# frankyeh/UNet-Studio

Measured on AMD Instinct MI355X. Metric: voxels/sec 3D U-Net train step @128^3 bf16, higher is better.
Workload: dtype bf16

## Files before the change

### include/unet_hip.h

```cpp
#ifndef UNET_HIP_H
#define UNET_HIP_H
#include <stddef.h>
#include <stdint.h>

#ifdef __cplusplus
extern "C" {
#endif

#define UNET_DTYPE_F32 0
#define UNET_DTYPE_BF16 1

#define UNET_IMPL_AUTO 0
#define UNET_IMPL_DIRECT 1

typedef struct unet_plan unet_plan;

const char* unet_last_error(void);
void unet_set_error(const char* msg);

int unet_init(int* n_devices);
int unet_device_info(int device, char* name, size_t name_len, size_t* total_mem, int* compute_units, int* gcn_arch_is_gfx950);

int unet_plan_create(const char* arch_dsl, int in_c, int out_c, int D, int H, int W, int dtype, int device, int impl,
                     unet_plan** out);
void unet_plan_destroy(unet_plan* plan);

int unet_plan_param_count(const unet_plan* plan, int* n);
int unet_plan_param_shape(const unet_plan* plan, int i, int64_t dims[5], int* ndim);
int unet_plan_param_name(const unet_plan* plan, int i, char* name, size_t name_len);
int unet_plan_param_decay(const unet_plan* plan, int i, int* decay);
int unet_plan_param_fan_in(const unet_plan* plan, int i, int64_t* fan_in, int* is_norm_weight);
int unet_plan_buffer_count(const unet_plan* plan, int* n);
int unet_plan_buffer_shape(const unet_plan* plan, int i, int64_t* numel);
int unet_plan_output_count(const unet_plan* plan, int* n);
int unet_plan_output_shape(const unet_plan* plan, int level, int64_t dims[5]);
int unet_plan_workspace_bytes(const unet_plan* plan, size_t* bytes);
int unet_plan_flops(const unet_plan* plan, double* fwd, double* bwd);
size_t unet_plan_describe(const unet_plan* plan, char* buf, size_t len);

int unet_plan_op_count(const unet_plan* plan, int* n);
int unet_plan_op_info(const unet_plan* plan, int i, int* kind, int* cin, int* cout, int* ks, int* stride, int64_t in_dims[3],
                      int64_t out_dims[3], char* name, size_t name_len);

#define UNET_PROF_CONV_FWD 0
#define UNET_PROF_DGRAD 1
#define UNET_PROF_WGRAD 2
#define UNET_PROF_NORM_FWD 3
#define UNET_PROF_NORM_BWD 4
#define UNET_PROF_OTHER 5
int unet_profile_begin(void);
int unet_profile_end(int max_records, int* op_index, int* category, float* ms, int* n_records);

#define UNET_MODE_PACKS_CURRENT 2
int unet_forward(const unet_plan* plan, const float* const* params, float* const* buffers, const float* x,
                 float* const* outs, void* workspace, int mode, void* stream);

int unet_backward(const unet_plan* plan, const float* const* params, const float* const* grad_outs,
                  float* const* grad_params, float* grad_x, void* workspace, void* stream);

int unet_plan_backward_buckets(const unet_plan* plan, int max_buckets, int* n_buckets, int* op_lo, int64_t* elem_lo);
int unet_backward_part(const unet_plan* plan, const float* const* params, const float* const* grad_outs, float* const* grad_params,
                       float* grad_x, void* workspace, int op_hi, int op_lo, void* stream);

int unet_loss_scratch_bytes(const unet_plan* plan, size_t* bytes);
int unet_loss(const unet_plan* plan, const float* const* outs, const int64_t* target, int cost_mask, int collapse_before,
              float* const* grad_outs, float* losses_out, void* scratch, void* stream);

int unet_forward_loss(const unet_plan* plan, const float* const* params, float* const* buffers, const float* x, float* const* outs,
                      const int64_t* target, int cost_mask, int collapse_before, float* const* grad_outs, float* losses_out,
                      void* loss_scratch, void* workspace, void* stream);
int unet_forward_loss_mode(const unet_plan* plan, const float* const* params, float* const* buffers, const float* x, float* const* outs,
                           const int64_t* target, int cost_mask, int collapse_before, float* const* grad_outs, float* losses_out,
                           void* loss_scratch, void* workspace, int mode, void* stream);

int unet_stream_create_cu_range(int device, int cu_first, int cu_count, void** stream);
int unet_stream_destroy(void* stream);
int unet_plan_side_cu_range(unet_plan* plan, int cu_first, int cu_count);

int unet_pack_filters(const unet_plan* plan, const float* const* params, void* workspace, int with_dgrad, int* made, void* stream);

#define UNET_SUM_MAX_BUFFERS 64
int unet_sum_buffers(const float* const* bufs, int n, float* out, int64_t count, int zero_inputs, void* stream);

int unet_sgd_step(const unet_plan* plan, float* params_flat, float* grads_flat, float* momentum_flat, float lr,
                  float momentum, int nesterov, float weight_decay, float clip_norm, float grad_scale, float* norm_out,
                  void* scratch, void* stream);

int unet_op_scratch_bytes(int cin, int cout, int D, int H, int W, size_t* bytes);
int unet_op_conv3d_fwd(int dtype, int impl, const void* x, const float* w, const float* b, void* y, int cin, int cout, int D,
                       int H, int W, int ks, int stride, void* scratch, void* stream);
int unet_op_conv3d_fwd_fused(int dtype, int impl, const void* x, const float* scale, const float* shift, int act, const float* w,
                             const float* b, void* y, float* stats, int cin, int cout, int D, int H, int W, int ks, int stride,
                             void* scratch, void* stream);
int unet_op_conv3d_pack(int dtype, const float* w, void* wpacked, int cin, int cout, int D, int H, int W, int ks, int stride,
                        void* stream);
int unet_op_conv3d_fwd_packed(int dtype, const void* x, const void* wpacked, const float* b, void* y, float* stats_partials,
                              int cin, int cout, int D, int H, int W, int ks, int stride, void* stream);
int unet_op_conv3d_bwd_data(int dtype, int impl, const void* dy, const float* w, void* dx, int cin, int cout, int D, int H,
                            int W, int ks, int stride, void* scratch, void* stream);
int unet_op_conv3d_fwd_norm(const void* x0, const void* x1, int cin0, int cin1, const float* w, const float* b, const float* gamma,
                            const float* beta, double eps, float* rm, float* rv, double momentum, int use_running, int act, void* y,
                            void* y_act, float* stat, int cout, int D, int H, int W, int stride, void* scratch, void* stream);
int unet_op_conv3d_bwd_data_norm(int transposed, const void* dy, const float* w, void* dx, int accumulate, const void* u, const float* stat,
                                 const float* gamma, int act, float* coef, float* dgamma, float* dbeta, int cin, int cout, int D, int H,
                                 int W, void* scratch, void* stream);
int unet_op_conv3d_bwd_weight(int dtype, int impl, const void* x, const void* dy, float* dw, float* db, int cin, int cout,
                              int D, int H, int W, int ks, int stride, void* scratch, void* stream);
int unet_op_convt_fwd(int dtype, int impl, const void* x, const float* w, const float* b, void* y, int cin, int cout, int D,
                      int H, int W, void* scratch, void* stream);
int unet_op_convt_bwd_data(int dtype, int impl, const void* dy, const float* w, void* dx, int cin, int cout, int D, int H,
                           int W, void* scratch, void* stream);
int unet_op_convt_bwd_weight(int dtype, int impl, const void* x, const void* dy, float* dw, float* db, int cin, int cout,
                             int D, int H, int W, void* scratch, void* stream);
int unet_op_pack_ndhwc(int dtype, const float* x_ncdhw, void* y_ndhwc, int C, int64_t S, void* stream);
int unet_op_unpack_ncdhw(int dtype, const void* x_ndhwc, float* y_ncdhw, int C, int64_t S, void* stream);

#define UNET_COMM_ID_BYTES 128
typedef struct unet_comm unet_comm;
int unet_comm_unique_id(void* id_bytes );
int unet_comm_create(int rank, int world, const void* id_bytes, int device, unet_comm** out);
int unet_comm_create_all(int n, const int* devices, unet_comm** out );
int unet_comm_destroy(unet_comm* comm);
int unet_comm_rank(const unet_comm* comm, int* rank, int* world);
int unet_allreduce_grads(unet_comm* comm, float* flat, int64_t elem_lo, int64_t elem_hi, void* stream);
int unet_allreduce_grads_all(unet_comm* const* comms, int n, float* const* flats, int64_t elem_lo, int64_t elem_hi, void* const* streams);
int unet_comm_broadcast(unet_comm* comm, float* buf, int64_t n, int root, void* stream);
int unet_comm_join(unet_comm* comm, void* stream);

#ifdef __cplusplus
}
#endif
#endif
```

### unet-studio_amd/csrc/engine.cpp

```cpp
#include <hip/hip_runtime.h>

#include <algorithm>
#include <atomic>
#include <cmath>
#include <cstdio>
#include <cstring>
#include <functional>
#include <stdexcept>
#include <string>
#include <mutex>
#include <random>
#include <unordered_map>
#include <vector>

#include "../../include/unet_hip.h"
#include "conv_select.h"
#include "graph.hpp"
#include "kernels.h"

using namespace unet;

namespace {

thread_local std::string g_err;
int fail(const std::string& m) { g_err = m; return 1; }

#define HIP_OK(expr)                                                                              \
    do {                                                                                          \
        hipError_t e_ = (expr);                                                                   \
        if (e_ != hipSuccess) throw std::runtime_error(std::string(#expr) + ": " + hipGetErrorString(e_)); \
    } while (0)

struct DeviceGuard {
    int prev = -1;
    explicit DeviceGuard(int dev) {
        HIP_OK(hipGetDevice(&prev));
        if (prev != dev) HIP_OK(hipSetDevice(dev));
        else prev = -1;
    }
    ~DeviceGuard() { if (prev >= 0) (void)hipSetDevice(prev); }
};

size_t align_up(size_t v, size_t a = 256) { return (v + a - 1) / a * a; }

struct EnvSwitches {
    bool no_side_stream = getenv("UNET_NO_SIDE_STREAM"), no_first_wgrad_fuse = getenv("UNET_NO_FIRST_WGRAD_FUSE"), op_polite = getenv("UNET_OP_POLITE");
};
const EnvSwitches& env() { static const EnvSwitches e; return e; }

struct ProfRec { int op, cat; hipEvent_t e0, e1; };
struct ProfSink { std::vector<ProfRec> recs; };
thread_local ProfSink* g_prof = nullptr;
struct ProfScope {
    ProfRec r{};
    hipStream_t s = nullptr;
    bool on = false;
    ProfScope(int op, int cat, hipStream_t st) {
        if (!g_prof) return;
        on = true; s = st; r.op = op; r.cat = cat;
        if (hipEventCreate(&r.e0) != hipSuccess || hipEventCreate(&r.e1) != hipSuccess) { on = false; return; }
        (void)hipEventRecord(r.e0, s);
    }
    ~ProfScope() {
        if (!on) return;
        (void)hipEventRecord(r.e1, s);
        g_prof->recs.push_back(r);
    }
};

}

struct unet_plan {
    Graph g;
    int dtype = 0, device = 0, impl = 0;
    size_t elsize = 4;
    std::vector<size_t> t_off, g_off;
    std::vector<size_t> a_off;
    std::vector<size_t> n_stat, n_coef;
    std::vector<size_t> w_fwd, w_dgrad;
    std::vector<size_t> wm_fwd, wm_dgrad;
    std::vector<int> n_consumers;
    std::vector<int> first_consumer;
    mutable std::mutex bn_mu;
    mutable std::unordered_map<const void*, std::pair<int, int>> bn_pending;
    mutable std::unordered_map<const void*, std::vector<int>> bn_done;
    std::vector<ConvChoice> conv;
    size_t wgrad_off = 0;
    std::vector<size_t> wz_off;
    std::vector<int> wz_job_of_op;
    std::vector<WgradReduceJob> wz_jobs;
    WgradReduceJob* wz_jobs_dev = nullptr;
    size_t partial_off = 0, partial_bytes = 0;
    size_t ws_bytes = 0;
    size_t loss_bytes = 0;
    std::vector<int64_t> p_off;
    std::vector<PackJob> pack_jobs;
    int64_t pack_blocks = 0;
    PackJob* jobs_dev = nullptr;
    SgdSeg* segs_dev = nullptr;
    int nseg = 0;
    int64_t n_param_elems = 0;

    hipStream_t side = nullptr;
    hipEvent_t ev_fork = nullptr, ev_join = nullptr, ev_pack = nullptr, ev_packd = nullptr;
    int pack_split_op = 0;
    int64_t pack_split_blocks = 0, pack_fwd_blocks = 0;
    size_t head_off = 0;
    size_t deep_part_off = 0, deep_part_bytes = 0, deep_cnt_off = 0;
    static constexpr int deep_ncnt = 4096;
    std::vector<size_t> head_op_off;

    ~unet_plan() {
        if (segs_dev) (void)hipFree(segs_dev);
        if (wz_jobs_dev) (void)hipFree(wz_jobs_dev);
        if (jobs_dev) (void)hipFree(jobs_dev);
        if (ev_fork) (void)hipEventDestroy(ev_fork);
        if (ev_join) (void)hipEventDestroy(ev_join);
        if (ev_pack) (void)hipEventDestroy(ev_pack);
        if (ev_packd) (void)hipEventDestroy(ev_packd);
        if (side) (void)hipStreamDestroy(side);
    }

    ConvGeom op_geom_of(const Op& op) const {
        const Tensor& a = g.tensors[op.src[0]];
        const Tensor& o = g.tensors[op.dst];
        ConvGeom cg;
        cg.Cin = op.cin; cg.Cout = op.cout; cg.D = a.D; cg.H = a.H; cg.W = a.W; cg.Do = o.D; cg.Ho = o.H; cg.Wo = o.W;
        cg.ks = op.ks; cg.stride = op.stride;
        return cg;
// ... 19 lines not shown
            const Op& op = g.ops[i];
            if (op.kind == OP_CONV || op.kind == OP_CONVT) side_polite[i] = wgrad_on_main[i] ? 0 : 1;
        }
    }

    bool head_only(size_t t) const {
        if (dtype != UNET_DTYPE_BF16 || g.tensors[t].norm < 0 || g.tensors[t].C % 16) return false;
        int readers = 0;
        for (size_t i = 0; i < g.ops.size(); ++i) {
            const Op& op = g.ops[i];
            if (op.kind == OP_NORM) continue;
            for (int k = 0; k < op.nsrc; ++k) {
                if (op.src[k] != (int)t) continue;
                if (conv[i].fwd != Fwd::head) return false;
                ++readers;
            }
        }
        return readers > 0;
    }
    void layout() {
        choose_polite();
        conv.assign(g.ops.size(), ConvChoice());
        for (size_t i = 0; i < g.ops.size(); ++i) {
            const Op& op = g.ops[i];
            if (op.kind != OP_CONV && op.kind != OP_CONVT) continue;
            SrcDesc sd[2];
            src_chans(op, sd);
            conv[i] = choose_conv(dtype, impl, op_geom_of(op), sd, op.nsrc, op.out_level >= 0, op.kind == OP_CONVT);
        }
        size_t off = 0;
        auto take = [&](size_t bytes) { size_t o = off; off = align_up(off + bytes); return o; };
        t_off.assign(g.tensors.size(), SIZE_MAX);
        g_off.assign(g.tensors.size(), SIZE_MAX);
        n_consumers.assign(g.tensors.size(), 0);
        first_consumer.assign(g.tensors.size(), -1);
        for (size_t oi = 0; oi < g.ops.size(); ++oi) {
            const Op& op = g.ops[oi];
            for (int k = 0; k < op.nsrc && op.kind != OP_NORM; ++k)
                if (op.src[k] >= 0) { ++n_consumers[op.src[k]]; if (first_consumer[op.src[k]] < 0) first_consumer[op.src[k]] = (int)oi; }
        }
        a_off.assign(g.tensors.size(), SIZE_MAX);
        for (size_t i = 0; i < g.tensors.size(); ++i) {
            t_off[i] = take((size_t)g.tensors[i].numel() * elsize);
            if (g.tensors[i].needs_grad) g_off[i] = take((size_t)g.tensors[i].numel() * elsize);
            if (impl == UNET_IMPL_AUTO && (g.tensors[i].norm >= 0 || g.tensors[i].act != ACT_NONE) && !head_only(i))
                a_off[i] = take((size_t)g.tensors[i].numel() * elsize);
        }
        n_stat.resize(g.norms.size()); n_coef.resize(g.norms.size());
        size_t pmax = 0;
        for (size_t i = 0; i < g.norms.size(); ++i) {
            n_stat[i] = take(4 * (size_t)g.norms[i].C * 4);
            n_coef[i] = take(3 * (size_t)g.norms[i].C * 4);
            size_t pb = (size_t)stats_blocks(g.tensors[g.norms[i].tensor].voxels()) * g.norms[i].C * 2 * (dtype == UNET_DTYPE_F32 ? 8 : 4);
            if (pb > pmax) pmax = pb;
        }
        w_fwd.assign(g.ops.size(), SIZE_MAX); w_dgrad.assign(g.ops.size(), SIZE_MAX);
        wm_fwd.assign(g.ops.size(), SIZE_MAX); wm_dgrad.assign(g.ops.size(), SIZE_MAX);
        auto grow = [](size_t& m, size_t b) { if (b > m) m = b; };
        for (size_t i = 0; i < g.ops.size(); ++i) {
            const Op& op = g.ops[i];
            if (op.kind != OP_CONV && op.kind != OP_CONVT) continue;
            const ConvChoice& c = conv[i];
            const ConvGeom cg = op_geom_of(op);
            int k3 = op.kind == OP_CONV ? op.ks * op.ks * op.ks : 8;
            w_fwd[i] = take((size_t)k3 * op.cin * round_up(op.cout, 8) * 4);
            w_dgrad[i] = take((size_t)k3 * op.cout * round_up(op.cin, 8) * 4);
            if (op.kind == OP_CONVT) {
                if (c.mfma_fwd()) { wm_fwd[i] = take(mfma_convt_w_bytes(cg)); wm_dgrad[i] = take(mfma_convt_dgrad_w_bytes(cg)); }
                continue;
            }
            const bool stats = g.tensors[op.dst].norm >= 0;
            SrcDesc sd[2];
            src_chans(op, sd);
            if (c.mfma_fwd()) {
                wm_fwd[i] = take(mfma_conv_w_bytes(cg));
                if (stats) grow(pmax, (size_t)mfma_conv_blocks(cg) * op.cout * 2 * 4);
            }
            if (c.fwd == Fwd::first_f32_mfma && stats) grow(pmax, (size_t)conv_first_f32_mfma_blocks(cg) * op.cout * 2 * 8);
            if (c.fwd == Fwd::f32_mfma && stats) grow(pmax, (size_t)conv_f32_mfma_stat_rows(cg, sd) * op.cout * 2 * 8);
            if (c.dgrad == Dgrad::mfma) {
                wm_dgrad[i] = take(mfma_conv_dgrad_w_bytes(cg));
                if (op.stride == 2) grow(pmax, (size_t)s2_conv_dgrad_rows_max() * op.cin * 2 * 4);
            }
        }
        partial_bytes = pmax ? pmax : 256;
        partial_off = take(partial_bytes);
        size_t wmax = 0, hmax = 0;
        for (size_t i = 0; i < g.ops.size(); ++i) {
            const Op& op = g.ops[i];
            if (op.kind != OP_CONV && op.kind != OP_CONVT) continue;
            const ConvChoice& c = conv[i];
            const ConvGeom cg = op_geom_of(op);
            grow(wmax, wgrad_direct_scratch_bytes(cg, op.kind == OP_CONVT));
            if (op.kind == OP_CONVT) {
                if (c.wgrad == Wgrad::mfma) {
                    grow(wmax, mfma_convt_wgrad_scratch_bytes(cg));
                    grow(wmax, bias_grad_scratch_bytes(cg.Cout, (int64_t)cg.Do * cg.Ho * cg.Wo));
                }
                continue;
            }
            if (c.wgrad == Wgrad::mfma) grow(wmax, mfma_wgrad_scratch_bytes(cg, side_polite[i]));
            if (c.wgrad == Wgrad::f32_mfma) grow(wmax, wgrad_f32_mfma_scratch_bytes(cg));
            if (wgrad_small_supported(cg, op.nsrc)) grow(wmax, wgrad_small_scratch_bytes(cg));
            if (cg.Cin == 1 && (cg.Cout == 16 || cg.Cout == 32)) grow(wmax, conv_first_wgrad_mfma_scratch_bytes(cg));
            if (head_supported(cg, op.nsrc)) grow(hmax, head_bwd_scratch_bytes(cg));
        }
        wgrad_off = take(wmax ? wmax : 256);
        head_off = take(hmax ? hmax : 256);
        if (dtype == UNET_DTYPE_BF16 && impl == UNET_IMPL_AUTO) {
            deep_part_bytes = (size_t)8 << 20;
            deep_part_off = take(deep_part_bytes);
            deep_cnt_off = take((size_t)deep_ncnt * 4);
        }
        head_op_off.assign(g.ops.size(), SIZE_MAX);
        for (size_t i = 0; i < g.ops.size(); ++i)
            if (conv[i].fwd == Fwd::head) head_op_off[i] = take(head_bwd_scratch_bytes(op_geom_of(g.ops[i])));
        wz_off.assign(g.ops.size(), SIZE_MAX);
        for (size_t i = 0; i < g.ops.size(); ++i) {
            const Op& op = g.ops[i];
            const Wgrad w = conv[i].wgrad;
            if (op.out_level >= 0 || (w != Wgrad::first_mfma && w != Wgrad::mfma)) continue;
            const ConvGeom cg = op_geom_of(op);
            if (w == Wgrad::first_mfma) wz_off[i] = take(conv_first_wgrad_mfma_scratch_bytes(cg));
            else if (op.kind == OP_CONV) { if (!mfma_conv_wgrad_direct(cg)) wz_off[i] = take(mfma_wgrad_scratch_bytes(cg, side_polite[i])); }
            else if (!mfma_convt_wgrad_direct(cg)) wz_off[i] = take(mfma_convt_wgrad_scratch_bytes(cg));
        }
        ws_bytes = off;
        p_off.assign(g.params.size() + 1, 0);
        for (size_t i = 0; i < g.params.size(); ++i) {
            int64_t n = 1;
            for (auto d : g.params[i].shape) n *= d;
            p_off[i + 1] = p_off[i] + n;
        }
        wz_jobs.clear();
        wz_job_of_op.assign(g.ops.size(), -1);
        int wz_blk = 0;
        for (size_t i = 0; i < g.ops.size(); ++i) {
            if (wz_off[i] == SIZE_MAX) continue;
            const Op& op = g.ops[i];
            ConvGeom cg = op_geom_of(op);
            WgradReduceJob j;
            j.op = (int)i;
            j.slab_off = (long long)(wz_off[i] / 4);
            j.dw_off = p_off[op.weight];
            j.Cb = op.cout;
            if (op.kind == OP_CONVT) {
                j.nsplit = mfma_convt_wgrad_splits(cg);
                j.n = (long long)8 * op.cin * op.cout;
                j.bias_off = op.bias >= 0 ? j.slab_off + (long long)j.nsplit * j.n : -1;
                j.db_off = op.bias >= 0 ? p_off[op.bias] : -1;
            } else {
                j.nsplit = conv[i].wgrad == Wgrad::first_mfma ? conv_first_wgrad_splits(cg) : mfma_conv_wgrad_splits(cg, side_polite[i]);
                j.n = (long long)27 * op.cin * op.cout;
                j.bias_off = op.bias >= 0 ? j.slab_off + (long long)j.nsplit * j.n : -1;
                j.db_off = op.bias >= 0 ? p_off[op.bias] : -1;
            }
            wz_blk += wgrad_reduce_job_blocks(j, wz_blk);
            wz_job_of_op[i] = (int)wz_jobs.size();
            wz_jobs.push_back(j);
        }
        pack_jobs.clear();
        pack_blocks = 0;
        pack_split_op = -1; pack_split_blocks = 0; pack_fwd_blocks = 0;
        for (int which = 0; which < 2; ++which) {
            for (size_t i = 0; i < g.ops.size(); ++i) {
                const Op& op = g.ops[i];
// ... 193 lines not shown
                        case Fwd::first_f32_mfma:
                            rows = launch_conv_first_f32_mfma(cg, sd, params[op.weight], params[op.bias], (float*)tptr(op.dst), (double*)part, s);
                            if (mode == 1 && !packs_current) launch_pack_conv_w(params[op.weight], wf, wd, op.cin, op.cout, k3, s);
                            break;
                        case Fwd::f32_mfma:
                            if (!packs_current) launch_pack_conv_w(params[op.weight], wf, wd, op.cin, op.cout, k3, s);
                            rows = launch_conv_f32_mfma(cg, sd, op.nsrc, wf, params[op.bias], (float*)tptr(op.dst), s, (double*)part);
                            break;
                        case Fwd::direct:
                            if (!packs_current) launch_pack_conv_w(params[op.weight], wf, wd, op.cin, op.cout, k3, s);
                            launch_conv_fwd_direct(p.dtype, cg, sd, op.nsrc, wf, params[op.bias], tptr(op.dst),
                                                   op.out_level >= 0 ? outs[op.out_level] : nullptr, s);
                            break;
                    }
                    if (want_stats) {
                        fused_blocks[T.norm] = rows;
                        fused_dbl[T.norm] = c.fwd == Fwd::first_f32_mfma || c.fwd == Fwd::f32_mfma;
                    }
                    break;
                }
                case OP_NORM: {
                    const Norm& n = g.norms[op.norm];
                    const Tensor& T = g.tensors[n.tensor];
                    if (fused_done[op.norm]) break;
                    norm_fwd_passes(p.dtype, tptr(n.tensor), n.C, T.voxels(), partial(), fused_blocks[op.norm], fused_dbl[op.norm] != 0,
                                    n.batch && mode == 0, params[n.gamma], params[n.beta], n.eps, stat(op.norm),
                                    n.batch ? buffers[n.buffer] : nullptr, n.batch ? buffers[n.buffer + 1] : nullptr, T.act,
                                    p.a_off[n.tensor] != SIZE_MAX ? ws + p.a_off[n.tensor] : nullptr, s);
                    break;
                }
                case OP_MATERIALIZE: {
                    SrcDesc sd[2] = {src(op.src[0]), op.nsrc > 1 ? src(op.src[1]) : SrcDesc()};
                    launch_materialize(p.dtype, sd, op.nsrc, tptr(op.dst), g.tensors[op.dst].voxels(), s);
                    break;
                }
                case OP_MAXPOOL: {
                    const Tensor& a = g.tensors[op.src[0]];
                    launch_maxpool_fwd(p.dtype, src(op.src[0]), tptr(op.dst), a.D, a.H, a.W, s);
                    break;
                }
                case OP_UPSAMPLE: {
                    const Tensor& a = g.tensors[op.src[0]];
                    launch_upsample_fwd(p.dtype, src(op.src[0]), tptr(op.dst), a.D, a.H, a.W, s);
                    break;
                }
                case OP_EXPORT:
                    if (outs && outs[op.out_level])
                        launch_export(p.dtype, src(op.src[0]), outs[op.out_level], g.tensors[op.src[0]].voxels(), s);
                    break;
            }
            if (op.kind != OP_NORM && op.kind != OP_EXPORT && op.dst >= 0) {
                const Tensor& T = g.tensors[op.dst];
                if (T.norm < 0 && T.act != ACT_NONE) apply_view(op.dst);
            }
            if (on_head && op.out_level >= 0 && outs && outs[op.out_level] && (op.kind == OP_CONV || op.kind == OP_CONVT || op.kind == OP_EXPORT))
                (*on_head)(op.out_level);
        }
        need_packs();
    }

    void view_backward(int t, const float* const* params, float* const* gparams, bool no_apply = false) {
        const Tensor& T = p.g.tensors[t];
        if (T.norm >= 0) {
            const Norm& n = p.g.norms[T.norm];
            int have = 0;
            {
                std::lock_guard<std::mutex> lk(p.bn_mu);
                auto d = p.bn_done.find(ws);
                if (d != p.bn_done.end()) {
                    auto f = std::find(d->second.begin(), d->second.end(), t);
                    if (f != d->second.end()) { d->second.erase(f); return; }
                }
                auto it = p.bn_pending.find(ws);
                if (it != p.bn_pending.end()) { if (it->second.first == t) have = it->second.second; p.bn_pending.erase(it); }
            }
            norm_bwd_passes(p.dtype, gptr(t), tptr(t), T.C, T.voxels(), stat(T.norm), T.act, params[n.gamma], coef(T.norm),
                            gparams[n.gamma], gparams[n.beta], partial(), have, no_apply, s);
        } else if (T.act != ACT_NONE) {
            launch_act_bwd(p.dtype, gptr(t), tptr(t), T.act, T.numel(), s);
        }
    }

    void backward(const float* const* params, const float* const* grad_outs, float* const* gparams, float* grad_x, int op_hi = 1 << 30,
                  int op_lo = 0) {
        const Graph& g = p.g;
        if (p.side) HIP_OK(hipStreamWaitEvent(s, p.ev_packd, 0));
        {
            bool flat = p.jobs_dev != nullptr;
            for (size_t k = 0; k < g.params.size() && flat; ++k) flat = params[k] == params[0] + p.p_off[k];
            deep_on = flat;
        }
        std::vector<char> init(g.tensors.size(), 0);
        auto dst_of = [&](int t) {
            DstGrad d;
            d.C = g.tensors[t].C;
            d.ptr = g.tensors[t].needs_grad ? gptr(t) : nullptr;
            d.accumulate = init[t];
            return d;
        };
        auto mark = [&](const Op& op) {
            for (int k = 0; k < op.nsrc; ++k)
                if (g.tensors[op.src[k]].needs_grad) init[op.src[k]] = 1;
        };
        const hipStream_t sb = (p.side && !env().no_side_stream && !g_prof) ? p.side : s;
        auto fork = [&]() {
            if (sb == s) return;
            HIP_OK(hipEventRecord(p.ev_fork, s));
            HIP_OK(hipStreamWaitEvent(sb, p.ev_fork, 0));
        };
        if (op_lo < 0) op_lo = 0;
        if (op_hi >= (int)g.ops.size()) { std::lock_guard<std::mutex> lk(p.bn_mu); p.bn_pending.erase(ws); p.bn_done.erase(ws); }
        bool gflat = p.wz_jobs_dev != nullptr;
        for (size_t k = 0; k < g.params.size() && gflat; ++k) gflat = gparams[k] == gparams[0] + p.p_off[k];
        std::vector<char> wz_ran(p.wz_jobs.size(), 0);
        int wz_pending = 0;
        auto flush_wz = [&](hipStream_t st) {
            for (size_t j = 0; j < wz_ran.size();) {
                if (!wz_ran[j]) { ++j; continue; }
                size_t e = j;
                int nblk = 0;
                while (e < wz_ran.size() && wz_ran[e]) { nblk += p.wz_jobs[e].nblk; wz_ran[e] = 0; ++e; }
                ProfScope pr(-1, UNET_PROF_WGRAD, st);
                launch_wgrad_reduce_batched(p.wz_jobs_dev, (int)j, (int)(e - j), p.wz_jobs[j].blk0, nblk, ws, gparams[0], st);
                j = e;
            }
            wz_pending = 0;
        };
        auto do_wgrad = [&](int i) {
            const Op& op = g.ops[i];
            const int t = op.dst;
            SrcDesc sd[2] = {src(op.src[0]), op.nsrc > 1 ? src(op.src[1]) : SrcDesc()};
            ConvGeom cg = geom(op);
            const bool on_main = op.kind == OP_CONV && p.wgrad_on_main[i] && p.wz_off[i] != SIZE_MAX;
            const bool defer = gflat && p.wz_job_of_op[i] >= 0 && !on_main;
            {
            ProfScope pw(i, UNET_PROF_WGRAD, sb);
            switch (p.conv[i].wgrad) {
                case Wgrad::first_mfma:
                    launch_conv_first_wgrad_mfma(cg, sd, gptr(t), gparams[op.weight], gparams[op.bias],
                                                 ws + (defer ? p.wz_off[i] : p.wgrad_off), sb, defer);
                    break;
                case Wgrad::mfma:
                    if (op.kind == OP_CONVT)
                        launch_mfma_convt_wgrad(cg, sd, gptr(t), gparams[op.weight], ws + (defer ? p.wz_off[i] : p.wgrad_off), sb, defer, gparams[op.bias],
                                                p.side_polite[i]);
                    else if (on_main)
                        launch_mfma_conv_wgrad(cg, sd, op.nsrc, gptr(t), gparams[op.weight], gparams[op.bias], ws + p.wz_off[i], s, false, 0);
                    else
                        launch_mfma_conv_wgrad(cg, sd, op.nsrc, gptr(t), gparams[op.weight], gparams[op.bias],
                                               ws + (p.wz_off[i] != SIZE_MAX ? p.wz_off[i] : p.wgrad_off), sb, defer, p.side_polite[i]);
                    break;
                case Wgrad::f32_mfma:
                    launch_wgrad_f32_mfma(cg, sd, op.nsrc, (const float*)gptr(t), gparams[op.weight], gparams[op.bias], ws + p.wgrad_off, sb);
                    break;
                case Wgrad::small:
                    launch_conv_wgrad_small(p.dtype, cg, sd, op.nsrc, gptr(t), gparams[op.weight], gparams[op.bias], ws + p.wgrad_off, sb);
                    break;
                case Wgrad::direct:
                    if (op.kind == OP_CONVT)
                        launch_convt_wgrad_direct(p.dtype, cg, sd, op.nsrc, gptr(t), gparams[op.weight], gparams[op.bias], ws + p.wgrad_off, sb);
                    else
                        launch_conv_wgrad_direct(p.dtype, cg, sd, op.nsrc, gptr(t), gparams[op.weight], gparams[op.bias], ws + p.wgrad_off, sb);
                    break;
            }
            }
            if (defer) { wz_ran[p.wz_job_of_op[i]] = 1; ++wz_pending; }
            if (wz_pending >= 3) flush_wz(sb);
        };
        const int64_t hold_from = (int64_t)64 * 64 * 64, hold_below = (int64_t)32 * 32 * 32;
        std::vector<int> held;
        bool deep_seen = false;
        constexpr int fork_every = 3;
        std::vector<int> pending;
        auto issue_pending = [&]() {
            if (pending.empty()) return;
            fork();
            for (int h : pending) do_wgrad(h);
            pending.clear();
        };
        for (int i = (int)g.ops.size() - 1; i >= op_lo; --i) {
            const Op& op = g.ops[i];
            const bool dry = i >= op_hi;
            if (op.kind == OP_NORM) continue;
            if (op.kind == OP_EXPORT) {
                if (grad_outs && grad_outs[op.out_level] && g.tensors[op.src[0]].needs_grad) {
                    if (!dry) launch_export_bwd(p.dtype, grad_outs[op.out_level], dst_of(op.src[0]), g.tensors[op.src[0]].voxels(), s);
                    mark(op);
                }
                continue;
            }
            int t = op.dst;
            if ((op.kind == OP_CONV) && op.out_level >= 0) {
                if (!(grad_outs && grad_outs[op.out_level])) continue;
                if (p.conv[i].fwd == Fwd::head) {
                    DstGrad dgh = dst_of(op.src[0]);
                    ProfScope ph(dry ? -2 : i, UNET_PROF_OTHER, s);
                    if (!dry) {
                        const bool defer = sb != s && p.head_op_off[i] != SIZE_MAX;
                        char* hs = ws + (defer ? p.head_op_off[i] : p.head_off);
                        launch_head_bwd(p.dtype, geom(op), src(op.src[0]), grad_outs[op.out_level], nullptr, params[op.weight], dgh,
                                        gparams[op.weight], gparams[op.bias], hs, s, defer);
                        if (defer) { fork(); launch_head_bwd_reduce(geom(op), gparams[op.weight], gparams[op.bias], hs, sb); }
                    }
                    if (dgh.ptr) mark(op);
                    continue;
                }
                if (!dry) launch_import_grad(p.dtype, grad_outs[op.out_level], gptr(t), g.tensors[t].C, g.tensors[t].voxels(), 0, s);
                init[t] = 1;
            }
            if (!g.tensors[t].needs_grad || !init[t]) continue;
            bool first_fused = false;
            if (!dry && p.conv[i].wgrad == Wgrad::first_mfma && g.tensors[t].norm >= 0 && !g.tensors[op.src[0]].needs_grad && sb != s &&
                p.wz_off[i] != SIZE_MAX && g.tensors[t].C % 8 == 0)
                first_fused = !env().no_first_wgrad_fuse;
            if (!dry) { ProfScope ps(i, UNET_PROF_NORM_BWD, s); view_backward(t, params, gparams, first_fused); }
            switch (op.kind) {
                case OP_CONV:
                case OP_CONVT: {
                    SrcDesc sd[2] = {src(op.src[0]), op.nsrc > 1 ? src(op.src[1]) : SrcDesc()};
                    DstGrad dg[2] = {dst_of(op.src[0]), op.nsrc > 1 ? dst_of(op.src[1]) : DstGrad()};
                    ConvGeom cg = geom(op);
                    const float* wd = (const float*)(ws + p.w_dgrad[i]);
                    bool any = dg[0].ptr || (op.nsrc > 1 && dg[1].ptr);
                    if (!dry && !any && sb != s && p.conv[i].wgrad == Wgrad::first_mfma && p.wz_off[i] != SIZE_MAX) {
                        ProfScope pw(i, UNET_PROF_WGRAD, s);
                        const Tensor& To = g.tensors[t];
                        NormBwdFuse nf = {tptr(t), first_fused ? stat(To.norm) : nullptr, first_fused ? coef(To.norm) : nullptr, To.act};
                        launch_conv_first_wgrad_mfma(cg, sd, gptr(t), gparams[op.weight], gparams[op.bias], ws + p.wz_off[i], s, false,
                                                     first_fused ? &nf : nullptr);
                    } else
                    if (!dry) {
                        const int64_t vox = (int64_t)cg.Do * cg.Ho * cg.Wo;
                        if (!deep_seen && vox <= hold_below && !held.empty()) {
                            deep_seen = true;
                            pending.insert(pending.begin(), held.begin(), held.end());
                            held.clear();
                            pending.push_back(i);
                            issue_pending();
                        } else if (!deep_seen && sb != s && vox >= hold_from) held.push_back(i);
                        else {
                            pending.push_back(i);
                            if ((int)pending.size() >= fork_every || sb == s || vox >= hold_below) issue_pending();
                        }
                    }
                    ProfScope pd(i, UNET_PROF_DGRAD, s);
                    if (!dry && any) switch (p.conv[i].dgrad) {
                        case Dgrad::mfma: {
                            const int ts = op.src[0];
                            const Tensor& Ts = g.tensors[ts];
                            const bool can = op.nsrc == 1 && Ts.norm >= 0 && p.first_consumer[ts] == i && p.dtype == UNET_DTYPE_BF16;
                            DeepNormBwd nb;
                            if (can) {
                                const Norm& n = g.norms[Ts.norm];
                                nb = {tptr(ts), stat(Ts.norm), params[n.gamma], coef(Ts.norm), gparams[n.gamma], gparams[n.beta], Ts.act};
                            }
                            if (op.kind == OP_CONVT) {
                                int norm_done = 0;
                                if (deep_on && launch_deep_convt_dgrad(cg, gptr(t), ws + p.wm_dgrad[i], dg, op.nsrc, can ? &nb : nullptr, deep(), &norm_done, s)) {
                                    if (norm_done) { std::lock_guard<std::mutex> lk(p.bn_mu); p.bn_done[ws].push_back(ts); }
                                } else
                                    launch_mfma_convt_dgrad(cg, gptr(t), ws + p.wm_dgrad[i], dg, op.nsrc, s);
                                break;
                            }
                            BnBwdStats bn = {tptr(ts), Ts.norm >= 0 ? stat(Ts.norm) : nullptr, partial(), Ts.act, Ts.C};
                            int rows = 0;
                            const int served = deep_on ? launch_deep_conv_dgrad(cg, gptr(t), ws + p.wm_dgrad[i], dg, op.nsrc, can ? &nb : nullptr, deep(), s) : 0;
                            if (served == 2) { std::lock_guard<std::mutex> lk(p.bn_mu); p.bn_done[ws].push_back(ts); }
                            if (!served) rows = launch_mfma_conv_dgrad(cg, gptr(t), ws + p.wm_dgrad[i], dg, op.nsrc, s, can ? &bn : nullptr);
                            if (rows > 0) { std::lock_guard<std::mutex> lk(p.bn_mu); p.bn_pending[ws] = {ts, rows}; }
                            break;
                        }
                        case Dgrad::f32_mfma: launch_conv_f32_mfma_dgrad(cg, (const float*)gptr(t), wd, dg, op.nsrc, s); break;
                        case Dgrad::direct:
                            if (op.kind == OP_CONVT) launch_convt_dgrad_direct(p.dtype, cg, gptr(t), wd, dg, op.nsrc, s);
                            else launch_conv_dgrad_direct(p.dtype, cg, gptr(t), wd, dg, op.nsrc, s);
// ... 142 lines not shown
    if (i < 0 || i >= (int)p->g.params.size()) return fail("parameter index out of range");
    const auto& s = p->g.params[i].shape;
    *ndim = (int)s.size();
    for (size_t k = 0; k < s.size(); ++k) dims[k] = s[k];
    return 0;
}
int unet_plan_param_name(const unet_plan* p, int i, char* name, size_t name_len) {
    if (i < 0 || i >= (int)p->g.params.size()) return fail("parameter index out of range");
    if (name && name_len) { std::strncpy(name, p->g.params[i].name.c_str(), name_len - 1); name[name_len - 1] = 0; }
    return 0;
}
int unet_plan_param_decay(const unet_plan* p, int i, int* decay) {
    if (i < 0 || i >= (int)p->g.params.size()) return fail("parameter index out of range");
    *decay = p->g.params[i].decay;
    return 0;
}
int unet_plan_param_fan_in(const unet_plan* p, int i, int64_t* fan_in, int* is_norm_weight) {
    if (i < 0 || i >= (int)p->g.params.size()) return fail("parameter index out of range");
    *fan_in = p->g.params[i].fan_in; *is_norm_weight = p->g.params[i].norm_weight;
    return 0;
}
int unet_plan_buffer_count(const unet_plan* p, int* n) { *n = (int)p->g.buffers.size(); return 0; }
int unet_plan_buffer_shape(const unet_plan* p, int i, int64_t* numel) {
    if (i < 0 || i >= (int)p->g.buffers.size()) return fail("buffer index out of range");
    *numel = p->g.buffers[i];
    return 0;
}
int unet_plan_output_count(const unet_plan* p, int* n) { *n = (int)p->g.outputs.size(); return 0; }
int unet_plan_output_shape(const unet_plan* p, int l, int64_t dims[5]) {
    if (l < 0 || l >= (int)p->g.outputs.size()) return fail("output level out of range");
    const auto& o = p->g.outputs[l];
    dims[0] = 1; dims[1] = o.C; dims[2] = o.D; dims[3] = o.H; dims[4] = o.W;
    return 0;
}
int unet_plan_workspace_bytes(const unet_plan* p, size_t* bytes) { *bytes = p->ws_bytes; return 0; }
int unet_plan_flops(const unet_plan* p, double* fwd, double* bwd) { *fwd = p->g.flops_fwd; *bwd = p->g.flops_bwd; return 0; }
size_t unet_plan_describe(const unet_plan* p, char* buf, size_t len) {
    std::string d = p->g.describe();
    if (buf && len) { std::strncpy(buf, d.c_str(), len - 1); buf[len - 1] = 0; }
    return d.size() + 1;
}

int unet_forward(const unet_plan* p, const float* const* params, float* const* buffers, const float* x, float* const* outs,
                 void* workspace, int mode, void* stream) {
    try {
        if (!p || !params || !x || !workspace) throw std::runtime_error("unet_forward: null argument");
        if (mode & ~(1 | UNET_MODE_PACKS_CURRENT)) throw std::runtime_error("unet_forward: unknown mode bits (0 = eval, 1 = train, optionally | UNET_MODE_PACKS_CURRENT)");
        if (!p->g.buffers.empty() && !buffers) throw std::runtime_error("unet_forward: architecture has bnorm layers but buffers is null");
        DeviceGuard dg(p->device);
        Exec ex(*p, workspace, stream);
        ex.forward(params, buffers, x, outs, mode);
        check_launch();
        return 0;
    } catch (const std::exception& e) { return fail(e.what()); }
}

int unet_backward(const unet_plan* p, const float* const* params, const float* const* grad_outs, float* const* grad_params,
                  float* grad_x, void* workspace, void* stream) {
    try {
        if (!p || !params || !grad_params || !workspace) throw std::runtime_error("unet_backward: null argument");
        if (grad_x) throw std::runtime_error("unet_backward: grad_x must be NULL -- dL/dx is not computed (the input carries no gradient, as in train.cpp:619-628)");
        DeviceGuard dg(p->device);
        Exec ex(*p, workspace, stream);
        ex.backward(params, grad_outs, grad_params, grad_x);
        check_launch();
        return 0;
    } catch (const std::exception& e) { return fail(e.what()); }
}

int unet_backward_part(const unet_plan* p, const float* const* params, const float* const* grad_outs, float* const* grad_params,
                       float* grad_x, void* workspace, int op_hi, int op_lo, void* stream) {
    try {
        if (!p || !params || !grad_params || !workspace) throw std::runtime_error("unet_backward_part: null argument");
        if (op_lo < 0 || op_hi < op_lo) throw std::runtime_error("unet_backward_part: invalid op range");
        if (grad_x) throw std::runtime_error("unet_backward_part: grad_x must be NULL -- dL/dx is not computed");
        DeviceGuard dg(p->device);
        Exec ex(*p, workspace, stream);
        ex.backward(params, grad_outs, grad_params, grad_x, op_hi, op_lo);
        check_launch();
        return 0;
    } catch (const std::exception& e) { return fail(e.what()); }
}

int unet_plan_backward_buckets(const unet_plan* p, int max_buckets, int* n_buckets, int* op_lo, int64_t* elem_lo) {
    try {
        if (!p || !n_buckets || !op_lo || !elem_lo || max_buckets < 1) throw std::runtime_error("unet_plan_backward_buckets: bad argument");
        const Graph& g = p->g;
        const int nops = (int)g.ops.size();
        std::vector<int64_t> first(nops, INT64_MAX);
        bool monotone = true;
        int64_t prev = -1;
        for (int i = 0; i < nops; ++i) {
            const Op& op = g.ops[i];
            if (op.kind != OP_CONV && op.kind != OP_CONVT) continue;
            int64_t f = p->p_off[op.weight];
            if (op.bias >= 0 && p->p_off[op.bias] < f) f = p->p_off[op.bias];
            first[i] = f;
            if (f <= prev) monotone = false;
            prev = f;
            const Tensor& T = g.tensors[op.dst];
            if (T.norm >= 0) {
                const Norm& n = g.norms[T.norm];
                if (p->p_off[n.gamma] < f || p->p_off[n.beta] < f) monotone = false;
            }
        }
        int nb = 0;
        if (monotone && max_buckets > 1) {
            const double thr = (double)p->n_param_elems / ((double)max_buckets - 0.5);
            int64_t hi = p->n_param_elems;
            for (int i = nops - 1; i > 0 && nb < max_buckets - 1; --i) {
                if (first[i] == INT64_MAX) continue;
                if ((double)(hi - first[i]) >= thr) { op_lo[nb] = i; elem_lo[nb] = first[i]; hi = first[i]; ++nb; }
            }
        }
        op_lo[nb] = 0; elem_lo[nb] = 0; ++nb;
        *n_buckets = nb;
        return 0;
    } catch (const std::exception& e) { return fail(e.what()); }
}

int unet_plan_op_count(const unet_plan* p, int* n) { *n = (int)p->g.ops.size(); return 0; }
int unet_plan_op_info(const unet_plan* p, int i, int* kind, int* cin, int* cout, int* ks, int* stride, int64_t in_dims[3],
                      int64_t out_dims[3], char* name, size_t name_len) {
    if (i < 0 || i >= (int)p->g.ops.size()) return fail("op index out of range");
    const Op& op = p->g.ops[i];
    if (kind) *kind = (int)op.kind;
    if (cin) *cin = op.cin;
    if (cout) *cout = op.cout;
    if (ks) *ks = op.ks;
    if (stride) *stride = op.stride;
    const Tensor* a = op.nsrc > 0 && op.src[0] >= 0 ? &p->g.tensors[op.src[0]] : nullptr;
    const Tensor* o = op.dst >= 0 ? &p->g.tensors[op.dst] : nullptr;
    if (in_dims) { in_dims[0] = a ? a->D : 0; in_dims[1] = a ? a->H : 0; in_dims[2] = a ? a->W : 0; }
    if (out_dims) { out_dims[0] = o ? o->D : 0; out_dims[1] = o ? o->H : 0; out_dims[2] = o ? o->W : 0; }
    if (name && name_len) { std::strncpy(name, op.name.c_str(), name_len - 1); name[name_len - 1] = 0; }
    return 0;
}

int unet_profile_begin(void) {
    if (g_prof) return fail("unet_profile_begin: a profile is already open on this thread");
    g_prof = new ProfSink();
    return 0;
}
int unet_profile_end(int max_records, int* op_index, int* category, float* ms, int* n_records) {
    if (!g_prof) return fail("unet_profile_end: no open profile on this thread");
    ProfSink* ps = g_prof;
    g_prof = nullptr;
    int n = 0, rc = 0;
    for (auto& r : ps->recs) {
        float t = 0.f;
        hipError_t e = hipEventSynchronize(r.e1);
        if (e == hipSuccess) e = hipEventElapsedTime(&t, r.e0, r.e1);
        if (e != hipSuccess) rc = fail(std::string("unet_profile_end: ") + hipGetErrorString(e));
        if (r.op != -2 && n < max_records && op_index && category && ms) { op_index[n] = r.op; category[n] = r.cat; ms[n] = t; ++n; }
        (void)hipEventDestroy(r.e0); (void)hipEventDestroy(r.e1);
    }
    if (n_records) *n_records = n;
    delete ps;
    return rc;
}

int unet_loss_scratch_bytes(const unet_plan* p, size_t* bytes) { *bytes = p->loss_bytes; return 0; }

namespace {
struct LossRun {
    const unet_plan* p;
    const float* const* outs; const int64_t* target; float* const* grad_outs; float* losses_out;
    int C, oc, collapse, cost_mask;
    float inv;
    std::vector<int64_t*> tgt;
    std::vector<float*> lvl;
    float* partial[2];
    LossRun(const unet_plan* plan, const float* const* outs_, const int64_t* target_, int cost_mask_, int collapse_before, float* const* grad_outs_,
            float* losses_out_, void* scratch)
        : p(plan), outs(outs_), target(target_), grad_outs(grad_outs_), losses_out(losses_out_), collapse(collapse_before), cost_mask(cost_mask_) {
        if (!p || !outs || !target || !losses_out || !scratch) throw std::runtime_error("unet_loss: null argument");
        const Graph& g = p->g;
        C = g.out_c;
        if (collapse_before < 0 || collapse_before >= C) throw std::runtime_error("invalid collapse_before");
        oc = collapse_before ? C - collapse_before + 1 : C;
        const size_t nl = g.outputs.size();
        float wsum = 0.f;
        for (size_t k = 0; k < nl; ++k) wsum += 1.0f / (float)(1 << k);
        inv = 1.0f / wsum;
        char* sc = (char*)scratch;
        size_t off = 0;
        tgt.resize(nl); lvl.resize(nl);
        for (size_t l = 0; l < nl; ++l) {
            int64_t S = (int64_t)(g.D >> l) * (g.H >> l) * (g.W >> l);
            if (S <= 0) S = 1;
            tgt[l] = (int64_t*)(sc + off); off = align_up(off + (size_t)S * 8);
            lvl[l] = (float*)(sc + off); off = align_up(off + (size_t)(4 + 2 * C) * 4);
        }
        partial[0] = (float*)(sc + off); off = align_up(off + (size_t)1024 * (3 + 2 * C) * 4);
        partial[1] = (float*)(sc + off);
        int D = g.D, H = g.H, W = g.W;
        for (size_t k = 0; k < nl; ++k) {
            if (k > 0) {
                if ((D >> 1) <= 0 || (H >> 1) <= 0 || (W >> 1) <= 0) throw std::runtime_error("deep supervision target size became zero");
                D >>= 1; H >>= 1; W >>= 1;
            }
            const auto& o = g.outputs[k];
            if (o.C == 0 || !outs[k]) throw std::runtime_error("undefined deep supervision output at level " + std::to_string(k));
            if (o.C != C)
                throw std::runtime_error("output channel mismatch at level " + std::to_string(k) + ": tensor has " + std::to_string(o.C) +
                                         ", out_count is " + std::to_string(C));
            if (o.D != D || o.H != H || o.W != W) throw std::runtime_error("deep supervision output/target size mismatch at level " + std::to_string(k));
        }
    }
    size_t levels() const { return p->g.outputs.size(); }
    const int64_t* target_of(size_t k) const { return k == 0 ? target : tgt[k]; }
    int64_t voxels(size_t k) const { const auto& o = p->g.outputs[k]; return (int64_t)o.D * o.H * o.W; }
    void prepare(hipStream_t s) {
        HIP_OK(hipMemsetAsync(losses_out, 0, 4 * sizeof(float), s));
        const Graph& g = p->g;
        int D = g.D, H = g.H, W = g.W;
        for (size_t k = 1; k < levels(); ++k) {
            launch_target_half(target_of(k - 1), tgt[k], D, H, W, s);
            D >>= 1; H >>= 1; W >>= 1;
        }
    }
    void level_partial(size_t k, int area, hipStream_t s) { launch_loss_partial(outs[k], target_of(k), C, voxels(k), collapse, partial[area], s); }
    void level_finish(size_t k, int area, hipStream_t s) {
        const float w = (1.0f / (float)(1 << k)) * inv;
        launch_loss_finalize(partial[area], loss_blocks(voxels(k)), oc, w, cost_mask, lvl[k], losses_out, k == 0, s);
        if (grad_outs && grad_outs[k]) launch_loss_grad(outs[k], target_of(k), C, voxels(k), collapse, lvl[k], w, cost_mask, grad_outs[k], s);
    }
};
}

int unet_loss(const unet_plan* p, const float* const* outs, const int64_t* target, int cost_mask, int collapse_before,
              float* const* grad_outs, float* losses_out, void* scratch, void* stream) {
    try {
        LossRun lr(p, outs, target, cost_mask, collapse_before, grad_outs, losses_out, scratch);
        DeviceGuard dg(p->device);
        hipStream_t s = (hipStream_t)stream;
        lr.prepare(s);
        for (size_t k = 0; k < lr.levels(); ++k) { lr.level_partial(k, 0, s); lr.level_finish(k, 0, s); }
        check_launch();
        return 0;
    } catch (const std::exception& e) { return fail(e.what()); }
}

int unet_forward_loss(const unet_plan* p, const float* const* params, float* const* buffers, const float* x, float* const* outs,
                      const int64_t* target, int cost_mask, int collapse_before, float* const* grad_outs, float* losses_out,
                      void* loss_scratch, void* workspace, void* stream) {
    return unet_forward_loss_mode(p, params, buffers, x, outs, target, cost_mask, collapse_before, grad_outs, losses_out, loss_scratch, workspace, 1,
                                  stream);
}

int unet_forward_loss_mode(const unet_plan* p, const float* const* params, float* const* buffers, const float* x, float* const* outs,
                           const int64_t* target, int cost_mask, int collapse_before, float* const* grad_outs, float* losses_out,
                           void* loss_scratch, void* workspace, int mode, void* stream) {
    try {
        if ((mode & 1) != 1 || (mode & ~(1 | UNET_MODE_PACKS_CURRENT)))
            throw std::runtime_error("unet_forward_loss_mode: mode must be 1 (train), optionally | UNET_MODE_PACKS_CURRENT");
        if (!p || !params || !x || !workspace || !outs) throw std::runtime_error("unet_forward_loss: null argument");
        if (!p->g.buffers.empty() && !buffers) throw std::runtime_error("unet_forward_loss: architecture has bnorm layers but buffers is null");
        LossRun lr(p, outs, target, cost_mask, collapse_before, grad_outs, losses_out, loss_scratch);
        DeviceGuard dg(p->device);
        hipStream_t s = (hipStream_t)stream;
        const bool side = p->side && !env().no_side_stream && !g_prof;
        Exec ex(*p, workspace, stream);
        if (!side) {
            ex.forward(params, buffers, x, outs, mode);
            lr.prepare(s);
            for (size_t k = 0; k < lr.levels(); ++k) { lr.level_partial(k, 0, s); lr.level_finish(k, 0, s); }
            check_launch();
            return 0;
        }
        hipStream_t sd = p->side;
        bool prepared = false;
        constexpr bool per_level = false;
        std::function<void(int)> on_head = [&](int level) {
            if (level < 1 || (size_t)level >= lr.levels()) return;
            if (!per_level && level != 1) return;
            HIP_OK(hipEventRecord(p->ev_fork, s));
            HIP_OK(hipStreamWaitEvent(sd, p->ev_fork, 0));
            if (!prepared) { lr.prepare(sd); prepared = true; }
            for (size_t k = per_level ? (size_t)level : lr.levels() - 1; k >= (size_t)level; --k) {
                lr.level_partial(k, 1, sd);
                lr.level_finish(k, 1, sd);
            }
        };
        ex.forward(params, buffers, x, outs, mode, &on_head);
        if (!prepared) {
            HIP_OK(hipEventRecord(p->ev_fork, s));
            HIP_OK(hipStreamWaitEvent(sd, p->ev_fork, 0));
            lr.prepare(sd);
        }
        lr.level_partial(0, 0, s);
        HIP_OK(hipEventRecord(p->ev_join, sd));
        HIP_OK(hipStreamWaitEvent(s, p->ev_join, 0));
        lr.level_finish(0, 0, s);
        check_launch();
        return 0;
    } catch (const std::exception& e) { return fail(e.what()); }
}

static bool create_cu_range_stream(int device, int cu_first, int cu_count, hipStream_t* out) {
    hipDeviceProp_t prop;
    if (cu_count <= 0 || hipGetDeviceProperties(&prop, device) != hipSuccess || prop.multiProcessorCount % 8 != 0) return false;
    const int per_xcd = prop.multiProcessorCount / 8;
    if (cu_count >= per_xcd) return false;
    std::vector<uint32_t> mask((prop.multiProcessorCount + 31) / 32, 0u);
    for (int c = 0; c < cu_count; ++c) {
        const int cu = ((cu_first + c) % per_xcd + per_xcd) % per_xcd;
        for (int x = 0; x < 8; ++x) { const int bit = cu * 8 + x; mask[bit / 32] |= 1u << (bit % 32); }
    }
    if (hipExtStreamCreateWithCUMask(out, (uint32_t)mask.size(), mask.data()) != hipSuccess) { (void)hipGetLastError(); return false; }
    return true;
}

int unet_stream_create_cu_range(int device, int cu_first, int cu_count, void** stream) {
    try {
        if (!stream) throw std::runtime_error("unet_stream_create_cu_range: null argument");
        DeviceGuard dg(device);
        hipStream_t st = nullptr;
        if (!create_cu_range_stream(device, cu_first, cu_count, &st)) throw std::runtime_error("unet_stream_create_cu_range: the device / driver does not take this CU range");
        *stream = (void*)st;
        return 0;
    } catch (const std::exception& e) { return fail(e.what()); }
}
int unet_stream_destroy(void* stream) {
    if (stream && hipStreamDestroy((hipStream_t)stream) != hipSuccess) return fail("hipStreamDestroy failed");
    return 0;
}
int unet_plan_side_cu_range(unet_plan* p, int cu_first, int cu_count) {
    try {
        if (!p) throw std::runtime_error("unet_plan_side_cu_range: null plan");
        if (!p->side) return 0;
        DeviceGuard dg(p->device);
        hipStream_t st = nullptr;
        if (!create_cu_range_stream(p->device, cu_first, cu_count, &st)) throw std::runtime_error("unet_plan_side_cu_range: the device / driver does not take this CU range");
        HIP_OK(hipStreamSynchronize(p->side));
        HIP_OK(hipStreamDestroy(p->side));
        p->side = st;
        return 0;
    } catch (const std::exception& e) { return fail(e.what()); }
}

int unet_pack_filters(const unet_plan* p, const float* const* params, void* workspace, int with_dgrad, int* made, void* stream) {
// ... 556 lines not shown
```

### unet-studio_amd/csrc/kernels.h

```cpp
#pragma once
#include <hip/hip_runtime.h>
#include <cstdint>

#include "../../include/unet_augment.h"
#include "../../include/unet_feed.h"
#include "../../include/unet_hip.h"
#include "../../include/unet_postproc.h"
#include "../../include/unet_qc.h"

namespace unet {

struct SrcDesc {
    const void* ptr = nullptr;
    int C = 0;
    const float* scale = nullptr;
    const float* shift = nullptr;
    int act = 0;
};
struct DstGrad {
    void* ptr = nullptr;
    int C = 0;
    int accumulate = 0;
};

// ... 35 lines not shown
void launch_norm_eval(int C, const float* gamma, const float* beta, const float* rm, const float* rv, double eps, float* stat,
                      hipStream_t s);

void launch_act_bwd(int dtype, void* g, const void* u, int act, int64_t n, hipStream_t s);
void launch_norm_bwd_partial(int dtype, void* g, const void* u, int C, int64_t S, const float* stat, int act, float* partial,
                             hipStream_t s);
void launch_norm_bwd_finalize(const float* partial, int nblk, int C, int64_t S, const float* gamma, const float* stat, float* coef,
                              float* dgamma, float* dbeta, hipStream_t s, bool dbl = false);
bool launch_norm_finalize_apply(int dtype, const float* partial, int nblk, int C, int64_t S, const float* gamma, const float* beta, double eps,
                                float* stat, float* running_mean, float* running_var, double momentum, const void* raw, int act, void* out,
                                hipStream_t s);
bool launch_norm_bwd_finalize_apply(int dtype, const float* partial, int nblk, int C, int64_t S, const float* gamma, const float* stat,
                                    float* coef, float* dgamma, float* dbeta, void* g, const void* u, int act, hipStream_t s);
void launch_norm_bwd_apply(int dtype, void* g, const void* u, int C, int64_t S, const float* stat, const float* coef, int act,
                           hipStream_t s);

void launch_maxpool_fwd(int dtype, SrcDesc src, void* out, int D, int H, int W, hipStream_t s);
void launch_maxpool_bwd(int dtype, SrcDesc src, const void* gout, DstGrad dst, int D, int H, int W, hipStream_t s);
void launch_upsample_fwd(int dtype, SrcDesc src, void* out, int D, int H, int W, hipStream_t s);
void launch_upsample_bwd(int dtype, const void* gout, DstGrad dst, int D, int H, int W, hipStream_t s);
void launch_materialize(int dtype, const SrcDesc* src, int nsrc, void* out, int64_t S, hipStream_t s);
void launch_apply_view(int dtype, SrcDesc src, void* out, int64_t S, hipStream_t s);
void launch_materialize_bwd(int dtype, const void* gout, const DstGrad* dst, int ndst, int64_t S, hipStream_t s);
void launch_export_bwd(int dtype, const float* g_ncdhw, DstGrad dst, int64_t S, hipStream_t s);
void launch_unpack_ncdhw(int dtype, const void* g, float* out_ncdhw, int C, int64_t S, hipStream_t s);

void launch_target_half(const int64_t* t, int64_t* o, int D, int H, int W, hipStream_t s);
int loss_blocks(int64_t S);
void launch_loss_partial(const float* logits, const int64_t* target, int C, int64_t S, int collapse, float* partial, hipStream_t s);
void launch_loss_finalize(const float* partial, int nblk, int oc, float level_weight, int cost_mask, float* level_out, float* totals,
                          int set_stats, hipStream_t s);
void launch_loss_grad(const float* logits, const int64_t* target, int C, int64_t S, int collapse, const float* level_out,
                      float level_weight, int cost_mask, float* dlogits, hipStream_t s);

void launch_sum_buffers(const float* const* bufs, int n, float* out, int64_t count, int zero_inputs, hipStream_t s);

struct SgdSeg { int64_t offset, count; float wd; };
void launch_sumsq_partial(const float* g, int64_t n, float scale, float* partial, int nblk, hipStream_t s);
void launch_sgd(float* p, float* g, float* m, int64_t n, const SgdSeg* segs_dev, int nseg, const float* partial, int nblk,
                float lr, float momentum, int nesterov, float weight_decay, float clip_norm, float grad_scale, float* norm_out,
                hipStream_t s);

struct PackJob { int64_t src_off, dst_off, total, blk0; int Ci, Co, CK, T, mode, A, B, pad; };
int mfma_conv_pack_jobs(const ConvGeom& g, bool want_dgrad, PackJob* out2);
int mfma_convt_pack_jobs(const ConvGeom& g, PackJob* out2);
void launch_mfma_pack_batched(const float* params_base, void* ws, const PackJob* jobs_dev, int njobs, int64_t nblocks, hipStream_t s,
                              int64_t blk_base = 0, int max_grid = 0, int* zero = nullptr, int nzero = 0);
bool mfma_conv_fwd_supported(int dtype, const ConvGeom& g, const SrcDesc* src, int nsrc);
size_t mfma_conv_w_bytes(const ConvGeom& g);
void launch_mfma_pack_conv_w(const float* w, void* w_mfma_fwd, void* w_mfma_dgrad, const ConvGeom& g, hipStream_t s);
int launch_mfma_conv_fwd(const ConvGeom& g, const SrcDesc* src, int nsrc, const void* w_mfma, const float* bias, void* out,
                         float* stats_partial, hipStream_t s);
bool conv_first_mfma_supported(int dtype, const ConvGeom& g, const SrcDesc* src, int nsrc);
int conv_first_mfma_blocks(const ConvGeom& g);
int launch_conv_first_mfma(const ConvGeom& g, const SrcDesc* src, const float* w, const float* bias, void* out, float* stats_partial,
                           hipStream_t s);
int mfma_conv_blocks(const ConvGeom& g);
bool mfma_wgrad_z_supported(int dtype, const ConvGeom& g, const SrcDesc* src, int nsrc);
size_t mfma_wgrad_z_scratch_bytes(const ConvGeom& g, int polite = 0);
int mfma_wgrad_z_splits(const ConvGeom& g, int polite = 0);
int launch_mfma_wgrad_z(const ConvGeom& g, const SrcDesc* src, int nsrc, const void* dy, bool want_bias, void* scratch, hipStream_t s,
                        int polite = 0);
void wgrad_reduce(const float* slab, const float* bias_slab, int nsplit, int64_t n, int Cb, float* dw, float* db, hipStream_t s);
struct WgradReduceJob { long long slab_off, bias_off, dw_off, db_off, n; int nsplit, Cb, ly, blk0, nblk, op; };
int wgrad_reduce_job_blocks(WgradReduceJob& j, int blk0);
void launch_wgrad_reduce_batched(const WgradReduceJob* jobs_dev, int job0, int njobs, int blk_base, int nblocks, const void* ws, float* gflat,
                                 hipStream_t s);
bool mfma_wgrad_supported(int dtype, const ConvGeom& g, const SrcDesc* src, int nsrc);
size_t mfma_wgrad_scratch_bytes(const ConvGeom& g, int polite = 0);
int mfma_conv_wgrad_splits(const ConvGeom& g, int polite = 0);
int mfma_convt_wgrad_splits(const ConvGeom& g);
bool mfma_conv_wgrad_direct(const ConvGeom& g);
bool mfma_convt_wgrad_direct(const ConvGeom& g);
int conv_first_wgrad_splits(const ConvGeom& g);
void launch_mfma_conv_wgrad(const ConvGeom& g, const SrcDesc* src, int nsrc, const void* dy, float* dw, float* db, void* scratch,
                            hipStream_t s, bool defer_reduce = false, int polite = 0);
bool head_supported(const ConvGeom& g, int nsrc);
size_t head_bwd_scratch_bytes(const ConvGeom& g);
void launch_head_fwd(int dtype, const ConvGeom& g, const SrcDesc& src, const float* w, const float* bias, void* y, float* out_ncdhw,
                     hipStream_t s);
void launch_head_bwd(int dtype, const ConvGeom& g, const SrcDesc& src, const float* dy_ncdhw, const void* dy_cl, const float* w,
                     DstGrad dst, float* dw, float* db, void* scratch, hipStream_t s, bool defer_reduce = false);
void launch_head_bwd_reduce(const ConvGeom& g, float* dw, float* db, const void* scratch, hipStream_t s);
bool conv_first_wgrad_mfma_supported(int dtype, const ConvGeom& g, const SrcDesc* src, int nsrc);
size_t conv_first_wgrad_mfma_scratch_bytes(const ConvGeom& g);
struct NormBwdFuse { const void* u; const float* stat; const float* coef; int act; };
void launch_conv_first_wgrad_mfma(const ConvGeom& g, const SrcDesc* src, const void* dy, float* dw, float* db, void* scratch, hipStream_t s,
                                  bool defer_reduce = false, const NormBwdFuse* nb_fuse = nullptr);
bool wgrad_small_supported(const ConvGeom& g, int nsrc);
size_t wgrad_small_scratch_bytes(const ConvGeom& g);
void launch_conv_wgrad_small(int dtype, const ConvGeom& g, const SrcDesc* src, int nsrc, const void* dy, float* dw, float* db,
                             void* scratch, hipStream_t s);
bool mfma_convt_wgrad_supported(int dtype, const ConvGeom& g, const SrcDesc* src, int nsrc);
size_t mfma_convt_wgrad_scratch_bytes(const ConvGeom& g);
void launch_mfma_convt_wgrad(const ConvGeom& g, const SrcDesc* src, const void* dy, float* dw, void* scratch, hipStream_t s,
                             bool defer_reduce = false, float* db = nullptr, int polite = 0);
int launch_colsum_partial8(int dtype, const void* x, int C, int64_t S, float* partial, hipStream_t s);
size_t bias_grad_scratch_bytes(int C, int64_t S);
void launch_bias_grad(int dtype, const void* dy, int C, int64_t S, float* db, void* scratch, hipStream_t s);
bool mfma_conv_dgrad_supported(int dtype, const ConvGeom& g, const SrcDesc* src, int nsrc);
size_t mfma_conv_dgrad_w_bytes(const ConvGeom& g);
struct BnBwdStats { const void* u; const float* stat; float* partial; int act, C; };
int launch_mfma_conv_dgrad(const ConvGeom& g, const void* dy, const void* w_mfma_dgrad, const DstGrad* dst, int ndst, hipStream_t s,
                           const BnBwdStats* bn = nullptr);
int launch_s2_conv_fwd(const ConvGeom& g, const SrcDesc* src, int nsrc, const void* w_mfma, const float* bias, void* out, float* stats_partial,
                       hipStream_t s);
int launch_s2_conv_dgrad(const ConvGeom& g, const void* dy, const void* w_s2_dgrad, const DstGrad* dst, int ndst, hipStream_t s,
                         const BnBwdStats* bn);
int s2_conv_dgrad_rows_max();
bool launch_s2_convt_fwd(const ConvGeom& g, const SrcDesc* src, int nsrc, const void* w_mfma, const float* bias, void* out, hipStream_t s);
bool launch_s2_convt_dgrad(const ConvGeom& g, const void* dy, const void* w_mfma_dgrad, const DstGrad* dst, int ndst, hipStream_t s);
int s2_wgrad_splits(int Ca, int Cb, int cD, int cH, int cW);
int launch_s2_wgrad(int ks, const void* fine, const void* fine2, int C0, int Ca, int fD, int fH, int fW, const void* coarse, int Cb, int cD, int cH,
                    int cW, bool want_bias, int bias_from_a, void* scratch, hipStream_t s, int polite);
constexpr int64_t DEEP_MAX_VOXELS = 512;
struct DeepScratch { float* part = nullptr; size_t part_bytes = 0; int* cnt = nullptr; int ncnt = 0; };
struct DeepNormFwd {
    const float* gamma; const float* beta; double eps; float* stat; float* rm; float* rv; double momentum; int use_running; int act;
    void* act_out;
};
struct DeepNormBwd {
    const void* u; const float* stat; const float* gamma; float* coef; float* dgamma; float* dbeta; int act;
};
bool deep_conv_applies(int dtype, int64_t out_voxels, int cin, int cout);
bool launch_deep_conv_fwd(const ConvGeom& g, const SrcDesc* src, int nsrc, const void* w_mfma, const float* bias, void* out,
                          const DeepNormFwd* nf, const DeepScratch& sc, hipStream_t s);
bool launch_deep_convt_fwd(const ConvGeom& g, const SrcDesc* src, int nsrc, const void* w_mfma, const float* bias, void* out,
                           const DeepScratch& sc, hipStream_t s);
int launch_deep_conv_dgrad(const ConvGeom& g, const void* dy, const void* w_mfma_dgrad, const DstGrad* dst, int ndst, const DeepNormBwd* nb,
                           const DeepScratch& sc, hipStream_t s);
bool launch_deep_convt_dgrad(const ConvGeom& g, const void* dy, const void* w_mfma_dgrad, const DstGrad* dst, int ndst, const DeepNormBwd* nb,
                             const DeepScratch& sc, int* norm_done, hipStream_t s);
bool mfma_convt_supported(int dtype, const ConvGeom& g, const SrcDesc* src, int nsrc);
size_t mfma_convt_w_bytes(const ConvGeom& g);
size_t mfma_convt_dgrad_w_bytes(const ConvGeom& g);
void launch_mfma_pack_convt_w(const float* w, void* w_mfma_fwd, void* w_mfma_dgrad, const ConvGeom& g, hipStream_t s);
void launch_mfma_convt_fwd(const ConvGeom& g, const SrcDesc* src, int nsrc, const void* w_mfma, const float* bias, void* out, hipStream_t s);
void launch_mfma_convt_dgrad(const ConvGeom& g, const void* dy, const void* w_mfma_dgrad, const DstGrad* dst, int ndst, hipStream_t s);

bool conv_f32_mfma_supported(int dtype, const ConvGeom& g, const SrcDesc* src, int nsrc);
int conv_f32_mfma_stat_rows(const ConvGeom& g, const SrcDesc* src);
int launch_conv_f32_mfma(const ConvGeom& g, const SrcDesc* src, int nsrc, const float* w_fwd, const float* bias, float* out,
                         hipStream_t s, double* stats_partial = nullptr);
bool conv_first_f32_mfma_supported(int dtype, const ConvGeom& g, const SrcDesc* src, int nsrc);
int conv_first_f32_mfma_blocks(const ConvGeom& g);
int launch_conv_first_f32_mfma(const ConvGeom& g, const SrcDesc* src, const float* w, const float* bias, float* out, double* stats_partial,
                               hipStream_t s);
bool convt_f32_mfma_supported(int dtype, const ConvGeom& g, const SrcDesc* src, int nsrc);
void launch_convt_f32_mfma(const ConvGeom& g, const SrcDesc* src, const float* w_fwd, const float* bias, float* out, hipStream_t s);
bool wgrad_f32_mfma_supported(int dtype, const ConvGeom& g, const SrcDesc* src, int nsrc);
size_t wgrad_f32_mfma_scratch_bytes(const ConvGeom& g);
void launch_wgrad_f32_mfma(const ConvGeom& g, const SrcDesc* src, int nsrc, const float* dy, float* dw, float* db, void* scratch,
                           hipStream_t s);
void slab_reduce_public(const float* slab, int nsplit, int64_t n, float* out, hipStream_t s);
bool conv_f32_mfma_dgrad_supported(int dtype, const ConvGeom& g, const DstGrad* dst, int ndst);
void launch_conv_f32_mfma_dgrad(const ConvGeom& g, const float* dy, const float* w_dgrad, const DstGrad* dst, int ndst, hipStream_t s);

size_t augment_scratch_bytes(const UnetAugmentRecipe& r);
void launch_augment(const UnetAugmentRecipe& r, float* image, float* label, void* scratch, hipStream_t st);
size_t simulate_scratch_bytes(const UnetSimulateRecipe& r);
void launch_simulate_modality(const UnetSimulateRecipe& r, float* t1w, const float* label, void* scratch, hipStream_t st);

size_t qc_scratch_bytes(int out_c, int64_t S, int collapse);
void launch_qc_counts(const float* logits, const float* label, const float* image0, int out_c, int64_t S, int collapse, int shift,
                      uint64_t* counts, void* scratch, hipStream_t s);

// ... 15 lines not shown
```

### unet-studio_amd/csrc/kernels_direct.hip

```cpp
#include "device_util.h"

namespace unet {

__global__ void k_pack_conv_w(const float* __restrict__ w, float* __restrict__ wf, float* __restrict__ wd, int Cin, int Cout,
                              int k3, int CoutP, int CinP) {
    int64_t i = (int64_t)blockIdx.x * blockDim.x + threadIdx.x;
    int64_t nf = (int64_t)k3 * Cin * CoutP, nd = (int64_t)k3 * Cout * CinP;
    if (i < nf) {
        int co = (int)(i % CoutP); int64_t r = i / CoutP;
        int ci = (int)(r % Cin); int t = (int)(r / Cin);
        wf[i] = co < Cout ? w[((int64_t)co * Cin + ci) * k3 + t] : 0.f;
    }
    if (i < nd) {
        int ci = (int)(i % CinP); int64_t r = i / CinP;
        int co = (int)(r % Cout); int t = (int)(r / Cout);
        wd[i] = ci < Cin ? w[((int64_t)co * Cin + ci) * k3 + t] : 0.f;
    }
}
__global__ void k_pack_convt_w(const float* __restrict__ w, float* __restrict__ wf, float* __restrict__ wd, int Cin, int Cout,
                               int CoutP, int CinP) {
    int64_t i = (int64_t)blockIdx.x * blockDim.x + threadIdx.x;
    int64_t nf = (int64_t)8 * Cin * CoutP, nd = (int64_t)8 * Cout * CinP;
    if (i < nf) {
        int co = (int)(i % CoutP); int64_t r = i / CoutP;
        int ci = (int)(r % Cin); int t = (int)(r / Cin);
        wf[i] = co < Cout ? w[((int64_t)ci * Cout + co) * 8 + t] : 0.f;
    }
    if (i < nd) {
        int ci = (int)(i % CinP); int64_t r = i / CinP;
        int co = (int)(r % Cout); int t = (int)(r / Cout);
        wd[i] = ci < Cin ? w[((int64_t)ci * Cout + co) * 8 + t] : 0.f;
    }
}
void launch_pack_conv_w(const float* w, float* wf, float* wd, int Cin, int Cout, int k3, hipStream_t s) {
    int CoutP = round_up(Cout, 8), CinP = round_up(Cin, 8);
    int64_t na = (int64_t)k3 * Cin * CoutP, nb = (int64_t)k3 * Cout * CinP;
    int64_t n = na > nb ? na : nb;
    k_pack_conv_w<<<cdiv64(n, 256), 256, 0, s>>>(w, wf, wd, Cin, Cout, k3, CoutP, CinP);
}
void launch_pack_convt_w(const float* w, float* wf, float* wd, int Cin, int Cout, hipStream_t s) {
    int CoutP = round_up(Cout, 8), CinP = round_up(Cin, 8);
    int64_t a = (int64_t)8 * Cin * CoutP, b = (int64_t)8 * Cout * CinP;
    k_pack_convt_w<<<cdiv64(a > b ? a : b, 256), 256, 0, s>>>(w, wf, wd, Cin, Cout, CoutP, CinP);
}

struct ConvFwdArgs {
    ConvGeom g;
    SrcDesc src[2];
    int nsrc;
    const float* w;
    const float* bias;
    void* out;
    float* out_ncdhw;
};

template <typename T> __global__ void __launch_bounds__(256) k_conv_fwd_direct(ConvFwdArgs a) {
    const ConvGeom& g = a.g;
    int64_t So = (int64_t)g.Do * g.Ho * g.Wo;
    int64_t v = (int64_t)blockIdx.x * 256 + threadIdx.x;
    if (v >= So) return;
    int co0 = blockIdx.y * 8, CoutP = round_up(g.Cout, 8);
    int x = (int)(v % g.Wo); int64_t r = v / g.Wo;
    int y = (int)(r % g.Ho); int z = (int)(r / g.Ho);
    int pad = (g.ks - 1) / 2;
    float acc[8];
#pragma unroll
    for (int j = 0; j < 8; ++j) acc[j] = (a.bias && co0 + j < g.Cout) ? a.bias[co0 + j] : 0.f;
    for (int kz = 0; kz < g.ks; ++kz) {
        int iz = z * g.stride + kz - pad;
        if (iz < 0 || iz >= g.D) continue;
        for (int ky = 0; ky < g.ks; ++ky) {
            int iy = y * g.stride + ky - pad;
            if (iy < 0 || iy >= g.H) continue;
            for (int kx = 0; kx < g.ks; ++kx) {
                int ix = x * g.stride + kx - pad;
                if (ix < 0 || ix >= g.W) continue;
                int64_t vin = ((int64_t)iz * g.H + iy) * g.W + ix;
                int tap = (kz * g.ks + ky) * g.ks + kx;
                int cb = 0;
                for (int s = 0; s < a.nsrc; ++s) {
                    const SrcDesc& sd = a.src[s];
                    for (int ci = 0; ci < sd.C; ++ci) {
                        float xv = view_ld<T>(sd, vin, ci);
// ... 610 lines not shown
            for (int u = 0; u < 4; ++u) {
                if constexpr (sizeof(T) == 2) {
                    const uint2 r = *(const uint2*)((const bf16*)dy + (vox + u) * g.Cout + co0);
                    ds[u][0] = __uint_as_float(r.x << 16); ds[u][1] = __uint_as_float(r.x & 0xffff0000u);
                    ds[u][2] = __uint_as_float(r.y << 16); ds[u][3] = __uint_as_float(r.y & 0xffff0000u);
                } else {
                    const float4 r = *(const float4*)((const float*)dy + (vox + u) * g.Cout + co0);
                    ds[u][0] = r.x; ds[u][1] = r.y; ds[u][2] = r.z; ds[u][3] = r.w;
                }
            }
#pragma unroll
            for (int kz = 0; kz < 3; ++kz)
#pragma unroll
                for (int ky = 0; ky < 3; ++ky)
#pragma unroll
                    for (int kx = 0; kx < 3; ++kx)
#pragma unroll
                        for (int u = 0; u < 4; ++u)
#pragma unroll
                            for (int c = 0; c < 4; ++c)
                                acc[((kz * 3 + ky) * 3 + kx) * 4 + c] = fmaf(in[kz][ky][u + kx], ds[u][c], acc[((kz * 3 + ky) * 3 + kx) * 4 + c]);
#pragma unroll
            for (int u = 0; u < 4; ++u)
#pragma unroll
                for (int c = 0; c < 4; ++c) acc[108 + c] += ds[u][c];
        }
    }
    __syncthreads();
    const int Cout = g.Cout, O = 27 * Cout;
    small_wgrad_epilogue<NACC>(acc, nchunk, sm, a.slab + (int64_t)blockIdx.x * (O + Cout), [=](int ch, int i) {
        if (i < 108) return (ch * 4 + i % 4) * 27 + i / 4;
        return O + ch * 4 + (i - 108);
    });
}

template <typename T> __device__ __forceinline__ void load_chunk16(const SrcDesc& src, bool plain, int64_t v, int c0, bool ok, float (&x)[16],
                                                                  const float* ss = nullptr, int Cin = 0) {
    if constexpr (sizeof(T) == 2) {
        if (plain || ss) {
            uint4 r0 = make_uint4(0, 0, 0, 0), r1 = r0;
            if (ok) {
                const uint4* q = (const uint4*)((const bf16*)src.ptr + v * src.C + c0);
                r0 = q[0]; r1 = q[1];
            }
            const unsigned w[8] = {r0.x, r0.y, r0.z, r0.w, r1.x, r1.y, r1.z, r1.w};
#pragma unroll
            for (int k = 0; k < 8; ++k) { x[2 * k] = __uint_as_float(w[k] << 16); x[2 * k + 1] = __uint_as_float(w[k] & 0xffff0000u); }
            if (!plain) {
#pragma unroll
                for (int k4 = 0; k4 < 4; ++k4) {
                    const float4 sc = *(const float4*)(ss + c0 + 4 * k4), sh = *(const float4*)(ss + Cin + c0 + 4 * k4);
                    x[4 * k4] = act_f(x[4 * k4] * sc.x + sh.x, src.act); x[4 * k4 + 1] = act_f(x[4 * k4 + 1] * sc.y + sh.y, src.act);
                    x[4 * k4 + 2] = act_f(x[4 * k4 + 2] * sc.z + sh.z, src.act); x[4 * k4 + 3] = act_f(x[4 * k4 + 3] * sc.w + sh.w, src.act);
                }
                if (!ok) {
#pragma unroll
                    for (int k = 0; k < 16; ++k) x[k] = 0.f;
                }
            }
            return;
        }
    }
#pragma unroll
    for (int k = 0; k < 16; ++k) x[k] = ok ? view_ld<T>(src, v, c0 + k) : 0.f;
}
template <typename T> __device__ __forceinline__ const float* stage_view(const SrcDesc& src, float* sm_after_filter, int Cin) {
    if (sizeof(T) != 2 || !src.scale) return nullptr;
    for (int i = threadIdx.x; i < Cin; i += 256) { sm_after_filter[i] = src.scale[i]; sm_after_filter[Cin + i] = src.shift[i]; }
    return sm_after_filter;
}

struct HeadArgs {
    SrcDesc src;
    const float* w;
    const float* bias;
    int Cin, Cout, lc;
    int64_t S;
    void* y;
    float* out;
    const float* dy_planes;
    const void* dy_cl;
    DstGrad dst;
    float* slab;
};

template <typename T, int CO> __global__ void __launch_bounds__(256) k_head_fwd(HeadArgs a) {
    extern __shared__ float sm[];
    for (int i = threadIdx.x; i < CO * a.Cin; i += 256) sm[i] = i < a.Cout * a.Cin ? a.w[i] : 0.f;
    const float* ss = stage_view<T>(a.src, sm + CO * a.Cin, a.Cin);
    __syncthreads();
    const int nchunk = 1 << a.lc, chunk = threadIdx.x & (nchunk - 1), c0 = chunk * 16;
    const int64_t vstride = ((int64_t)gridDim.x * 256) >> a.lc;
    const bool plain = !a.src.scale && a.src.act == 0;
    float b[CO];
#pragma unroll
    for (int c = 0; c < CO; ++c) b[c] = (a.bias && c < a.Cout) ? a.bias[c] : 0.f;
    for (int64_t v0 = ((int64_t)blockIdx.x * 256 + threadIdx.x) >> a.lc; v0 < ((a.S + 63) & ~(int64_t)63); v0 += vstride) {
        const bool ok = v0 < a.S;
        float x[16], o[CO];
        load_chunk16<T>(a.src, plain, v0, c0, ok, x, ss, a.Cin);
#pragma unroll
        for (int c = 0; c < CO; ++c) {
            const float4* wr = (const float4*)(sm + c * a.Cin + c0);
            float r = 0.f;
#pragma unroll
            for (int k4 = 0; k4 < 4; ++k4) {
                const float4 w4 = wr[k4];
                r = fmaf(x[4 * k4], w4.x, r); r = fmaf(x[4 * k4 + 1], w4.y, r); r = fmaf(x[4 * k4 + 2], w4.z, r); r = fmaf(x[4 * k4 + 3], w4.w, r);
            }
            for (int m = 1; m < nchunk; m <<= 1) r += __shfl_xor(r, m);
            o[c] = r + b[c];
        }
        if (ok && chunk == 0) {
#pragma unroll
            for (int c = 0; c < CO; ++c) {
                if (c < a.Cout) {
                    if (a.out) a.out[(int64_t)c * a.S + v0] = o[c];
                    if (a.y) st<T>((T*)a.y, v0 * a.Cout + c, o[c]);
                }
            }
        }
    }
}

template <typename T, int CO> __global__ void __launch_bounds__(256) k_head_bwd(HeadArgs a) {
    extern __shared__ float sm[];
    constexpr int NACC = CO * 16 + CO;
    for (int i = threadIdx.x; i < CO * a.Cin; i += 256) sm[i] = i < a.Cout * a.Cin ? a.w[i] : 0.f;
    const float* ss = stage_view<T>(a.src, sm + CO * a.Cin, a.Cin);
    __syncthreads();
    const int nchunk = 1 << a.lc, chunk = threadIdx.x & (nchunk - 1), c0 = chunk * 16;
    const int64_t vstride = ((int64_t)gridDim.x * 256) >> a.lc;
    const bool plain = !a.src.scale && a.src.act == 0;
    float acc[NACC];
#pragma unroll
    for (int i = 0; i < NACC; ++i) acc[i] = 0.f;
    auto fetch = [&](int64_t v, float (&xo)[16], float (&dout)[CO]) {
        load_chunk16<T>(a.src, plain, v, c0, true, xo, ss, a.Cin);
#pragma unroll
        for (int c = 0; c < CO; ++c) {
            dout[c] = 0.f;
            if (c < a.Cout) dout[c] = a.dy_planes ? a.dy_planes[(int64_t)c * a.S + v] : ld<T>((const T*)a.dy_cl, v * a.Cout + c);
        }
    };
    float xn[16], dn[CO];
    int64_t v0 = ((int64_t)blockIdx.x * 256 + threadIdx.x) >> a.lc;
    if (v0 < a.S) fetch(v0, xn, dn);
    for (; v0 < a.S; v0 += vstride) {
        float x[16], d[CO];
#pragma unroll
        for (int k = 0; k < 16; ++k) x[k] = xn[k];
#pragma unroll
        for (int c = 0; c < CO; ++c) d[c] = dn[c];
        if (v0 + vstride < a.S) fetch(v0 + vstride, xn, dn);
        if (a.slab) {
#pragma unroll
            for (int c = 0; c < CO; ++c) {
#pragma unroll
                for (int k = 0; k < 16; ++k) acc[c * 16 + k] = fmaf(d[c], x[k], acc[c * 16 + k]);
                acc[CO * 16 + c] += d[c];
            }
        }
        if (a.dst.ptr) {
            float g[16];
#pragma unroll
            for (int k = 0; k < 16; ++k) g[k] = 0.f;
#pragma unroll
            for (int c = 0; c < CO; ++c) {
                const float4* wr = (const float4*)(sm + c * a.Cin + c0);
#pragma unroll
                for (int k4 = 0; k4 < 4; ++k4) {
                    const float4 w4 = wr[k4];
                    g[4 * k4] = fmaf(d[c], w4.x, g[4 * k4]); g[4 * k4 + 1] = fmaf(d[c], w4.y, g[4 * k4 + 1]);
                    g[4 * k4 + 2] = fmaf(d[c], w4.z, g[4 * k4 + 2]); g[4 * k4 + 3] = fmaf(d[c], w4.w, g[4 * k4 + 3]);
                }
            }
            if constexpr (sizeof(T) == 2) {
                uint4* q = (uint4*)((bf16*)a.dst.ptr + v0 * a.dst.C + c0);
                if (a.dst.accumulate) {
                    const uint4 r0 = q[0], r1 = q[1];
                    const unsigned w[8] = {r0.x, r0.y, r0.z, r0.w, r1.x, r1.y, r1.z, r1.w};
#pragma unroll
                    for (int k = 0; k < 8; ++k) { g[2 * k] += __uint_as_float(w[k] << 16); g[2 * k + 1] += __uint_as_float(w[k] & 0xffff0000u); }
                }
                unsigned pk[8];
#pragma unroll
                for (int k = 0; k < 8; ++k) {
                    const bf16 lo = __float2bfloat16(g[2 * k]), hi = __float2bfloat16(g[2 * k + 1]);
                    pk[k] = (unsigned)__builtin_bit_cast(unsigned short, lo) | ((unsigned)__builtin_bit_cast(unsigned short, hi) << 16);
                }
                q[0] = make_uint4(pk[0], pk[1], pk[2], pk[3]); q[1] = make_uint4(pk[4], pk[5], pk[6], pk[7]);
            } else {
                float* q = (float*)a.dst.ptr + v0 * a.dst.C + c0;
#pragma unroll
                for (int k = 0; k < 16; ++k) q[k] = a.dst.accumulate ? q[k] + g[k] : g[k];
            }
        }
    }
    if (a.slab) {
        __syncthreads();
        const int Cin = a.Cin, Cout = a.Cout, O = Cin * Cout;
        small_wgrad_epilogue<NACC>(acc, nchunk, sm, a.slab + (int64_t)blockIdx.x * (O + Cout), [=](int ch, int i) {
            if (i < CO * 16) { int c = i / 16, k = i % 16; return c < Cout ? c * Cin + ch * 16 + k : -1; }
            int c = i - CO * 16;
            return (ch == 0 && c < Cout) ? O + c : -1;
        });
    }
}

static int ilog2_exact(int v) { int l = 0; while ((1 << l) < v) ++l; return (1 << l) == v ? l : -1; }
static bool wgrad_head_ok(const ConvGeom& g, int nsrc) {
    return nsrc == 1 && g.ks == 1 && g.stride == 1 && g.Cout <= 8 && g.Cin % 16 == 0 && ilog2_exact(g.Cin / 16) >= 0 && g.Cin <= 256;
}
static bool wgrad_first_ok(const ConvGeom& g, int nsrc) {
    return nsrc == 1 && g.ks == 3 && g.stride == 1 && g.Cin == 1 && g.Cout % 4 == 0 && ilog2_exact(g.Cout / 4) >= 0 && g.Cout <= 64 &&
           g.W % 4 == 0 && g.W <= 256;
}
static int wgrad_reg_blocks(int64_t items4) { int64_t nb = (items4 + 1023) / 1024; return nb < 1 ? 1 : (nb > 512 ? 512 : (int)nb); }
static bool wgrad_rows_ok(const ConvGeom& g) {
    int k3 = g.ks * g.ks * g.ks;
    int WI = (g.Wo - 1) * g.stride + g.ks;
    size_t lds = ((size_t)g.ks * g.ks * WI * g.Cin + (size_t)g.Wo * g.Cout) * 4;
    return (int64_t)k3 * g.Cin * g.Cout <= 1024 && lds <= 48 * 1024;
}

static int wgrad_small_blocks(const ConvGeom& g) { int rows = g.Do * g.Ho; return rows < 1024 ? rows : 1024; }
bool wgrad_small_supported(const ConvGeom& g, int nsrc) { return wgrad_head_ok(g, nsrc) || wgrad_first_ok(g, nsrc) || wgrad_rows_ok(g); }
size_t wgrad_small_scratch_bytes(const ConvGeom& g) {
    int k3 = g.ks * g.ks * g.ks;
    int64_t So = (int64_t)g.Do * g.Ho * g.Wo;
    size_t O = (size_t)k3 * g.Cin * g.Cout;
    size_t rows = (size_t)wgrad_small_blocks(g) * O * 4 + bias_grad_scratch_bytes(g.Cout, So) + 256;
    size_t regs = (size_t)512 * (O + g.Cout) * 4 + 256;
    return rows > regs ? rows : regs;
}
void launch_conv_wgrad_small(int dtype, const ConvGeom& g, const SrcDesc* src, int nsrc, const void* dy, float* dw, float* db,
                             void* scratch, hipStream_t s) {
    const int k3 = g.ks * g.ks * g.ks;
    const int64_t O = (int64_t)k3 * g.Cin * g.Cout;
    const bool head = wgrad_head_ok(g, nsrc), first = !head && wgrad_first_ok(g, nsrc);
    if (head || first) {
        WgradRegArgs a;
        a.g = g; a.src = src[0]; a.dy = dy; a.slab = (float*)scratch;
        const int64_t S = (int64_t)g.D * g.H * g.W;
        int nb;
        if (head) {
            a.lc = ilog2_exact(g.Cin / 16);
            nb = wgrad_reg_blocks((S << a.lc) * 4);
            const int CO = g.Cout <= 2 ? 2 : g.Cout <= 4 ? 4 : g.Cout <= 6 ? 6 : 8;
            const size_t lds = small_wgrad_lds_bytes(CO * 17, 1 << a.lc);
            switch (CO) {
                case 2: UNET_DISPATCH(dtype, (k_wgrad_head<T, 2><<<nb, 256, lds, s>>>(a))); break;
                case 4: UNET_DISPATCH(dtype, (k_wgrad_head<T, 4><<<nb, 256, lds, s>>>(a))); break;
                case 6: UNET_DISPATCH(dtype, (k_wgrad_head<T, 6><<<nb, 256, lds, s>>>(a))); break;
                default: UNET_DISPATCH(dtype, (k_wgrad_head<T, 8><<<nb, 256, lds, s>>>(a))); break;
            }
        } else {
            a.lc = ilog2_exact(g.Cout / 4);
            const int tiles = g.D * ((g.H + FIRST_TY - 1) / FIRST_TY);
            nb = tiles < 512 ? tiles : 512;
            const size_t l0 = (size_t)3 * (FIRST_TY + 2) * ((g.W + 5) & ~3) * 4, l1 = small_wgrad_lds_bytes(112, 1 << a.lc);
            const size_t lds = l0 > l1 ? l0 : l1;
            UNET_DISPATCH(dtype, (k_wgrad_first<T><<<nb, 256, lds, s>>>(a)));
        }
        slab_reduce2(a.slab, nb, O + g.Cout, dw, O, db, s);
        return;
    }
    WgradSmallArgs a;
    a.g = g; a.nsrc = nsrc; a.src[0] = src[0]; if (nsrc > 1) a.src[1] = src[1];
    a.dy = dy; a.slab = (float*)scratch;
    int nb = wgrad_small_blocks(g);
    int WI = (g.Wo - 1) * g.stride + g.ks;
    size_t lds = ((size_t)g.ks * g.ks * WI * g.Cin + (size_t)g.Wo * g.Cout) * 4;
    UNET_DISPATCH(dtype, (k_wgrad_small<T><<<nb, 256, lds, s>>>(a)));
    slab_reduce(a.slab, nb, O, dw, s);
    if (db) launch_bias_grad(dtype, dy, g.Cout, (int64_t)g.Do * g.Ho * g.Wo, db, (float*)scratch + (size_t)nb * O, s);
}

bool head_supported(const ConvGeom& g, int nsrc) { return wgrad_head_ok(g, nsrc); }
size_t head_bwd_scratch_bytes(const ConvGeom& g) { return (size_t)512 * ((size_t)g.Cin * g.Cout + g.Cout) * 4 + 256; }
template <typename T> static void head_launch(bool bwd, int CO, int nb, size_t lds, const HeadArgs& a, hipStream_t s) {
    switch (CO) {
        case 2: if (bwd) k_head_bwd<T, 2><<<nb, 256, lds, s>>>(a); else k_head_fwd<T, 2><<<nb, 256, lds, s>>>(a); break;
        case 4: if (bwd) k_head_bwd<T, 4><<<nb, 256, lds, s>>>(a); else k_head_fwd<T, 4><<<nb, 256, lds, s>>>(a); break;
        case 6: if (bwd) k_head_bwd<T, 6><<<nb, 256, lds, s>>>(a); else k_head_fwd<T, 6><<<nb, 256, lds, s>>>(a); break;
        default: if (bwd) k_head_bwd<T, 8><<<nb, 256, lds, s>>>(a); else k_head_fwd<T, 8><<<nb, 256, lds, s>>>(a); break;
    }
}
static int head_co(int Cout) { return Cout <= 2 ? 2 : Cout <= 4 ? 4 : Cout <= 6 ? 6 : 8; }
void launch_head_fwd(int dtype, const ConvGeom& g, const SrcDesc& src, const float* w, const float* bias, void* y, float* out_ncdhw,
                     hipStream_t s) {
    HeadArgs a = {};
    a.src = src; a.w = w; a.bias = bias; a.Cin = g.Cin; a.Cout = g.Cout; a.lc = ilog2_exact(g.Cin / 16);
    a.S = (int64_t)g.D * g.H * g.W; a.y = y; a.out = out_ncdhw;
    const int CO = head_co(g.Cout);
    int64_t items = ((a.S + 63) & ~(int64_t)63) << a.lc;
    int64_t nb = (items + 255) / 256;
    if (nb > 2048) nb = 2048;
    UNET_DISPATCH(dtype, (head_launch<T>(false, CO, (int)nb, (size_t)(CO + 2) * g.Cin * 4, a, s)));
}
void launch_head_bwd(int dtype, const ConvGeom& g, const SrcDesc& src, const float* dy_ncdhw, const void* dy_cl, const float* w,
                     DstGrad dst, float* dw, float* db, void* scratch, hipStream_t s, bool defer_reduce) {
    HeadArgs a = {};
    a.src = src; a.w = w; a.Cin = g.Cin; a.Cout = g.Cout; a.lc = ilog2_exact(g.Cin / 16);
    a.S = (int64_t)g.D * g.H * g.W; a.dy_planes = dy_ncdhw; a.dy_cl = dy_cl; a.dst = dst;
    a.slab = dw ? (float*)scratch : nullptr;
    const int CO = head_co(g.Cout);
    const int nb = wgrad_reg_blocks((a.S << a.lc) * 4);
    const size_t l0 = (size_t)(CO + 2) * g.Cin * 4, l1 = small_wgrad_lds_bytes(CO * 17, 1 << a.lc);
    UNET_DISPATCH(dtype, (head_launch<T>(true, CO, nb, l0 > l1 ? l0 : l1, a, s)));
    if (dw && !defer_reduce) slab_reduce2(a.slab, nb, (int64_t)g.Cin * g.Cout + g.Cout, dw, (int64_t)g.Cin * g.Cout, db, s);
}
void launch_head_bwd_reduce(const ConvGeom& g, float* dw, float* db, const void* scratch, hipStream_t s) {
    const int lc = ilog2_exact(g.Cin / 16);
    const int nb = wgrad_reg_blocks((((int64_t)g.D * g.H * g.W) << lc) * 4);
    slab_reduce2((const float*)scratch, nb, (int64_t)g.Cin * g.Cout + g.Cout, dw, (int64_t)g.Cin * g.Cout, db, s);
}

}
```

### unet-studio_amd/csrc/kernels_elem.hip

```cpp
#include "device_util.h"

namespace unet {

template <typename T> __global__ void k_pack_input(const float* __restrict__ x, T* __restrict__ y, int C, int64_t S) {
    int64_t i = (int64_t)blockIdx.x * 256 + threadIdx.x;
    if (i >= S * C) return;
    int c = (int)(i % C); int64_t v = i / C;
    st<T>(y, i, x[(int64_t)c * S + v]);
}
void launch_pack_input(int dtype, const float* x, void* y, int C, int64_t S, hipStream_t s) {
    UNET_DISPATCH(dtype, (k_pack_input<T><<<cdiv64(S * C, 256), 256, 0, s>>>(x, (T*)y, C, S)));
}

template <typename T> __global__ void k_export(SrcDesc src, float* __restrict__ y, int64_t S) {
    int64_t i = (int64_t)blockIdx.x * 256 + threadIdx.x;
    if (i >= S * src.C) return;
    int c = (int)(i / S); int64_t v = i % S;
    y[i] = view_ld<T>(src, v, c);
}
void launch_export(int dtype, SrcDesc src, float* y, int64_t S, hipStream_t s) {
    UNET_DISPATCH(dtype, (k_export<T><<<cdiv64(S * src.C, 256), 256, 0, s>>>(src, y, S)));
}
void launch_unpack_ncdhw(int dtype, const void* g, float* out, int C, int64_t S, hipStream_t s) {
    SrcDesc d;
    d.ptr = g; d.C = C;
    launch_export(dtype, d, out, S, s);
}

template <typename T> __global__ void k_import_grad(const float* __restrict__ g, T* __restrict__ o, int C, int64_t S, int acc) {
    int64_t i = (int64_t)blockIdx.x * 256 + threadIdx.x;
    if (i >= S * C) return;
    int c = (int)(i % C); int64_t v = i / C;
    float val = g[(int64_t)c * S + v];
    if (acc) val += ld<T>(o, i);
    st<T>(o, i, val);
}
void launch_import_grad(int dtype, const float* g, void* o, int C, int64_t S, int accumulate, hipStream_t s) {
    UNET_DISPATCH(dtype, (k_import_grad<T><<<cdiv64(S * C, 256), 256, 0, s>>>(g, (T*)o, C, S, accumulate)));
}
void launch_export_bwd(int dtype, const float* g, DstGrad dst, int64_t S, hipStream_t s) {
    if (!dst.ptr) return;
    launch_import_grad(dtype, g, dst.ptr, dst.C, S, dst.accumulate, s);
}

static inline int64_t stats_vpb(int64_t S) {
    int64_t vpb = (S + 1023) / 1024;
    return vpb < 32 ? 32 : vpb;
}
int stats_blocks(int64_t S) {
    int64_t vpb = stats_vpb(S);
    return (int)((S + vpb - 1) / vpb);
}
static inline int pow2_ge(int c) { int p = 1; while (p < c && p < 256) p <<= 1; return p; }

template <typename T> struct StatAcc { typedef float type; };
template <> struct StatAcc<float> { typedef double type; };

template <typename T, int MODE>
__global__ void __launch_bounds__(256) k_stats_partial(const T* __restrict__ x, T* __restrict__ gbuf, int C, int64_t S, int64_t VPB,
                                                       int CW, const float* __restrict__ stat, int act, float* __restrict__ partial_) {
    typedef typename StatAcc<T>::type A;
    A* partial = (A*)partial_;
    __shared__ A red[2][256];
    int NV = 256 / CW, cl = threadIdx.x % CW, lane = threadIdx.x / CW;
    int64_t v0 = (int64_t)blockIdx.x * VPB, v1 = v0 + VPB < S ? v0 + VPB : S;
    for (int cg = 0; cg < C; cg += CW) {
        int c = cg + cl;
        A s1 = 0, s2 = 0;
        if (c < C) {
            float mean = 0.f, rstd = 1.f, sc = 1.f, sh = 0.f;
            if (MODE == 1) { mean = stat[c]; rstd = stat[C + c]; sc = stat[2 * C + c]; sh = stat[3 * C + c]; }
            for (int64_t v = v0 + lane; v < v1; v += NV) {
                float u = ld<T>(x, v * C + c);
                if (MODE == 0) { s1 += (A)u; s2 += (A)u * (A)u; }
                else {
                    float dv = ld<T>(gbuf, v * C + c) * act_d(fmaf(u, sc, sh), act);
                    s1 += (A)dv; s2 += (A)dv * (A)((u - mean) * rstd);
                }
            }
        }
        red[0][threadIdx.x] = s1; red[1][threadIdx.x] = s2;
        __syncthreads();
        if (lane == 0 && c < C) {
// ... 572 lines not shown
        out[v * G8 + grp] = make_uint4(w[0], w[1], w[2], w[3]);
    }
}
static inline bool fused_norm_ok(int dtype, int C, int nblk) {
    return dtype == 1 && C % 8 == 0 && C <= FUSED_MAX_C && 256 % (C / 8) == 0 && nblk <= FUSED_MAX_ROWS;
}
static inline int64_t fused_vpb(int C, int64_t S) {
    const int64_t nv = 256 / (C / 8);
    int64_t vpb = (S + 255) / 256;
    if (vpb < 2 * nv) vpb = 2 * nv;
    return (vpb + nv - 1) / nv * nv;
}
bool launch_norm_finalize_apply(int dtype, const float* partial, int nblk, int C, int64_t S, const float* gamma, const float* beta, double eps,
                                float* stat, float* rm, float* rv, double momentum, const void* raw, int act, void* out, hipStream_t s) {
    if (!fused_norm_ok(dtype, C, nblk)) return false;
    const int64_t vpb = fused_vpb(C, S);
    k_norm_finalize_apply8<<<cdiv64(S, vpb), 256, 0, s>>>(partial, nblk, C, S, vpb, gamma, beta, eps, stat, rm, rv, momentum,
                                                          (const uint4*)raw, act, (uint4*)out);
    return true;
}

void launch_materialize(int dtype, const SrcDesc* src, int nsrc, void* out, int64_t S, hipStream_t s) {
    Src2 a;
    a.n = nsrc; a.s[0] = src[0]; if (nsrc > 1) a.s[1] = src[1];
    int C = src[0].C + (nsrc > 1 ? src[1].C : 0);
    UNET_DISPATCH(dtype, (k_materialize<T><<<cdiv64(S * C, 256), 256, 0, s>>>(a, (T*)out, C, S * C)));
}
template <typename T> __global__ void k_materialize_bwd(const T* __restrict__ gout, Dst2 dst, int C, int64_t n) {
    int64_t i = (int64_t)blockIdx.x * 256 + threadIdx.x;
    if (i >= n) return;
    int c = (int)(i % C); int64_t v = i / C;
    int which = (dst.n > 1 && c >= dst.d[0].C) ? 1 : 0;
    const DstGrad& d = dst.d[which];
    if (!d.ptr) return;
    int64_t j = v * d.C + (which ? c - dst.d[0].C : c);
    float val = ld<T>(gout, i);
    T* p = (T*)d.ptr;
    if (d.accumulate) val += ld<T>(p, j);
    st<T>(p, j, val);
}
void launch_materialize_bwd(int dtype, const void* gout, const DstGrad* dst, int ndst, int64_t S, hipStream_t s) {
    Dst2 a;
    a.n = ndst; a.d[0] = dst[0]; if (ndst > 1) a.d[1] = dst[1];
    int C = dst[0].C + (ndst > 1 ? dst[1].C : 0);
    UNET_DISPATCH(dtype, (k_materialize_bwd<T><<<cdiv64(S * C, 256), 256, 0, s>>>((const T*)gout, a, C, S * C)));
}

__global__ void k_target_half(const int64_t* __restrict__ t, int64_t* __restrict__ o, int D, int H, int W) {
    int Do = D >> 1, Ho = H >> 1, Wo = W >> 1;
    int64_t i = (int64_t)blockIdx.x * 256 + threadIdx.x;
    if (i >= (int64_t)Do * Ho * Wo) return;
    int x = (int)(i % Wo); int64_t r = i / Wo;
    int y = (int)(r % Ho); int z = (int)(r / Ho);
    float sd = (float)D / Do, sh = (float)H / Ho, sw = (float)W / Wo;
    int iz = min((int)floorf(z * sd), D - 1), iy = min((int)floorf(y * sh), H - 1), ix = min((int)floorf(x * sw), W - 1);
    o[i] = (int64_t)(float)t[((int64_t)iz * H + iy) * W + ix];
}
void launch_target_half(const int64_t* t, int64_t* o, int D, int H, int W, hipStream_t s) {
    int64_t n = (int64_t)(D >> 1) * (H >> 1) * (W >> 1);
    k_target_half<<<cdiv64(n, 256), 256, 0, s>>>(t, o, D, H, W);
}

int loss_blocks(int64_t S) {
    int64_t nb = (S + 255) / 256;
    return (int)(nb > 1024 ? 1024 : nb);
}

struct VoxelLogits {
    const float* p; int64_t S, v; int k; float lse0;
    __device__ float get(int cp) const { return (k && cp == 0) ? lse0 : p[(int64_t)(k ? cp + k - 1 : cp) * S + v]; }
};
__device__ __forceinline__ VoxelLogits make_vl(const float* logits, int64_t S, int64_t v, int k) {
    VoxelLogits L;
    L.p = logits; L.S = S; L.v = v; L.k = k; L.lse0 = 0.f;
    if (k) {
        float mx = -INFINITY;
        for (int c = 0; c < k; ++c) mx = fmaxf(mx, logits[(int64_t)c * S + v]);
        float s = 0.f;
        for (int c = 0; c < k; ++c) s += __expf(logits[(int64_t)c * S + v] - mx);
        L.lse0 = mx + __logf(s);
    }
    return L;
}
__device__ __forceinline__ float clamp_p(float q) { return fminf(fmaxf(q, 1e-6f), 1.0f - 1e-6f); }

__global__ void __launch_bounds__(256) k_loss_partial(const float* __restrict__ logits, const int64_t* __restrict__ target, int C,
                                                      int64_t S, int k, float* __restrict__ partial) {
    extern __shared__ float sh[];
    int oc = k ? C - k + 1 : C;
    int np = 3 + 2 * oc;
    for (int i = threadIdx.x; i < np; i += 256) sh[i] = 0.f;
    __syncthreads();
    float ce = 0.f, mse = 0.f, nv = 0.f;
    for (int64_t v = (int64_t)blockIdx.x * 256 + threadIdx.x; v < S; v += (int64_t)gridDim.x * 256) {
        int64_t t = target[v];
        bool valid = t < C;
        if (!valid) continue;
        int tt = k ? (int)(t - k + 1 > 0 ? t - k + 1 : 0) : (int)t;
        VoxelLogits L = make_vl(logits, S, v, k);
        float mx = -INFINITY;
        for (int c = 0; c < oc; ++c) mx = fmaxf(mx, L.get(c));
        float sum = 0.f;
        for (int c = 0; c < oc; ++c) sum += __expf(L.get(c) - mx);
        float inv = 1.f / sum, psq = 0.f, pt = 0.f;
        for (int c = 0; c < oc; ++c) {
            float p = clamp_p(__expf(L.get(c) - mx) * inv);
            psq = fmaf(p, p, psq);
            if (c == tt) pt = p;
            if (c >= 1) atomicAdd(&sh[3 + oc + c], p + (c == tt ? 1.f : 0.f));
        }
        if (tt >= 1) atomicAdd(&sh[3 + tt], pt);
        ce += -(L.get(tt) - mx - __logf(sum));
        mse += psq - 2.f * pt + 1.f;
        nv += 1.f;
    }
    atomicAdd(&sh[0], ce); atomicAdd(&sh[1], mse); atomicAdd(&sh[2], nv);
    __syncthreads();
    for (int i = threadIdx.x; i < np; i += 256) partial[(int64_t)blockIdx.x * np + i] = sh[i];
}
template <int OCMAX>
__global__ void __launch_bounds__(256) k_loss_partial_reg(const float* __restrict__ logits, const int64_t* __restrict__ target, int C,
                                                          int64_t S, int k, float* __restrict__ partial) {
    constexpr int RS = 3 + 2 * OCMAX + 1;
    __shared__ float red[4 * RS];
    const int oc = k ? C - k + 1 : C, np = 3 + 2 * oc;
    float ce = 0.f, mse = 0.f, nv = 0.f, inter[OCMAX], card[OCMAX];
#pragma unroll
    for (int c = 0; c < OCMAX; ++c) { inter[c] = 0.f; card[c] = 0.f; }
    for (int64_t v = (int64_t)blockIdx.x * 256 + threadIdx.x; v < S; v += (int64_t)gridDim.x * 256) {
        int64_t t = target[v];
        if (!(t < C)) continue;
        int tt = k ? (int)(t - k + 1 > 0 ? t - k + 1 : 0) : (int)t;
        VoxelLogits L = make_vl(logits, S, v, k);
        float lg[OCMAX], mx = -INFINITY;
#pragma unroll
        for (int c = 0; c < OCMAX; ++c) { lg[c] = c < oc ? L.get(c) : -INFINITY; mx = fmaxf(mx, lg[c]); }
        float sum = 0.f;
#pragma unroll
        for (int c = 0; c < OCMAX; ++c) { lg[c] = c < oc ? __expf(lg[c] - mx) : 0.f; sum += lg[c]; }
        float inv = 1.f / sum, psq = 0.f, pt = 0.f, lt = 0.f;
#pragma unroll
        for (int c = 0; c < OCMAX; ++c) {
            if (c < oc) {
                float p = clamp_p(lg[c] * inv);
                psq = fmaf(p, p, psq);
                bool hit = c == tt;
                if (hit) { pt = p; lt = L.get(c); inter[c] += p; }
                card[c] += p + (hit ? 1.f : 0.f);
            }
        }
        ce += -(lt - mx - __logf(sum));
        mse += psq - 2.f * pt + 1.f;
        nv += 1.f;
    }
    auto wsum = [](float v) { for (int o = 32; o > 0; o >>= 1) v += __shfl_xor(v, o); return v; };
    const int lane = threadIdx.x & 63, wave = threadIdx.x >> 6;
    float w3[3] = {wsum(ce), wsum(mse), wsum(nv)};
    if (lane == 0) { red[wave * RS + 0] = w3[0]; red[wave * RS + 1] = w3[1]; red[wave * RS + 2] = w3[2]; }
#pragma unroll
    for (int c = 0; c < OCMAX; ++c) {
        if (c < oc) {
            const float a = wsum(inter[c]), b = wsum(card[c]);
            if (lane == 0) { red[wave * RS + 3 + c] = a; red[wave * RS + 3 + oc + c] = b; }
        }
    }
    __syncthreads();
    if ((int)threadIdx.x < np)
// ... 87 lines not shown
    __syncthreads();
    if (threadIdx.x == 0) {
        double n = shd[2] < 1.0 ? 1.0 : shd[2];
        double eps = (double)1e-5f, dsum = 0.0;
        for (int c = 1; c < oc; ++c) dsum += (2.0 * shd[3 + c] + eps) / (shd[3 + oc + c] + eps);
        double ce = shd[0] / n, mse = shd[1] / n, dice = 1.0 - dsum / (double)(oc - 1 > 1 ? oc - 1 : 1);
        level_out[0] = (float)ce; level_out[1] = (float)dice; level_out[2] = (float)mse; level_out[3] = (float)n;
        for (int c = 0; c < oc; ++c) { level_out[4 + c] = (float)shd[3 + c]; level_out[4 + oc + c] = (float)shd[3 + oc + c]; }
        double sel = 0.0;
        if (!(cost_mask & 7)) sel = ce;
        else sel = ((cost_mask & 1) ? ce : 0.0) + ((cost_mask & 2) ? dice : 0.0) + ((cost_mask & 4) ? mse : 0.0);
        totals[0] += (float)(weight * sel);
        if (set_stats) { totals[1] = (float)ce; totals[2] = (float)dice; totals[3] = (float)mse; }
    }
}
void launch_loss_finalize(const float* partial, int nblk, int oc, float weight, int cost_mask, float* level_out, float* totals,
                          int set_stats, hipStream_t s) {
    k_loss_finalize<<<1, 3 + 2 * oc > 8 ? 1024 : 512, (3 + 2 * oc) * sizeof(double), s>>>(partial, nblk, oc, weight, cost_mask, level_out, totals, set_stats);
}

__global__ void __launch_bounds__(256) k_loss_grad(const float* __restrict__ logits, const int64_t* __restrict__ target, int C, int64_t S,
                                                   int k, const float* __restrict__ level_out, float weight, int cost_mask,
                                                   float* __restrict__ dlogits) {
    int oc = k ? C - k + 1 : C;
    int64_t v = (int64_t)blockIdx.x * 256 + threadIdx.x;
    if (v >= S) return;
    int64_t t = target[v];
    if (!(t < C)) {
        for (int c = 0; c < C; ++c) dlogits[(int64_t)c * S + v] = 0.f;
        return;
    }
    float w_ce = (!(cost_mask & 7) || (cost_mask & 1)) ? weight : 0.f;
    float w_dice = (cost_mask & 2) ? weight : 0.f, w_mse = (cost_mask & 4) ? weight : 0.f;
    float n = level_out[3];
    const float* inter = level_out + 4;
    const float* card = level_out + 4 + oc;
    float dden = (float)(oc - 1 > 1 ? oc - 1 : 1), eps = 1e-5f;
    int tt = k ? (int)(t - k + 1 > 0 ? t - k + 1 : 0) : (int)t;
    VoxelLogits L = make_vl(logits, S, v, k);
    float mx = -INFINITY;
    for (int c = 0; c < oc; ++c) mx = fmaxf(mx, L.get(c));
    float sum = 0.f;
    for (int c = 0; c < oc; ++c) sum += __expf(L.get(c) - mx);
    float inv = 1.f / sum;
    float dot = 0.f;
    for (int c = 0; c < oc; ++c) {
        float q = __expf(L.get(c) - mx) * inv, p = clamp_p(q), g = 0.f;
        g += w_mse * (2.f * p - (c == tt ? 2.f : 0.f)) / n;
        if (c >= 1) {
            float m = c == tt ? 1.f : 0.f, den = card[c] + eps;
            g += w_dice * (-(2.f * m * den - (2.f * inter[c] + eps)) / (den * den)) / dden;
        }
        if (!(q >= 1e-6f && q <= 1.0f - 1e-6f)) g = 0.f;
        dot = fmaf(g, q, dot);
    }
    float d0 = 0.f;
    for (int c = 0; c < oc; ++c) {
        float q = __expf(L.get(c) - mx) * inv, p = clamp_p(q), g = 0.f;
        g += w_mse * (2.f * p - (c == tt ? 2.f : 0.f)) / n;
        if (c >= 1) {
            float m = c == tt ? 1.f : 0.f, den = card[c] + eps;
            g += w_dice * (-(2.f * m * den - (2.f * inter[c] + eps)) / (den * den)) / dden;
        }
        if (!(q >= 1e-6f && q <= 1.0f - 1e-6f)) g = 0.f;
        float dl = q * (g - dot) + w_ce * (q - (c == tt ? 1.f : 0.f)) / n;
        if (k && c == 0) d0 = dl;
        else dlogits[(int64_t)(k ? c + k - 1 : c) * S + v] = dl;
    }
    if (k) {
        float m0 = -INFINITY;
        for (int c = 0; c < k; ++c) m0 = fmaxf(m0, logits[(int64_t)c * S + v]);
        float s0 = 0.f;
        for (int c = 0; c < k; ++c) s0 += __expf(logits[(int64_t)c * S + v] - m0);
        for (int c = 0; c < k; ++c) dlogits[(int64_t)c * S + v] = d0 * __expf(logits[(int64_t)c * S + v] - m0) / s0;
    }
}
template <int OCMAX>
__global__ void __launch_bounds__(256) k_loss_grad_v4(const float* __restrict__ logits, const int64_t* __restrict__ target, int C, int64_t S,
                                                      const float* __restrict__ level_out, float weight, int cost_mask,
                                                      float* __restrict__ dlogits) {
    const int oc = C;
    const int64_t q4 = (int64_t)blockIdx.x * 256 + threadIdx.x;
    if (q4 >= (S >> 2)) return;
    const float w_ce = (!(cost_mask & 7) || (cost_mask & 1)) ? weight : 0.f;
    const float w_dice = (cost_mask & 2) ? weight : 0.f, w_mse = (cost_mask & 4) ? weight : 0.f;
    const float n = level_out[3];
    const float dden = (float)(oc - 1 > 1 ? oc - 1 : 1), eps = 1e-5f;
    float dice_hit[OCMAX], dice_miss[OCMAX];
#pragma unroll
    for (int c = 0; c < OCMAX; ++c) {
        dice_hit[c] = dice_miss[c] = 0.f;
        if (c >= 1 && c < oc) {
            const float den = level_out[4 + oc + c] + eps, in2 = 2.f * level_out[4 + c] + eps;
            dice_hit[c] = w_dice * (-(2.f * 1.f * den - in2) / (den * den)) / dden;
            dice_miss[c] = w_dice * (-(2.f * 0.f * den - in2) / (den * den)) / dden;
        }
    }
    const longlong2 t01 = ((const longlong2*)target)[2 * q4], t23 = ((const longlong2*)target)[2 * q4 + 1];
    const int64_t tv[4] = {t01.x, t01.y, t23.x, t23.y};
    float4 pl[OCMAX];
#pragma unroll
    for (int c = 0; c < OCMAX; ++c)
        pl[c] = c < oc ? ((const float4*)(logits + (int64_t)c * S))[q4] : make_float4(-INFINITY, -INFINITY, -INFINITY, -INFINITY);
    float out[OCMAX][4];
#pragma unroll
    for (int j = 0; j < 4; ++j) {
        const int64_t t = tv[j];
        const bool valid = t < C;
        const int tt = (int)t;
        float lg[OCMAX], mx = -INFINITY;
#pragma unroll
        for (int c = 0; c < OCMAX; ++c) { lg[c] = j == 0 ? pl[c].x : j == 1 ? pl[c].y : j == 2 ? pl[c].z : pl[c].w; mx = fmaxf(mx, lg[c]); }
        float sum = 0.f;
#pragma unroll
        for (int c = 0; c < OCMAX; ++c) { lg[c] = c < oc ? __expf(lg[c] - mx) : 0.f; sum += lg[c]; }
        const float inv = 1.f / sum;
        float g[OCMAX], dot = 0.f;
#pragma unroll
        for (int c = 0; c < OCMAX; ++c) {
            g[c] = 0.f;
            if (c < oc) {
                const float q = lg[c] * inv, p = clamp_p(q);
                float gg = 0.f;
                gg += w_mse * (2.f * p - (c == tt ? 2.f : 0.f)) / n;
                if (c >= 1) gg += c == tt ? dice_hit[c] : dice_miss[c];
                if (!(q >= 1e-6f && q <= 1.0f - 1e-6f)) gg = 0.f;
                dot = fmaf(gg, q, dot);
                g[c] = gg; lg[c] = q;
            }
        }
#pragma unroll
        for (int c = 0; c < OCMAX; ++c)
            out[c][j] = (c < oc && valid) ? lg[c] * (g[c] - dot) + w_ce * (lg[c] - (c == tt ? 1.f : 0.f)) / n : 0.f;
    }
#pragma unroll
    for (int c = 0; c < OCMAX; ++c)
        if (c < oc) ((float4*)(dlogits + (int64_t)c * S))[q4] = make_float4(out[c][0], out[c][1], out[c][2], out[c][3]);
}
void launch_loss_grad(const float* logits, const int64_t* target, int C, int64_t S, int collapse, const float* level_out, float weight,
                      int cost_mask, float* dlogits, hipStream_t s) {
    if (loss_v4_ok(logits, target, dlogits, C, S, collapse)) {
        k_loss_grad_v4<8><<<cdiv64(S >> 2, 256), 256, 0, s>>>(logits, target, C, S, level_out, weight, cost_mask, dlogits);
        return;
    }
    k_loss_grad<<<cdiv64(S, 256), 256, 0, s>>>(logits, target, C, S, collapse, level_out, weight, cost_mask, dlogits);
}

struct SumBufs { const float* in[UNET_SUM_MAX_BUFFERS]; int n; };
__global__ void __launch_bounds__(256) k_sum_buffers(SumBufs b, float* __restrict__ out, int64_t count, int zero_inputs) {
    for (int64_t i0 = ((int64_t)blockIdx.x * 256 + threadIdx.x) * 4; i0 < count; i0 += (int64_t)gridDim.x * 1024) {
        if (i0 + 3 < count) {
            float4 acc = *(const float4*)(b.in[0] + i0);
            for (int k = 1; k < b.n; ++k) {
                const float4 v = *(const float4*)(b.in[k] + i0);
                acc.x += v.x; acc.y += v.y; acc.z += v.z; acc.w += v.w;
            }
            *(float4*)(out + i0) = acc;
            if (zero_inputs)
                for (int k = 0; k < b.n; ++k)
                    if (b.in[k] != out) *(float4*)(const_cast<float*>(b.in[k]) + i0) = make_float4(0.f, 0.f, 0.f, 0.f);
        } else {
            for (int j = 0; j < 4 && i0 + j < count; ++j) {
                float acc = b.in[0][i0 + j];
                for (int k = 1; k < b.n; ++k) acc += b.in[k][i0 + j];
                out[i0 + j] = acc;
                if (zero_inputs)
                    for (int k = 0; k < b.n; ++k)
                        if (b.in[k] != out) const_cast<float*>(b.in[k])[i0 + j] = 0.f;
            }
        }
    }
}
void launch_sum_buffers(const float* const* bufs, int n, float* out, int64_t count, int zero_inputs, hipStream_t s) {
    SumBufs b;
    b.n = n;
    for (int k = 0; k < UNET_SUM_MAX_BUFFERS; ++k) b.in[k] = k < n ? bufs[k] : nullptr;
    int64_t nb = (count + 1023) / 1024;
    if (nb > 4096) nb = 4096;
    k_sum_buffers<<<(unsigned)nb, 256, 0, s>>>(b, out, count, zero_inputs);
}

__global__ void __launch_bounds__(256) k_sumsq_partial(const float* __restrict__ g, int64_t n, float scale, float* __restrict__ partial) {
    __shared__ double red[256];
    double acc = 0.0;
    for (int64_t i0 = ((int64_t)blockIdx.x * 256 + threadIdx.x) * 4; i0 < n; i0 += (int64_t)gridDim.x * 1024) {
        float r = 0.f;
        if (i0 + 3 < n) {
            const float4 v = *(const float4*)(g + i0);
            const float a0 = v.x * scale, a1 = v.y * scale, a2 = v.z * scale, a3 = v.w * scale;
            r = fmaf(a0, a0, fmaf(a1, a1, fmaf(a2, a2, a3 * a3)));
        } else {
            for (int j = 0; j < 4; ++j)
                if (i0 + j < n) { float x = g[i0 + j] * scale; r = fmaf(x, x, r); }
        }
        acc += (double)r;
    }
    red[threadIdx.x] = acc;
    __syncthreads();
    for (int o = 128; o > 0; o >>= 1) {
        if ((int)threadIdx.x < o) red[threadIdx.x] += red[threadIdx.x + o];
        __syncthreads();
    }
    if (threadIdx.x == 0) partial[blockIdx.x] = (float)red[0];
}
void launch_sumsq_partial(const float* g, int64_t n, float scale, float* partial, int nblk, hipStream_t s) {
    k_sumsq_partial<<<nblk, 256, 0, s>>>(g, n, scale, partial);
}

constexpr int SGD_MAXSEG = 1024;
__global__ void __launch_bounds__(256) k_sgd(float* __restrict__ p, float* __restrict__ g, float* __restrict__ m, int64_t n,
                                             const SgdSeg* __restrict__ segs, int nseg, const float* __restrict__ partial, int nblk,
                                             float lr, float momentum, int nesterov, float wdecay, float clip_norm, float grad_scale, float* norm_out) {
    __shared__ double red[256];
    __shared__ float s_coef;
    __shared__ int64_t s_off[SGD_MAXSEG];
    __shared__ float s_wd[SGD_MAXSEG];
// ... 63 lines not shown
```

### unet-studio_amd/csrc/unet_host.cpp

```cpp
#include "../../include/unet.hpp"
#include "../../include/unet_hip.h"

#include <c10/hip/HIPStream.h>
#include <hip/hip_runtime_api.h>

#include <functional>
#include <sstream>
#include <thread>

namespace {

void check(int rc) { if (rc) throw std::runtime_error(unet_last_error()); }

void* stream_of(const torch::Device& d) {
    return d.is_cuda() ? (void*)c10::hip::getCurrentHIPStream(d.index()).stream() : nullptr;
}

struct Holder : torch::nn::Module {};

}

struct UNet3dImpl::WorkspacePool {
    struct Entry { torch::Tensor buf; hipEvent_t ev = nullptr; };
    static constexpr size_t MAX_IDLE = 4;
// ... 183 lines not shown
{
    auto dev = device();
    std::shared_ptr<WorkspacePool> pool;
    {
        std::scoped_lock<std::mutex> lock(plans_mutex_);
        if (!ws_pool_) ws_pool_ = std::make_shared<WorkspacePool>();
        pool = ws_pool_;
    }
    WorkspacePool::Entry e;
    {
        std::scoped_lock<std::mutex> lock(pool->m);
        auto& v = pool->idle[plan];
        if (!v.empty()) { e = v.back(); v.pop_back(); }
    }
    c10::DeviceGuard guard(dev);
    void* const lease_stream = stream_of(dev);
    if (e.buf.defined()) {
        if (e.ev) (void)hipStreamWaitEvent((hipStream_t)lease_stream, e.ev, 0);
    } else {
        size_t bytes = 0;
        unet_plan_workspace_bytes(plan, &bytes);
        e.buf = torch::empty({(int64_t)bytes}, torch::TensorOptions().dtype(torch::kUInt8).device(dev));
        if (dev.is_cuda() && hipEventCreateWithFlags(&e.ev, hipEventDisableTiming) != hipSuccess) e.ev = nullptr;
    }
    std::weak_ptr<WorkspacePool> wp = pool;
    auto back = [wp, e, plan, dev, lease_stream](void*) mutable {
        auto p = wp.lock();
        if (e.ev && dev.is_cuda()) {
            c10::DeviceGuard g(dev);
            (void)hipEventRecord(e.ev, (hipStream_t)lease_stream);
        }
        if (p) {
            std::scoped_lock<std::mutex> lock(p->m);
            auto& v = p->idle[plan];
            if (v.size() < WorkspacePool::MAX_IDLE) { v.push_back(e); return; }
        }
        if (e.ev) (void)hipEventDestroy(e.ev);
    };
    return torch::from_blob(e.buf.data_ptr(), e.buf.sizes(), back, e.buf.options());
}

std::vector<torch::Tensor> UNet3dImpl::run_forward(unet_plan* plan, torch::Tensor ws, torch::Tensor x, int mode)
{
    std::vector<const float*> pp;
    for (auto& p : params_) pp.push_back(p.data_ptr<float>());
    std::vector<float*> bp;
    for (auto& b : buffers_) bp.push_back(b.data_ptr<float>());
    int nl = 0;
    unet_plan_output_count(plan, &nl);
    std::vector<torch::Tensor> outs(nl);
    std::vector<float*> op(nl, nullptr);
    for (int l = 0; l < nl; ++l) {
        int64_t d[5];
        unet_plan_output_shape(plan, l, d);
        if (d[1]) {
            outs[l] = torch::empty({d[0], d[1], d[2], d[3], d[4]}, torch::TensorOptions().dtype(torch::kFloat32).device(x.device()));
            op[l] = outs[l].data_ptr<float>();
        }
    }
    check(unet_forward(plan, pp.data(), bp.empty() ? nullptr : bp.data(), x.data_ptr<float>(), op.data(), ws.data_ptr(), mode,
                       stream_of(x.device())));
    return outs;
}

void UNet3dImpl::run_backward(unet_plan* plan, torch::Tensor ws, const std::vector<torch::Tensor>& grad_outs)
{
    rebind_grads();
    std::vector<const float*> pp, go;
    std::vector<float*> gp;
    std::vector<torch::Tensor> keep;
    int64_t off = 0;
    for (auto& p : params_) {
        pp.push_back(p.data_ptr<float>());
        gp.push_back(flat_grads.data_ptr<float>() + off);
        off += p.numel();
    }
    for (auto& t : grad_outs) {
        if (t.defined()) { keep.push_back(t.contiguous()); go.push_back(keep.back().data_ptr<float>()); }
        else go.push_back(nullptr);
    }
    check(unet_backward(plan, pp.data(), go.data(), gp.data(), nullptr, ws.data_ptr(), stream_of(flat_params.device())));
}

struct UNetForwardFn : torch::autograd::Function<UNetForwardFn> {
    static torch::autograd::variable_list forward(torch::autograd::AutogradContext* ctx, torch::Tensor x, torch::Tensor trigger,
                                                  int64_t self, int64_t plan, torch::Tensor ws) {
        (void)trigger;
        auto* m = reinterpret_cast<UNet3dImpl*>(self);
        auto outs = m->run_forward(reinterpret_cast<unet_plan*>(plan), ws, x, 1);
        ctx->saved_data["self"] = self;
        ctx->saved_data["plan"] = plan;
        ctx->saved_data["ws"] = ws;
        return outs;
    }
    static torch::autograd::variable_list backward(torch::autograd::AutogradContext* ctx, torch::autograd::variable_list grads) {
        auto* m = reinterpret_cast<UNet3dImpl*>(ctx->saved_data["self"].toInt());
        m->run_backward(reinterpret_cast<unet_plan*>(ctx->saved_data["plan"].toInt()), ctx->saved_data["ws"].toTensor(), grads);
        return {torch::Tensor(), torch::Tensor(), torch::Tensor(), torch::Tensor(), torch::Tensor()};
    }
};

std::vector<torch::Tensor> UNet3dImpl::forward(torch::Tensor inputTensor)
{
    if (inputTensor.dim() != 5 || inputTensor.size(0) != 1 || inputTensor.size(1) != in_count)
        throw std::runtime_error("UNet3d::forward expects a {1,in_count,D,H,W} tensor");
    ensure_flat();
    if (inputTensor.device() != device())
        throw std::runtime_error("UNet3d::forward: input and model are on different devices");
    auto x = inputTensor.to(torch::kFloat32).contiguous();
    unet_plan* plan = plan_for(x.size(2), x.size(3), x.size(4));
    auto ws = workspace_for(plan);
    if (is_training() && torch::GradMode::is_enabled())
        return UNetForwardFn::apply(x, trigger_, reinterpret_cast<int64_t>(this), reinterpret_cast<int64_t>(plan), ws);
    return run_forward(plan, ws, x, is_training() ? 1 : 0);
}

void UNet3dImpl::prepare_for_inference(const torch::Device& device)
{
    to_device(device);
    eval();
    for (size_t i = 0; i + 1 < buffers_.size(); i += 2) {
        buffers_[i].zero_();
        buffers_[i + 1].fill_(1.0f);
    }
}

void UNet3dImpl::copy_from(const UNet3dImpl& r)
{
    torch::NoGradGuard no_grad;
    ensure_flat();
    const_cast<UNet3dImpl&>(r).ensure_flat();
    if (flat_params.sizes() == r.flat_params.sizes())
        flat_params.copy_(r.flat_params);
    else {
        auto rhs = r.parameters(), lhs = parameters();
        for (size_t i = 0; i < rhs.size() && i < lhs.size(); ++i)
            if (lhs[i].sizes() == rhs[i].sizes()) lhs[i].copy_(rhs[i]);
    }
    for (size_t i = 0; i < r.buffers_.size() && i < buffers_.size(); ++i)
        if (buffers_[i].sizes() == r.buffers_[i].sizes()) buffers_[i].copy_(r.buffers_[i]);
    voxel_size = r.voxel_size;
    dim = r.dim;
    fov_strategy = r.fov_strategy;
    postproc = r.postproc;
    preproc = r.preproc;
}

void UNet3dImpl::add_gradient_from(const UNet3dImpl& r)
{
    torch::NoGradGuard no_grad;
    ensure_flat();
    rebind_grads();
    const_cast<UNet3dImpl&>(r).ensure_flat();
    const_cast<UNet3dImpl&>(r).rebind_grads();
    flat_grads.add_(r.flat_grads.to(flat_grads.device()).to(torch::kFloat32));
}

void UNet3dImpl::create_optimizer(float learning_rate)
{
    std::vector<torch::Tensor> decay_params, no_decay_params;
    for (auto& p : named_parameters()) {
        auto v = p.value();
        const auto& name = p.key();
        bool no_decay = name.find("bias") != std::string::npos || v.dim() <= 1;
        (no_decay ? no_decay_params : decay_params).push_back(v);
    }
    std::vector<torch::optim::OptimizerParamGroup> groups;
    auto opt_d = std::make_unique<torch::optim::SGDOptions>(learning_rate);
    opt_d->momentum(0.99); opt_d->nesterov(true); opt_d->weight_decay(3e-5);
    auto opt_nd = std::make_unique<torch::optim::SGDOptions>(learning_rate);
    opt_nd->momentum(0.99); opt_nd->nesterov(true); opt_nd->weight_decay(0.0);
    groups.push_back(torch::optim::OptimizerParamGroup(decay_params, std::move(opt_d)));
    groups.push_back(torch::optim::OptimizerParamGroup(no_decay_params, std::move(opt_nd)));
    optimizer = std::make_shared<torch::optim::SGD>(groups, torch::optim::SGDOptions(learning_rate));
}

std::string UNet3dImpl::get_info(void) const
{
    std::ostringstream out;
    out << "in: " << in_count << " out: " << out_count << std::endl;
    out << "dim: " << dim << " reso: " << voxel_size << std::endl;
    out << "structure: " << architecture << std::endl;
    if (!preproc.empty()) out << "preproc: " << preproc << std::endl;
    if (!postproc.empty()) out << "postproc: " << postproc << std::endl;
    return out.str();
}

void UNet3dImpl::print_layers(void)
{
    for (auto& p : named_parameters()) std::cout << p.key() << " " << p.value().sizes() << std::endl;
}

torch::Tensor UNet3dImpl::loss_and_backward(torch::Tensor input, torch::Tensor target, bool ce, bool dice, bool mse, int collapse_before)
{
    ensure_flat();
    auto x = input.to(torch::kFloat32).contiguous();
    unet_plan* plan = plan_for(x.size(2), x.size(3), x.size(4));
    auto ws = workspace_for(plan);
    auto outs = run_forward(plan, ws, x, 1);
    size_t sb = 0;
    unet_loss_scratch_bytes(plan, &sb);
    auto sc = torch::empty({(int64_t)sb}, torch::TensorOptions().dtype(torch::kUInt8).device(x.device()));
    auto losses = torch::empty({4}, torch::TensorOptions().dtype(torch::kFloat32).device(x.device()));
    std::vector<torch::Tensor> gouts;
    std::vector<const float*> op;
    std::vector<float*> gp;
    for (auto& o : outs) {
        gouts.push_back(o.defined() ? torch::empty_like(o) : torch::Tensor());
        op.push_back(o.defined() ? o.data_ptr<float>() : nullptr);
        gp.push_back(o.defined() ? gouts.back().data_ptr<float>() : nullptr);
    }
    auto t = target.to(torch::kLong).contiguous();
    int mask = (ce ? 1 : 0) | (dice ? 2 : 0) | (mse ? 4 : 0);
    check(unet_loss(plan, op.data(), t.data_ptr<int64_t>(), mask, collapse_before, gp.data(), losses.data_ptr<float>(), sc.data_ptr(),
                    stream_of(x.device())));
    run_backward(plan, ws, gouts);
    return losses;
}

void UNet3dImpl::broadcast_parameters(int root)
{
    if (!comm_) throw std::runtime_error("broadcast_parameters: no communicator attached");
    ensure_flat();
    void* st = stream_of(flat_params.device());
    check(unet_comm_broadcast(comm_, flat_params.data_ptr<float>(), flat_params.numel(), root, st));
    for (auto& b : buffers_) check(unet_comm_broadcast(comm_, b.data_ptr<float>(), b.numel(), root, st));
    check(unet_comm_join(comm_, st));
}

void UNet3dImpl::broadcast_buffers(int root)
{
    if (!comm_) throw std::runtime_error("broadcast_buffers: no communicator attached");
    if (buffers_.empty()) return;
    ensure_flat();
    void* st = stream_of(flat_params.device());
    for (auto& b : buffers_) check(unet_comm_broadcast(comm_, b.data_ptr<float>(), b.numel(), root, st));
    check(unet_comm_join(comm_, st));
}

void UNet3dImpl::allreduce_gradients(void)
{
    if (!comm_) throw std::runtime_error("allreduce_gradients: no communicator attached");
    ensure_flat();
    rebind_grads();
    void* st = stream_of(flat_grads.device());
    const int64_t hi = reduced_from_ >= 0 ? reduced_from_ : flat_grads.numel();
    check(unet_allreduce_grads(comm_, flat_grads.data_ptr<float>(), 0, hi, st));
    for (auto& b : buffers_) check(unet_comm_broadcast(comm_, b.data_ptr<float>(), b.numel(), 0, st));
    check(unet_comm_join(comm_, st));
    reduced_from_ = -1;
}

torch::Tensor UNet3dImpl::loss_and_backward_overlapped(torch::Tensor input, torch::Tensor target, bool ce, bool dice, bool mse, int collapse_before)
{
    if (!comm_) return loss_and_backward(input, target, ce, dice, mse, collapse_before);
    ensure_flat();
    rebind_grads();
    auto x = input.to(torch::kFloat32).contiguous();
    unet_plan* plan = plan_for(x.size(2), x.size(3), x.size(4));
    auto ws = workspace_for(plan);
    auto outs = run_forward(plan, ws, x, 1);
    size_t sb = 0;
    unet_loss_scratch_bytes(plan, &sb);
    auto sc = torch::empty({(int64_t)sb}, torch::TensorOptions().dtype(torch::kUInt8).device(x.device()));
    auto losses = torch::empty({4}, torch::TensorOptions().dtype(torch::kFloat32).device(x.device()));
    std::vector<torch::Tensor> gouts;
    std::vector<const float*> op, go;
    std::vector<float*> gp;
    for (auto& o : outs) {
        gouts.push_back(o.defined() ? torch::empty_like(o) : torch::Tensor());
        op.push_back(o.defined() ? o.data_ptr<float>() : nullptr);
        gp.push_back(o.defined() ? gouts.back().data_ptr<float>() : nullptr);
        go.push_back(gp.back());
    }
    auto t = target.to(torch::kLong).contiguous();
    int mask = (ce ? 1 : 0) | (dice ? 2 : 0) | (mse ? 4 : 0);
    void* st = stream_of(x.device());
    check(unet_loss(plan, op.data(), t.data_ptr<int64_t>(), mask, collapse_before, gp.data(), losses.data_ptr<float>(), sc.data_ptr(), st));
    std::vector<const float*> pp;
    std::vector<float*> gw;
    int64_t off = 0;
    for (auto& p : params_) { pp.push_back(p.data_ptr<float>()); gw.push_back(flat_grads.data_ptr<float>() + off); off += p.numel(); }
    int nb = 0, op_lo[8];
    int64_t elem_lo[8];
    check(unet_plan_backward_buckets(plan, 3, &nb, op_lo, elem_lo));
    int op_hi = 1 << 30;
    int64_t elem_hi = flat_grads.numel();
    for (int k = 0; k < nb; ++k) {
        check(unet_backward_part(plan, pp.data(), go.data(), gw.data(), nullptr, ws.data_ptr(), op_hi, op_lo[k], st));
        if (k + 1 < nb) {
            check(unet_allreduce_grads(comm_, flat_grads.data_ptr<float>(), elem_lo[k], elem_hi, st));
            reduced_from_ = elem_lo[k];
        }
        op_hi = op_lo[k]; elem_hi = elem_lo[k];
    }
    return losses;
}

void UNet3dImpl::bind_optimizer_state(void)
{
    ensure_flat();
    if (!momentum_.defined() || momentum_.device() != flat_params.device() || momentum_.numel() != flat_params.numel())
        momentum_ = momentum_.defined() && momentum_.numel() == flat_params.numel() ? momentum_.to(flat_params.device()) : torch::zeros_like(flat_params);
    if (!optimizer) return;
    torch::NoGradGuard ng;
    auto& st = optimizer->state();
    auto opts = torch::TensorOptions().dtype(torch::kFloat32).device(momentum_.device());
    int64_t off = 0;
    for (auto& p : params_) {
        float* slot = momentum_.data_ptr<float>() + off;
        off += p.numel();
        void* key = p.unsafeGetTensorImpl();
        auto it = st.find(key);
        if (it == st.end()) {
            auto ps = std::make_unique<torch::optim::SGDParamState>();
            ps->momentum_buffer(torch::from_blob(slot, p.sizes(), opts));
            st[key] = std::move(ps);
            continue;
        }
        auto& ps = static_cast<torch::optim::SGDParamState&>(*it->second);
        if (ps.momentum_buffer().defined() && ps.momentum_buffer().data_ptr() == (void*)slot) continue;
        auto alias = torch::from_blob(slot, p.sizes(), opts);
        if (ps.momentum_buffer().defined()) alias.copy_(ps.momentum_buffer().reshape(p.sizes()));
        ps.momentum_buffer(alias);
    }
}

bool UNet3dImpl::save_optimizer(const std::string& file_name)
{
    try {
        if (!optimizer) throw std::runtime_error("save_optimizer: no optimizer (create_optimizer first)");
        bind_optimizer_state();
        torch::save(*optimizer, file_name);
        return true;
    } catch (const std::exception& e) { error_msg = std::string("cannot save optimizer: ") + e.what(); return false; }
}

bool UNet3dImpl::load_optimizer(const std::string& file_name)
{
    try {
        if (!optimizer) throw std::runtime_error("load_optimizer: no optimizer (create_optimizer first)");
        torch::load(*optimizer, file_name);
        bind_optimizer_state();
        return true;
    } catch (const std::exception& e) { error_msg = std::string("cannot load optimizer: ") + e.what(); return false; }
}

void UNet3dImpl::sgd_step(float lr, float grad_scale, float clip_norm)
{
    ensure_flat();
    rebind_grads();
    bind_optimizer_state();
    if (!scratch_.defined()) scratch_ = torch::empty({65536 + 16}, torch::TensorOptions().dtype(torch::kUInt8).device(flat_params.device()));
    if (plans_.empty()) throw std::runtime_error("sgd_step before any forward");
    check(unet_sgd_step(plans_.begin()->second, flat_params.data_ptr<float>(), flat_grads.data_ptr<float>(), momentum_.data_ptr<float>(), lr,
                        0.99f, 1, 3e-5f, clip_norm, grad_scale, (float*)((char*)scratch_.data_ptr() + 65536), scratch_.data_ptr(),
                        stream_of(flat_params.device())));
}
```

### unet-studio_amd/engine.py

```python
import ctypes as C
import os

_HERE = os.path.dirname(os.path.abspath(__file__))
LIB_PATH = os.environ.get("UNET_HIP_LIBRARY") or os.path.join(_HERE, "libunet_hip.so")

DTYPE_F32, DTYPE_BF16 = 0, 1
IMPL_AUTO, IMPL_DIRECT = 0, 1

if not os.path.exists(LIB_PATH):
    raise ImportError(
        "libunet_hip.so not found at %s: build it first (python -c 'import __graft_entry__ as g; g.build()' "
        "or unet-studio_amd/csrc/build.sh); there is no CPU fallback" % LIB_PATH)

import torch

lib = C.CDLL(LIB_PATH)

_vp, _i, _sz, _f = C.c_void_p, C.c_int, C.c_size_t, C.c_float
_pp = C.POINTER(C.c_void_p)


def _sig(name, res, *args):
    fn = getattr(lib, name)
    fn.restype = res
    fn.argtypes = list(args)
    return fn


_sig("unet_last_error", C.c_char_p)
_sig("unet_init", _i, C.POINTER(_i))
_sig("unet_device_info", _i, _i, C.c_char_p, _sz, C.POINTER(_sz), C.POINTER(_i), C.POINTER(_i))
_sig("unet_plan_create", _i, C.c_char_p, _i, _i, _i, _i, _i, _i, _i, _i, C.POINTER(_vp))
_sig("unet_plan_destroy", None, _vp)
_sig("unet_plan_param_count", _i, _vp, C.POINTER(_i))
_sig("unet_plan_param_shape", _i, _vp, _i, C.POINTER(C.c_int64), C.POINTER(_i))
_sig("unet_plan_param_name", _i, _vp, _i, C.c_char_p, _sz)
_sig("unet_plan_param_decay", _i, _vp, _i, C.POINTER(_i))
_sig("unet_plan_param_fan_in", _i, _vp, _i, C.POINTER(C.c_int64), C.POINTER(_i))
_sig("unet_plan_buffer_count", _i, _vp, C.POINTER(_i))
_sig("unet_plan_buffer_shape", _i, _vp, _i, C.POINTER(C.c_int64))
_sig("unet_plan_output_count", _i, _vp, C.POINTER(_i))
_sig("unet_plan_output_shape", _i, _vp, _i, C.POINTER(C.c_int64))
_sig("unet_plan_workspace_bytes", _i, _vp, C.POINTER(_sz))
_sig("unet_plan_flops", _i, _vp, C.POINTER(C.c_double), C.POINTER(C.c_double))
_sig("unet_plan_describe", _sz, _vp, C.c_char_p, _sz)
_sig("unet_plan_op_count", _i, _vp, C.POINTER(_i))
_sig("unet_plan_op_info", _i, _vp, _i, C.POINTER(_i), C.POINTER(_i), C.POINTER(_i), C.POINTER(_i), C.POINTER(_i), C.POINTER(C.c_int64),
     C.POINTER(C.c_int64), C.c_char_p, _sz)
_sig("unet_profile_begin", _i)
_sig("unet_profile_end", _i, _i, C.POINTER(_i), C.POINTER(_i), C.POINTER(_f), C.POINTER(_i))
_sig("unet_forward", _i, _vp, _pp, _pp, _vp, _pp, _vp, _i, _vp)
_sig("unet_backward", _i, _vp, _pp, _pp, _pp, _vp, _vp, _vp)
_sig("unet_backward_part", _i, _vp, _pp, _pp, _pp, _vp, _vp, _i, _i, _vp)
_sig("unet_plan_backward_buckets", _i, _vp, _i, C.POINTER(_i), C.POINTER(_i), C.POINTER(C.c_int64))
_sig("unet_loss_scratch_bytes", _i, _vp, C.POINTER(_sz))
_sig("unet_loss", _i, _vp, _pp, _vp, _i, _i, _pp, _vp, _vp, _vp)
_sig("unet_forward_loss", _i, _vp, _pp, _pp, _vp, _pp, _vp, _i, _i, _pp, _vp, _vp, _vp, _vp)
_sig("unet_forward_loss_mode", _i, _vp, _pp, _pp, _vp, _pp, _vp, _i, _i, _pp, _vp, _vp, _vp, _i, _vp)
_sig("unet_sum_buffers", _i, _pp, _i, _vp, C.c_int64, _i, _vp)
_sig("unet_stream_create_cu_range", _i, _i, _i, _i, _vp)
_sig("unet_stream_destroy", _i, _vp)
_sig("unet_plan_side_cu_range", _i, _vp, _i, _i)
_sig("unet_pack_filters", _i, _vp, _vp, _vp, _i, _vp, _vp)
_sig("unet_sgd_step", _i, _vp, _vp, _vp, _vp, _f, _f, _i, _f, _f, _f, _vp, _vp, _vp)
_sig("unet_set_error", None, C.c_char_p)
_sig("unet_comm_unique_id", _i, _vp)
_sig("unet_comm_create", _i, _i, _i, _vp, _i, C.POINTER(_vp))
_sig("unet_comm_create_all", _i, _i, C.POINTER(_i), C.POINTER(_vp))
_sig("unet_comm_destroy", _i, _vp)
_sig("unet_comm_rank", _i, _vp, C.POINTER(_i), C.POINTER(_i))
_sig("unet_allreduce_grads", _i, _vp, _vp, C.c_int64, C.c_int64, _vp)
_sig("unet_allreduce_grads_all", _i, _pp, _i, _pp, C.c_int64, C.c_int64, _pp)
_sig("unet_comm_broadcast", _i, _vp, _vp, C.c_int64, _i, _vp)
_sig("unet_comm_join", _i, _vp, _vp)
_sig("unet_op_scratch_bytes", _i, _i, _i, _i, _i, _i, C.POINTER(_sz))
_sig("unet_op_conv3d_fwd", _i, _i, _i, _vp, _vp, _vp, _vp, _i, _i, _i, _i, _i, _i, _i, _vp, _vp)
_sig("unet_op_conv3d_pack", _i, _i, _vp, _vp, _i, _i, _i, _i, _i, _i, _i, _vp)
_sig("unet_op_conv3d_fwd_packed", _i, _i, _vp, _vp, _vp, _vp, _vp, _i, _i, _i, _i, _i, _i, _i, _vp)
_sig("unet_op_conv3d_fwd_fused", _i, _i, _i, _vp, _vp, _vp, _i, _vp, _vp, _vp, _vp, _i, _i, _i, _i, _i, _i, _i, _vp, _vp)
_sig("unet_op_conv3d_bwd_data", _i, _i, _i, _vp, _vp, _vp, _i, _i, _i, _i, _i, _i, _i, _vp, _vp)
_sig("unet_op_conv3d_fwd_norm", _i, _vp, _vp, _i, _i, _vp, _vp, _vp, _vp, C.c_double, _vp, _vp, C.c_double, _i, _i, _vp, _vp, _vp,
     _i, _i, _i, _i, _i, _vp, _vp)
_sig("unet_op_conv3d_bwd_data_norm", _i, _i, _vp, _vp, _vp, _i, _vp, _vp, _vp, _i, _vp, _vp, _vp, _i, _i, _i, _i, _i, _vp, _vp)
_sig("unet_op_conv3d_bwd_weight", _i, _i, _i, _vp, _vp, _vp, _vp, _i, _i, _i, _i, _i, _i, _i, _vp, _vp)
_sig("unet_op_convt_fwd", _i, _i, _i, _vp, _vp, _vp, _vp, _i, _i, _i, _i, _i, _vp, _vp)
_sig("unet_op_convt_bwd_data", _i, _i, _i, _vp, _vp, _vp, _i, _i, _i, _i, _i, _vp, _vp)
_sig("unet_op_convt_bwd_weight", _i, _i, _i, _vp, _vp, _vp, _vp, _i, _i, _i, _i, _i, _vp, _vp)
_sig("unet_op_pack_ndhwc", _i, _i, _vp, _vp, _i, C.c_int64, _vp)
_sig("unet_op_unpack_ncdhw", _i, _i, _vp, _vp, _i, C.c_int64, _vp)

EXPORTS = [
    "unet_last_error", "unet_init", "unet_device_info", "unet_plan_create", "unet_plan_destroy", "unet_plan_param_count",
    "unet_plan_param_shape", "unet_plan_param_name", "unet_plan_param_decay", "unet_plan_param_fan_in", "unet_plan_buffer_count",
    "unet_plan_buffer_shape", "unet_plan_output_count", "unet_plan_output_shape", "unet_plan_workspace_bytes",
    "unet_plan_flops", "unet_plan_describe", "unet_plan_op_count", "unet_plan_op_info", "unet_profile_begin", "unet_profile_end", "unet_forward", "unet_backward", "unet_backward_part", "unet_plan_backward_buckets", "unet_loss_scratch_bytes", "unet_loss", "unet_forward_loss", "unet_forward_loss_mode", "unet_sum_buffers",
    "unet_sgd_step", "unet_pack_filters", "unet_stream_create_cu_range", "unet_stream_destroy", "unet_plan_side_cu_range", "unet_set_error", "unet_comm_unique_id", "unet_comm_create", "unet_comm_create_all", "unet_comm_destroy", "unet_comm_rank",
    "unet_allreduce_grads", "unet_allreduce_grads_all", "unet_comm_broadcast", "unet_comm_join", "unet_op_scratch_bytes", "unet_op_conv3d_fwd", "unet_op_conv3d_fwd_fused", "unet_op_conv3d_pack", "unet_op_conv3d_fwd_packed", "unet_op_conv3d_bwd_data", "unet_op_conv3d_fwd_norm", "unet_op_conv3d_bwd_data_norm", "unet_op_conv3d_bwd_weight",
    "unet_op_convt_fwd", "unet_op_convt_bwd_data", "unet_op_convt_bwd_weight", "unet_op_pack_ndhwc", "unet_op_unpack_ncdhw",
]


MODE_PACKS_CURRENT = 2


class UNetError(RuntimeError):
    """What the C++ host rethrows as std::runtime_error (unet.cpp:53,66,88,117)."""


def check(rc):
    if rc != 0:
        raise UNetError(lib.unet_last_error().decode("utf-8", "replace"))


def ptr_array(ptrs):
    arr = (C.c_void_p * max(1, len(ptrs)))()
    for i, p in enumerate(ptrs):
        arr[i] = p
    return arr


class Plan:

    def __init__(self, arch, in_c, out_c, size, dtype=DTYPE_BF16, device=0, impl=IMPL_AUTO):
        self.handle = C.c_void_p()
        self._pid = os.getpid()
        D, H, W = size
        check(lib.unet_plan_create(arch.encode(), in_c, out_c, D, H, W, dtype, device, impl, C.byref(self.handle)))
        self.arch, self.in_c, self.out_c, self.size, self.dtype, self.device = arch, in_c, out_c, (D, H, W), dtype, device
        n = C.c_int()
        check(lib.unet_plan_param_count(self.handle, C.byref(n)))
        self.param_shapes, self.param_decay, self.param_fan_in, self.param_is_norm_weight, self.param_names = [], [], [], [], []
        dims, nd, dec, fan, isn = (C.c_int64 * 5)(), C.c_int(), C.c_int(), C.c_int64(), C.c_int()
        for i in range(n.value):
            check(lib.unet_plan_param_shape(self.handle, i, dims, C.byref(nd)))
            self.param_shapes.append(tuple(dims[k] for k in range(nd.value)))
            nm = C.create_string_buffer(128)
            check(lib.unet_plan_param_name(self.handle, i, nm, 128))
            self.param_names.append(nm.value.decode())
            check(lib.unet_plan_param_decay(self.handle, i, C.byref(dec)))
            self.param_decay.append(bool(dec.value))
            check(lib.unet_plan_param_fan_in(self.handle, i, C.byref(fan), C.byref(isn)))
            self.param_fan_in.append(fan.value)
            self.param_is_norm_weight.append(bool(isn.value))
        check(lib.unet_plan_buffer_count(self.handle, C.byref(n)))
        self.buffer_numel = []
        ne = C.c_int64()
        for i in range(n.value):
            check(lib.unet_plan_buffer_shape(self.handle, i, C.byref(ne)))
            self.buffer_numel.append(ne.value)
        check(lib.unet_plan_output_count(self.handle, C.byref(n)))
        self.output_shapes = []
        for l in range(n.value):
            check(lib.unet_plan_output_shape(self.handle, l, dims))
            self.output_shapes.append(tuple(dims[k] for k in range(5)))
        b = C.c_size_t()
        check(lib.unet_plan_workspace_bytes(self.handle, C.byref(b)))
        self.workspace_bytes = b.value
        check(lib.unet_loss_scratch_bytes(self.handle, C.byref(b)))
        self.loss_scratch_bytes = b.value
        f, g = C.c_double(), C.c_double()
        check(lib.unet_plan_flops(self.handle, C.byref(f), C.byref(g)))
        self.flops_fwd, self.flops_bwd = f.value, g.value

    def backward_buckets(self, max_buckets=3):
        n = C.c_int()
        ops, el = (C.c_int * max_buckets)(), (C.c_int64 * max_buckets)()
        check(lib.unet_plan_backward_buckets(self.handle, max_buckets, C.byref(n), ops, el))
        return [(ops[k], el[k]) for k in range(n.value)]

    def ops(self):
        n = C.c_int()
        check(lib.unet_plan_op_count(self.handle, C.byref(n)))
        out = []
        k, ci, co, ks, st = C.c_int(), C.c_int(), C.c_int(), C.c_int(), C.c_int()
        di, do = (C.c_int64 * 3)(), (C.c_int64 * 3)()
        for i in range(n.value):
            nm = C.create_string_buffer(128)
            check(lib.unet_plan_op_info(self.handle, i, C.byref(k), C.byref(ci), C.byref(co), C.byref(ks), C.byref(st), di, do, nm, 128))
            out.append({"kind": k.value, "cin": ci.value, "cout": co.value, "ks": ks.value, "stride": st.value,
                        "in_dims": tuple(di), "out_dims": tuple(do), "name": nm.value.decode()})
        return out

    def describe(self):
        n = lib.unet_plan_describe(self.handle, None, 0)
        buf = C.create_string_buffer(n)
# ... 77 lines not shown
```

### unet-studio_amd/unet3d.py

```python
import math
import threading

import torch

from . import engine as E

_DT = {"fp32": E.DTYPE_F32, "f32": E.DTYPE_F32, "float32": E.DTYPE_F32, "bf16": E.DTYPE_BF16, "bfloat16": E.DTYPE_BF16}


_NO_FUSED_LOSS = False


def _stream_ptr(device):
    return torch.cuda.current_stream(device).cuda_stream


class SGD:

    def __init__(self, model, lr):
        self.model = model
        self.param_groups = [{"lr": lr, "weight_decay": 3e-5}, {"lr": lr, "weight_decay": 0.0}]
        self.momentum, self.nesterov, self.weight_decay = 0.99, True, 3e-5
        self.momentum_buffer = torch.zeros_like(model.flat_params)
        self.last_grad_norm = torch.zeros(1, device=model.flat_params.device, dtype=torch.float32)
# ... 173 lines not shown
                raise E.UNetError("load_optimizer: no optimizer (create_optimizer first)")
            self.optimizer.load_state_dict(torch.load(file_name, map_location="cpu"))
            return True
        except (OSError, RuntimeError, KeyError) as e:
            self.error_msg = "cannot load optimizer: %s" % e
            return False

    def prepare_for_inference(self, device=None):
        self.eval()
        for i in range(0, len(self._buffers), 2):
            self._buffers[i].zero_()
            self._buffers[i + 1].fill_(1.0)
        self.num_batches_tracked = 0

    def get_training_errors(self):
        with self.error_mutex:
            return list(self.training_errors)

    def get_testing_errors(self):
        with self.error_mutex:
            return list(self.testing_errors)

    def get_info(self):
        s = "in: %d out: %d\n" % (self.in_count, self.out_count)
        s += "dim: %s reso: %s\n" % (" ".join(str(d) for d in self.dim), " ".join(str(v) for v in self.voxel_size))
        s += "structure: %s\n" % self.architecture
        if self.preproc:
            s += "preproc: %s\n" % self.preproc
        if self.postproc:
            s += "postproc: %s\n" % self.postproc
        return s

    def print_layers(self):
        print(self._probe.describe())

    def plan_for(self, size):
        key = tuple(int(s) for s in size)
        p = self._plans.get(key)
        if p is None:
            p = E.Plan(self.architecture, self.in_count, self.out_count, key, self._dtype, self._device.index or 0, self._impl)
            self._plans[key] = p
        return p

    def _any_plan(self):
        return next(iter(self._plans.values())) if self._plans else self._probe

    def _workspace(self, plan):
        key = (plan.size, threading.get_ident())
        ws = self._workspaces.get(key)
        if ws is None:
            ws = torch.empty(plan.workspace_bytes, dtype=torch.uint8, device=self._device)
            self._workspaces[key] = ws
        return ws

    def _run_forward(self, plan, ws, x, mode):
        outs = [torch.empty(s, dtype=torch.float32, device=self._device) if s[1] > 0 else None for s in plan.output_shapes]
        pp, bp = self._pp, self._bp
        op = E.ptr_array([o.data_ptr() if o is not None else None for o in outs])
        E.check(E.lib.unet_forward(plan.handle, pp, bp, x.data_ptr(), op, ws.data_ptr(), mode, _stream_ptr(self._device)))
        if (mode & 1) and self._buffers:
            self.num_batches_tracked += 1
        return outs

    def pack_filters(self, size, with_dgrad=True):
        import ctypes
        plan = self.plan_for(tuple(size))
        ws = self._workspace(plan)
        made = ctypes.c_int(0)
        E.check(E.lib.unet_pack_filters(plan.handle, self._pp, ws.data_ptr(), 1 if with_dgrad else 0, ctypes.byref(made),
                                        _stream_ptr(self._device)))
        return bool(made.value)

    def _run_backward(self, plan, ws, grad_outs, grad_x=None, gp=None):
        pp, gp = self._pp, (gp if gp is not None else self._gp)
        go = E.ptr_array([g.data_ptr() if g is not None else None for g in grad_outs])
        E.check(E.lib.unet_backward(plan.handle, pp, go, gp, grad_x.data_ptr() if grad_x is not None else None,
                                    ws.data_ptr(), _stream_ptr(self._device)))

    def _run_backward_part(self, plan, ws, grad_outs, op_hi, op_lo):
        pp, gp = self._pp, self._gp
        go = E.ptr_array([g.data_ptr() if g is not None else None for g in grad_outs])
        E.check(E.lib.unet_backward_part(plan.handle, pp, go, gp, None, ws.data_ptr(), op_hi, op_lo, _stream_ptr(self._device)))

    def forward_backward_bucketed(self, x, target, on_bucket, cost_ce=True, cost_dice=True, cost_mse=True, collapse_before=0,
                                  max_buckets=3, packs_current=False, losses_out=None):
        x = self._check_input(x)
        plan = self.plan_for(x.shape[2:])
        ws = self._workspace(plan)
        outs, losses, gouts = self._run_forward_loss(plan, ws, x, target, cost_ce, cost_dice, cost_mse, collapse_before, packs_current,
                                                     losses_out=losses_out)
        op_hi, elem_hi = 1 << 30, int(self.flat_grads.numel())
        for op_lo, elem_lo in plan.backward_buckets(max_buckets):
            self._run_backward_part(plan, ws, gouts, op_hi, op_lo)
            on_bucket(int(elem_lo), elem_hi)
            op_hi, elem_hi = op_lo, int(elem_lo)
        return losses

    def grad_pointers(self, flat):
        assert flat.numel() == self.flat_grads.numel() and flat.dtype == torch.float32 and flat.device == self._device
        return E.ptr_array([flat.data_ptr() + 4 * self._offsets[i] for i in range(len(self._params))])

    def make_lane(self, size, cu_range=None):
        key = tuple(int(v) for v in size)
        plan = E.Plan(self.architecture, self.in_count, self.out_count, key, self._dtype, self._device.index or 0, self._impl)
        stream = torch.cuda.Stream(self._device)
        if cu_range is not None:
            import ctypes
            h = ctypes.c_void_p()
            E.check(E.lib.unet_stream_create_cu_range(self._device.index or 0, int(cu_range[0]), int(cu_range[1]), ctypes.byref(h)))
            stream = torch.cuda.ExternalStream(h.value, device=self._device)
            E.check(E.lib.unet_plan_side_cu_range(plan.handle, int(cu_range[0]), int(cu_range[1])))
        return {"plan": plan, "stream": stream,
                "ws": torch.empty(plan.workspace_bytes, dtype=torch.uint8, device=self._device),
                "loss": torch.empty(plan.loss_scratch_bytes, dtype=torch.uint8, device=self._device)}

    def forward_backward_lane(self, lane, x, target, gp, cost_ce=True, cost_dice=True, cost_mse=True, collapse_before=0, packs_current=False):
        x = self._check_input(x)
        plan, ws = lane["plan"], lane["ws"]
        outs, losses, gouts = self._run_forward_loss(plan, ws, x, target, cost_ce, cost_dice, cost_mse, collapse_before, packs_current,
                                                     loss_scratch=lane["loss"])
        self._run_backward(plan, ws, gouts, gp=gp)
        return losses

    def _check_input(self, x):
        if x.dim() != 5 or x.size(0) != 1 or x.size(1) != self.in_count:
            raise E.UNetError("forward expects a {1,%d,D,H,W} tensor, got %s" % (self.in_count, tuple(x.shape)))
        if x.device != self._device:
            raise E.UNetError("input is on %s, model is on %s" % (x.device, self._device))
        return x.to(torch.float32).contiguous()

    def forward(self, x, packs_current=False):
        x = self._check_input(x)
        plan = self.plan_for(x.shape[2:])
        ws = self._workspace(plan)
        if self._training and torch.is_grad_enabled():
            return list(_Forward.apply(x, self._trigger, self, plan, ws))
        return self._run_forward(plan, ws, x, mode=(1 if self._training else 0) | (E.MODE_PACKS_CURRENT if packs_current else 0))

    __call__ = forward

    def _forward_level0(self, x):
        x = self._check_input(x)
        plan = self.plan_for(x.shape[2:])
        ws = self._workspace(plan)
        shape = plan.output_shapes[0]
        if shape[1] == 0:
            return None
        out = torch.empty(shape, dtype=torch.float32, device=self._device)
        op = E.ptr_array([out.data_ptr()] + [None] * (len(plan.output_shapes) - 1))
        mode = 1 if self._training else 0
        E.check(E.lib.unet_forward(plan.handle, self._pp, self._bp, x.data_ptr(), op, ws.data_ptr(), mode, _stream_ptr(self._device)))
        if mode and self._buffers:
            self.num_batches_tracked += 1
        return out

    def forward_backward(self, x, target, cost_ce=True, cost_dice=True, cost_mse=True, collapse_before=0, packs_current=False, losses_out=None):
        x = self._check_input(x)
        plan = self.plan_for(x.shape[2:])
        ws = self._workspace(plan)
        outs, losses, gouts = self._run_forward_loss(plan, ws, x, target, cost_ce, cost_dice, cost_mse, collapse_before, packs_current,
                                                     losses_out=losses_out)
        self._run_backward(plan, ws, gouts)
        return losses

    def _loss_scratch(self, plan):
        key = ("loss", plan.size, threading.get_ident())
        sc = self._workspaces.get(key)
        if sc is None:
            sc = torch.empty(plan.loss_scratch_bytes, dtype=torch.uint8, device=self._device)
            self._workspaces[key] = sc
        return sc

    def _run_forward_loss(self, plan, ws, x, target, cost_ce, cost_dice, cost_mse, collapse_before, packs_current=False, loss_scratch=None,
                          losses_out=None):
        if target.dtype != torch.int64 or target.device != self._device:
            raise E.UNetError("target must be an int64 tensor on the model's device")
        target = target.contiguous()
        if any(s[1] == 0 for s in plan.output_shapes) or _NO_FUSED_LOSS:
            outs = self._run_forward(plan, ws, x, mode=1 | (E.MODE_PACKS_CURRENT if packs_current else 0))
            losses, gouts = self.loss(outs, target, cost_ce, cost_dice, cost_mse, collapse_before, plan=plan)
            if losses_out is not None:
                losses_out.copy_(losses)
                losses = losses_out
            return outs, losses, gouts
        outs = [torch.empty(s, dtype=torch.float32, device=self._device) for s in plan.output_shapes]
        gouts = [torch.empty_like(o) for o in outs]
        losses = losses_out if losses_out is not None else torch.empty(4, dtype=torch.float32, device=self._device)
        mask = (1 if cost_ce else 0) | (2 if cost_dice else 0) | (4 if cost_mse else 0)
        mode = 1 | (E.MODE_PACKS_CURRENT if packs_current else 0)
        E.check(E.lib.unet_forward_loss_mode(plan.handle, self._pp, self._bp, x.data_ptr(), E.ptr_array([o.data_ptr() for o in outs]),
                                             target.data_ptr(), mask, collapse_before, E.ptr_array([g.data_ptr() for g in gouts]),
                                             losses.data_ptr(), (loss_scratch if loss_scratch is not None else self._loss_scratch(plan)).data_ptr(),
                                             ws.data_ptr(), mode,
                                             _stream_ptr(self._device)))
        if self._buffers:
            self.num_batches_tracked += 1
        return outs, losses, gouts

    def loss(self, outs, target, cost_ce=True, cost_dice=True, cost_mse=True, collapse_before=0, want_grad=True, plan=None):
        if plan is None:
            plan = self.plan_for(outs[0].shape[2:])
        if target.dtype != torch.int64 or target.device != self._device:
            raise E.UNetError("target must be an int64 tensor on the model's device")
        target = target.contiguous()
        sc = self._loss_scratch(plan)
        gouts = [torch.empty_like(o) if (o is not None and want_grad) else None for o in outs]
        losses = torch.empty(4, dtype=torch.float32, device=self._device)
        mask = (1 if cost_ce else 0) | (2 if cost_dice else 0) | (4 if cost_mse else 0)
        E.check(E.lib.unet_loss(plan.handle, E.ptr_array([o.data_ptr() if o is not None else None for o in outs]),
                                target.data_ptr(), mask, collapse_before,
                                E.ptr_array([g.data_ptr() if g is not None else None for g in gouts]),
                                losses.data_ptr(), sc.data_ptr(), _stream_ptr(self._device)))
        return losses, gouts
```

Measured before the change: 797.9 million.

## Fuse loss gradient computation into head backward kernels

Skips writing the per-level loss gradient tensors in the forward+loss pass when the output head is a bf16 1x1 head with few classes. The head backward kernels instead recompute dlogits on the fly from the logits, the target labels and the finalized loss coefficients, for both the weight gradient and the source gradient (which also folds in the BN backward stats). This removes a full-resolution gradient write and read at the largest tensor sizes. In exchange it adds new kernels, extra partial scratch and a new API path, and the logits and target are read twice.

```diff
diff --git a/include/unet_hip.h b/include/unet_hip.h
--- a/include/unet_hip.h
+++ b/include/unet_hip.h
@@ -73,6 +73,14 @@
                            const int64_t* target, int cost_mask, int collapse_before, float* const* grad_outs, float* losses_out,
                            void* loss_scratch, void* workspace, int mode, void* stream);
 
+#define UNET_MODE_LOSS_BACKWARD 4
+int unet_backward_loss(const unet_plan* plan, const float* const* params, const float* const* grad_outs, const float* const* outs,
+                       const int64_t* target, int cost_mask, int collapse_before, void* loss_scratch, float* const* grad_params,
+                       float* grad_x, void* workspace, void* stream);
+int unet_backward_loss_part(const unet_plan* plan, const float* const* params, const float* const* grad_outs, const float* const* outs,
+                            const int64_t* target, int cost_mask, int collapse_before, void* loss_scratch, float* const* grad_params,
+                            float* grad_x, void* workspace, int op_hi, int op_lo, void* stream);
+
 int unet_stream_create_cu_range(int device, int cu_first, int cu_count, void** stream);
 int unet_stream_destroy(void* stream);
 int unet_plan_side_cu_range(unet_plan* plan, int cu_first, int cu_count);
diff --git a/unet-studio_amd/csrc/engine.cpp b/unet-studio_amd/csrc/engine.cpp
--- a/unet-studio_amd/csrc/engine.cpp
+++ b/unet-studio_amd/csrc/engine.cpp
@@ -45,6 +45,7 @@
 
 struct EnvSwitches {
     bool no_side_stream = getenv("UNET_NO_SIDE_STREAM"), no_first_wgrad_fuse = getenv("UNET_NO_FIRST_WGRAD_FUSE"), op_polite = getenv("UNET_OP_POLITE");
+    bool no_head_loss_fusion = getenv("UNET_NO_HEAD_LOSS_FUSION");
 };
 const EnvSwitches& env() { static const EnvSwitches e; return e; }
 
@@ -230,6 +231,7 @@
                 wm_dgrad[i] = take(mfma_conv_dgrad_w_bytes(cg));
                 if (op.stride == 2) grow(pmax, (size_t)s2_conv_dgrad_rows_max() * op.cin * 2 * 4);
             }
+            if (c.fwd == Fwd::head && dtype == UNET_DTYPE_BF16) grow(pmax, (size_t)head_bwd_src_blocks(cg) * op.cin * 2 * 4);
         }
         partial_bytes = pmax ? pmax : 256;
         partial_off = take(partial_bytes);
@@ -589,7 +591,7 @@
     }
 
     void backward(const float* const* params, const float* const* grad_outs, float* const* gparams, float* grad_x, int op_hi = 1 << 30,
-                  int op_lo = 0) {
+                  int op_lo = 0, const std::vector<HeadLoss>* head_loss = nullptr) {
         const Graph& g = p.g;
         if (p.side) HIP_OK(hipStreamWaitEvent(s, p.ev_packd, 0));
         {
@@ -638,6 +640,12 @@
             const int t = op.dst;
             SrcDesc sd[2] = {src(op.src[0]), op.nsrc > 1 ? src(op.src[1]) : SrcDesc()};
             ConvGeom cg = geom(op);
+            if (op.out_level >= 0 && p.conv[i].fwd == Fwd::head) {
+                ProfScope pw(i, UNET_PROF_WGRAD, sb);
+                launch_head_bwd_w(cg, sd[0], (*head_loss)[op.out_level], params[op.weight], gparams[op.weight], gparams[op.bias],
+                                  ws + p.head_op_off[i], sb);
+                return;
+            }
             const bool on_main = op.kind == OP_CONV && p.wgrad_on_main[i] && p.wz_off[i] != SIZE_MAX;
             const bool defer = gflat && p.wz_job_of_op[i] >= 0 && !on_main;
             {
@@ -698,6 +706,30 @@
             }
             int t = op.dst;
             if ((op.kind == OP_CONV) && op.out_level >= 0) {
+                const HeadLoss* hl = head_loss && (*head_loss)[op.out_level].logits ? &(*head_loss)[op.out_level] : nullptr;
+                if (hl) {
+                    const int ts = op.src[0];
+                    const Tensor& Ts = g.tensors[ts];
+                    DstGrad dgh = dst_of(ts);
+                    if (!dry) {
+                        const ConvGeom cg = geom(op);
+                        if (dgh.ptr) {
+                            ProfScope ph(i, UNET_PROF_OTHER, s);
+                            const bool can = Ts.norm >= 0 && p.first_consumer[ts] == i;
+                            BnBwdStats bn = {tptr(ts), can ? stat(Ts.norm) : nullptr, partial(), Ts.act, Ts.C};
+                            const int rows = launch_head_bwd_src(cg, *hl, params[op.weight], dgh, can ? &bn : nullptr, s);
+                            if (rows > 0) { std::lock_guard<std::mutex> lk(p.bn_mu); p.bn_pending[ws] = {ts, rows}; }
+                        }
+                        const int64_t vox = (int64_t)cg.D * cg.H * cg.W;
+                        if (!deep_seen && sb != s && vox >= hold_from) held.push_back(i);
+                        else {
+                            pending.push_back(i);
+                            if ((int)pending.size() >= fork_every || sb == s || vox >= hold_below) issue_pending();
+                        }
+                    }
+                    if (dgh.ptr) mark(op);
+                    continue;
+                }
                 if (!(grad_outs && grad_outs[op.out_level])) continue;
                 if (p.conv[i].fwd == Fwd::head) {
                     DstGrad dgh = dst_of(op.src[0]);
@@ -1006,6 +1038,41 @@
     } catch (const std::exception& e) { return fail(e.what()); }
 }
 
+namespace {
+struct LossRun;
+void head_loss_sources(const unet_plan* p, const float* const* outs, const int64_t* target, int cost_mask, int collapse_before,
+                       void* loss_scratch, std::vector<HeadLoss>& hl);
+int backward_loss(const char* who, const unet_plan* p, const float* const* params, const float* const* grad_outs, const float* const* outs,
+                  const int64_t* target, int cost_mask, int collapse_before, void* loss_scratch, float* const* grad_params, float* grad_x,
+                  void* workspace, int op_hi, int op_lo, void* stream) {
+    try {
+        if (!p || !params || !grad_params || !workspace) throw std::runtime_error(std::string(who) + ": null argument");
+        if (op_lo < 0 || op_hi < op_lo) throw std::runtime_error(std::string(who) + ": invalid op range");
+        if (grad_x) throw std::runtime_error(std::string(who) + ": grad_x must be NULL -- dL/dx is not computed");
+        std::vector<HeadLoss> hl;
+        head_loss_sources(p, outs, target, cost_mask, collapse_before, loss_scratch, hl);
+        DeviceGuard dg(p->device);
+        Exec ex(*p, workspace, stream);
+        ex.backward(params, grad_outs, grad_params, grad_x, op_hi, op_lo, &hl);
+        check_launch();
+        return 0;
+    } catch (const std::exception& e) { return fail(e.what()); }
+}
+}
+
+int unet_backward_loss(const unet_plan* p, const float* const* params, const float* const* grad_outs, const float* const* outs,
+                       const int64_t* target, int cost_mask, int collapse_before, void* loss_scratch, float* const* grad_params,
+                       float* grad_x, void* workspace, void* stream) {
+    return backward_loss("unet_backward_loss", p, params, grad_outs, outs, target, cost_mask, collapse_before, loss_scratch, grad_params, grad_x,
+                         workspace, 1 << 30, 0, stream);
+}
+int unet_backward_loss_part(const unet_plan* p, const float* const* params, const float* const* grad_outs, const float* const* outs,
+                            const int64_t* target, int cost_mask, int collapse_before, void* loss_scratch, float* const* grad_params,
+                            float* grad_x, void* workspace, int op_hi, int op_lo, void* stream) {
+    return backward_loss("unet_backward_loss_part", p, params, grad_outs, outs, target, cost_mask, collapse_before, loss_scratch, grad_params,
+                         grad_x, workspace, op_hi, op_lo, stream);
+}
+
 int unet_plan_backward_buckets(const unet_plan* p, int max_buckets, int* n_buckets, int* op_lo, int64_t* elem_lo) {
     try {
         if (!p || !n_buckets || !op_lo || !elem_lo || max_buckets < 1) throw std::runtime_error("unet_plan_backward_buckets: bad argument");
@@ -1087,6 +1154,14 @@
 int unet_loss_scratch_bytes(const unet_plan* p, size_t* bytes) { *bytes = p->loss_bytes; return 0; }
 
 namespace {
+bool loss_on_the_fly(const unet_plan& p, int level, int collapse_before) {
+    if (env().no_head_loss_fusion || p.dtype != UNET_DTYPE_BF16 || collapse_before != 0 || p.g.out_c > 8) return false;
+    for (size_t i = 0; i < p.g.ops.size(); ++i) {
+        const Op& op = p.g.ops[i];
+        if (op.kind == OP_CONV && op.out_level == level) return p.conv[i].fwd == Fwd::head && p.g.tensors[op.src[0]].needs_grad;
+    }
+    return false;
+}
 struct LossRun {
     const unet_plan* p;
     const float* const* outs; const int64_t* target; float* const* grad_outs; float* losses_out;
@@ -1095,10 +1170,11 @@
     std::vector<int64_t*> tgt;
     std::vector<float*> lvl;
     float* partial[2];
+    bool grads_in_backward = false;
     LossRun(const unet_plan* plan, const float* const* outs_, const int64_t* target_, int cost_mask_, int collapse_before, float* const* grad_outs_,
-            float* losses_out_, void* scratch)
+            float* losses_out_, void* scratch, bool need_losses = true)
         : p(plan), outs(outs_), target(target_), grad_outs(grad_outs_), losses_out(losses_out_), collapse(collapse_before), cost_mask(cost_mask_) {
-        if (!p || !outs || !target || !losses_out || !scratch) throw std::runtime_error("unet_loss: null argument");
+        if (!p || !outs || !target || (need_losses && !losses_out) || !scratch) throw std::runtime_error("unet_loss: null argument");
         const Graph& g = p->g;
         C = g.out_c;
         if (collapse_before < 0 || collapse_before >= C) throw std::runtime_error("invalid collapse_before");
@@ -1145,12 +1221,24 @@
         }
     }
     void level_partial(size_t k, int area, hipStream_t s) { launch_loss_partial(outs[k], target_of(k), C, voxels(k), collapse, partial[area], s); }
+    float weight(size_t k) const { return (1.0f / (float)(1 << k)) * inv; }
     void level_finish(size_t k, int area, hipStream_t s) {
-        const float w = (1.0f / (float)(1 << k)) * inv;
+        const float w = weight(k);
         launch_loss_finalize(partial[area], loss_blocks(voxels(k)), oc, w, cost_mask, lvl[k], losses_out, k == 0, s);
+        if (grads_in_backward && loss_on_the_fly(*p, (int)k, collapse)) return;
         if (grad_outs && grad_outs[k]) launch_loss_grad(outs[k], target_of(k), C, voxels(k), collapse, lvl[k], w, cost_mask, grad_outs[k], s);
     }
 };
+void head_loss_sources(const unet_plan* p, const float* const* outs, const int64_t* target, int cost_mask, int collapse_before,
+                       void* loss_scratch, std::vector<HeadLoss>& hl) {
+    hl.assign(p->g.outputs.size(), HeadLoss());
+    bool any = false;
+    for (size_t k = 0; k < hl.size(); ++k) any = any || loss_on_the_fly(*p, (int)k, collapse_before);
+    if (!any) return;
+    LossRun lr(p, outs, target, cost_mask, collapse_before, nullptr, nullptr, loss_scratch, false);
+    for (size_t k = 0; k < hl.size(); ++k)
+        if (loss_on_the_fly(*p, (int)k, collapse_before)) hl[k] = {outs[k], lr.target_of(k), lr.lvl[k], lr.weight(k), cost_mask};
+}
 }
 
 int unet_loss(const unet_plan* p, const float* const* outs, const int64_t* target, int cost_mask, int collapse_before,
@@ -1177,11 +1265,14 @@
                            const int64_t* target, int cost_mask, int collapse_before, float* const* grad_outs, float* losses_out,
                            void* loss_scratch, void* workspace, int mode, void* stream) {
     try {
-        if ((mode & 1) != 1 || (mode & ~(1 | UNET_MODE_PACKS_CURRENT)))
-            throw std::runtime_error("unet_forward_loss_mode: mode must be 1 (train), optionally | UNET_MODE_PACKS_CURRENT");
+        if ((mode & 1) != 1 || (mode & ~(1 | UNET_MODE_PACKS_CURRENT | UNET_MODE_LOSS_BACKWARD)))
+            throw std::runtime_error("unet_forward_loss_mode: mode must be 1 (train), optionally | UNET_MODE_PACKS_CURRENT | UNET_MODE_LOSS_BACKWARD");
+        const bool loss_backward = (mode & UNET_MODE_LOSS_BACKWARD) != 0;
+        mode &= ~UNET_MODE_LOSS_BACKWARD;
         if (!p || !params || !x || !workspace || !outs) throw std::runtime_error("unet_forward_loss: null argument");
         if (!p->g.buffers.empty() && !buffers) throw std::runtime_error("unet_forward_loss: architecture has bnorm layers but buffers is null");
         LossRun lr(p, outs, target, cost_mask, collapse_before, grad_outs, losses_out, loss_scratch);
+        lr.grads_in_backward = loss_backward;
         DeviceGuard dg(p->device);
         hipStream_t s = (hipStream_t)stream;
         const bool side = p->side && !env().no_side_stream && !g_prof;
diff --git a/unet-studio_amd/csrc/kernels.h b/unet-studio_amd/csrc/kernels.h
--- a/unet-studio_amd/csrc/kernels.h
+++ b/unet-studio_amd/csrc/kernels.h
@@ -141,6 +141,12 @@
 void launch_head_bwd(int dtype, const ConvGeom& g, const SrcDesc& src, const float* dy_ncdhw, const void* dy_cl, const float* w,
                      DstGrad dst, float* dw, float* db, void* scratch, hipStream_t s, bool defer_reduce = false);
 void launch_head_bwd_reduce(const ConvGeom& g, float* dw, float* db, const void* scratch, hipStream_t s);
+struct HeadLoss { const float* logits = nullptr; const int64_t* target = nullptr; const float* level_out = nullptr; float weight = 0.f; int cost_mask = 0; };
+struct BnBwdStats;
+int head_bwd_src_blocks(const ConvGeom& g);
+int launch_head_bwd_src(const ConvGeom& g, const HeadLoss& loss, const float* w, DstGrad dst, const BnBwdStats* bn, hipStream_t s);
+void launch_head_bwd_w(const ConvGeom& g, const SrcDesc& src, const HeadLoss& loss, const float* w, float* dw, float* db, void* scratch,
+                       hipStream_t s);
 bool conv_first_wgrad_mfma_supported(int dtype, const ConvGeom& g, const SrcDesc* src, int nsrc);
 size_t conv_first_wgrad_mfma_scratch_bytes(const ConvGeom& g);
 struct NormBwdFuse { const void* u; const float* stat; const float* coef; int act; };
diff --git a/unet-studio_amd/csrc/kernels_direct.hip b/unet-studio_amd/csrc/kernels_direct.hip
--- a/unet-studio_amd/csrc/kernels_direct.hip
+++ b/unet-studio_amd/csrc/kernels_direct.hip
@@ -1,4 +1,5 @@
 #include "device_util.h"
+#include "loss_grad.h"
 
 namespace unet {
 
@@ -775,6 +776,11 @@
     const void* dy_cl;
     DstGrad dst;
     float* slab;
+    HeadLoss loss;
+    const void* bn_u;
+    const float* bn_stat;
+    float* bn_partial;
+    int bn_act;
 };
 
 template <typename T, int CO> __global__ void __launch_bounds__(256) k_head_fwd(HeadArgs a) {
@@ -816,8 +822,7 @@
     }
 }
 
-template <typename T, int CO> __global__ void __launch_bounds__(256) k_head_bwd(HeadArgs a) {
-    extern __shared__ float sm[];
+template <typename T, int CO, bool LOSS> __device__ __forceinline__ void head_bwd_body(const HeadArgs& a, float* sm) {
     constexpr int NACC = CO * 16 + CO;
     for (int i = threadIdx.x; i < CO * a.Cin; i += 256) sm[i] = i < a.Cout * a.Cin ? a.w[i] : 0.f;
     const float* ss = stage_view<T>(a.src, sm + CO * a.Cin, a.Cin);
@@ -828,13 +833,18 @@
     float acc[NACC];
 #pragma unroll
     for (int i = 0; i < NACC; ++i) acc[i] = 0.f;
+    LossGradCoef<CO> kc;
+    if constexpr (LOSS) kc = loss_grad_coef<CO>(a.loss.level_out, a.Cout, a.loss.weight, a.loss.cost_mask);
+    int64_t tn = 0;
     auto fetch = [&](int64_t v, float (&xo)[16], float (&dout)[CO]) {
         load_chunk16<T>(a.src, plain, v, c0, true, xo, ss, a.Cin);
 #pragma unroll
         for (int c = 0; c < CO; ++c) {
             dout[c] = 0.f;
-            if (c < a.Cout) dout[c] = a.dy_planes ? a.dy_planes[(int64_t)c * a.S + v] : ld<T>((const T*)a.dy_cl, v * a.Cout + c);
-        }
+            if constexpr (LOSS) { if (c < a.Cout) dout[c] = a.loss.logits[(int64_t)c * a.S + v]; }
+            else if (c < a.Cout) dout[c] = a.dy_planes ? a.dy_planes[(int64_t)c * a.S + v] : ld<T>((const T*)a.dy_cl, v * a.Cout + c);
+        }
+        if constexpr (LOSS) tn = a.loss.target[v];
     };
     float xn[16], dn[CO];
     int64_t v0 = ((int64_t)blockIdx.x * 256 + threadIdx.x) >> a.lc;
@@ -845,7 +855,14 @@
         for (int k = 0; k < 16; ++k) x[k] = xn[k];
 #pragma unroll
         for (int c = 0; c < CO; ++c) d[c] = dn[c];
+        const int64_t t = tn;
         if (v0 + vstride < a.S) fetch(v0 + vstride, xn, dn);
+        if constexpr (LOSS) {
+            float lg[CO];
+#pragma unroll
+            for (int c = 0; c < CO; ++c) lg[c] = d[c];
+            loss_dlogits<CO>(lg, t, a.Cout, kc, d);
+        }
         if (a.slab) {
 #pragma unroll
             for (int c = 0; c < CO; ++c) {
@@ -897,6 +914,104 @@
             if (i < CO * 16) { int c = i / 16, k = i % 16; return c < Cout ? c * Cin + ch * 16 + k : -1; }
             int c = i - CO * 16;
             return (ch == 0 && c < Cout) ? O + c : -1;
+        });
+    }
+}
+
+template <typename T, int CO> __global__ void __launch_bounds__(256) k_head_bwd(HeadArgs a) {
+    extern __shared__ float sm[];
+    head_bwd_body<T, CO, false>(a, sm);
+}
+template <int CO> __global__ void __launch_bounds__(256) k_head_bwd_w(HeadArgs a) {
+    extern __shared__ float sm[];
+    head_bwd_body<bf16, CO, true>(a, sm);
+}
+
+typedef __attribute__((ext_vector_type(4))) float lds_f4;
+template <int CO> __global__ void __launch_bounds__(256) k_head_bwd_src(HeadArgs a) {
+    extern __shared__ float sm[];
+    for (int i = threadIdx.x; i < CO * a.Cin; i += 256) sm[i] = i < a.Cout * a.Cin ? a.w[i] : 0.f;
+    const bool bn = a.bn_partial != nullptr;
+    float* st4 = sm + CO * a.Cin;
+    if (bn) for (int i = threadIdx.x; i < 4 * a.Cin; i += 256) st4[i] = a.bn_stat[i];
+    __syncthreads();
+    const int nchunk = 1 << a.lc, chunk = threadIdx.x & (nchunk - 1), c0 = chunk * 16;
+    const int64_t vstride = ((int64_t)gridDim.x * 256) >> a.lc;
+    const LossGradCoef<CO> kc = loss_grad_coef<CO>(a.loss.level_out, a.Cout, a.loss.weight, a.loss.cost_mask);
+    const bool accumulate = a.dst.accumulate != 0;
+    float acc[32];
+#pragma unroll
+    for (int i = 0; i < 32; ++i) acc[i] = 0.f;
+    float lgn[CO];
+    int64_t tn = 0;
+    uint4 un0 = make_uint4(0, 0, 0, 0), un1 = un0, on0 = un0, on1 = un0;
+    auto fetch = [&](int64_t v) {
+#pragma unroll
+        for (int c = 0; c < CO; ++c) lgn[c] = c < a.Cout ? a.loss.logits[(int64_t)c * a.S + v] : 0.f;
+        tn = a.loss.target[v];
+        if (bn) { const uint4* q = (const uint4*)((const bf16*)a.bn_u + v * a.Cin + c0); un0 = q[0]; un1 = q[1]; }
+        if (accumulate) { const uint4* q = (const uint4*)((const bf16*)a.dst.ptr + v * a.dst.C + c0); on0 = q[0]; on1 = q[1]; }
+    };
+    int64_t v0 = ((int64_t)blockIdx.x * 256 + threadIdx.x) >> a.lc;
+    if (v0 < a.S) fetch(v0);
+#pragma unroll 1
+    for (; v0 < a.S; v0 += vstride) {
+        __builtin_amdgcn_fence(__ATOMIC_ACQUIRE, "workgroup", "local");
+        float lg[CO], d[CO];
+#pragma unroll
+        for (int c = 0; c < CO; ++c) lg[c] = lgn[c];
+        const int64_t t = tn;
+        const unsigned uw[8] = {un0.x, un0.y, un0.z, un0.w, un1.x, un1.y, un1.z, un1.w};
+        const unsigned ow[8] = {on0.x, on0.y, on0.z, on0.w, on1.x, on1.y, on1.z, on1.w};
+        if (v0 + vstride < a.S) fetch(v0 + vstride);
+        loss_dlogits<CO>(lg, t, a.Cout, kc, d);
+        unsigned pk[8];
+#pragma unroll
+        for (int k4 = 0; k4 < 4; ++k4) {
+            __builtin_amdgcn_sched_barrier(0);
+            float g[4] = {0.f, 0.f, 0.f, 0.f};
+#pragma unroll
+            for (int c = 0; c < CO; ++c) {
+                const lds_f4 w4 = *(const lds_f4*)(sm + c * a.Cin + c0 + 4 * k4);
+                g[0] = fmaf(d[c], w4.x, g[0]); g[1] = fmaf(d[c], w4.y, g[1]); g[2] = fmaf(d[c], w4.z, g[2]); g[3] = fmaf(d[c], w4.w, g[3]);
+            }
+            if (accumulate) {
+#pragma unroll
+                for (int e = 0; e < 2; ++e) {
+                    g[2 * e] += __uint_as_float(ow[2 * k4 + e] << 16); g[2 * e + 1] += __uint_as_float(ow[2 * k4 + e] & 0xffff0000u);
+                }
+            }
+#pragma unroll
+            for (int e = 0; e < 2; ++e) {
+                const bf16 lo = __float2bfloat16(g[2 * e]), hi = __float2bfloat16(g[2 * e + 1]);
+                pk[2 * k4 + e] = (unsigned)__builtin_bit_cast(unsigned short, lo) | ((unsigned)__builtin_bit_cast(unsigned short, hi) << 16);
+            }
+            if (bn) {
+                const lds_f4 mean = *(const lds_f4*)(st4 + c0 + 4 * k4), rstd = *(const lds_f4*)(st4 + a.Cin + c0 + 4 * k4);
+                const lds_f4 sc = *(const lds_f4*)(st4 + 2 * a.Cin + c0 + 4 * k4), sh = *(const lds_f4*)(st4 + 3 * a.Cin + c0 + 4 * k4);
+                const float mn[4] = {mean.x, mean.y, mean.z, mean.w}, rs[4] = {rstd.x, rstd.y, rstd.z, rstd.w};
+                const float sv[4] = {sc.x, sc.y, sc.z, sc.w}, hv[4] = {sh.x, sh.y, sh.z, sh.w};
+#pragma unroll
+                for (int e = 0; e < 4; ++e) {
+                    const int k = 4 * k4 + e;
+                    const unsigned gw = pk[k >> 1], uwk = uw[k >> 1];
+                    const float gs = __uint_as_float((k & 1) ? (gw & 0xffff0000u) : (gw << 16));
+                    const float u = __uint_as_float((k & 1) ? (uwk & 0xffff0000u) : (uwk << 16));
+                    const float dv = gs * act_d(fmaf(u, sv[e], hv[e]), a.bn_act);
+                    acc[k] += dv;
+                    acc[16 + k] = fmaf(dv, (u - mn[e]) * rs[e], acc[16 + k]);
+                }
+            }
+        }
+        __builtin_amdgcn_sched_barrier(0);
+        uint4* q = (uint4*)((bf16*)a.dst.ptr + v0 * a.dst.C + c0);
+        q[0] = make_uint4(pk[0], pk[1], pk[2], pk[3]); q[1] = make_uint4(pk[4], pk[5], pk[6], pk[7]);
+    }
+    if (bn) {
+        __syncthreads();
+        const int Cin = a.Cin;
+        small_wgrad_epilogue<32>(acc, nchunk, sm, a.bn_partial + (int64_t)blockIdx.x * Cin * 2, [=](int ch, int i) {
+            return i < 16 ? (ch * 16 + i) * 2 : (ch * 16 + i - 16) * 2 + 1;
         });
     }
 }
@@ -1010,4 +1125,46 @@
     slab_reduce2((const float*)scratch, nb, (int64_t)g.Cin * g.Cout + g.Cout, dw, (int64_t)g.Cin * g.Cout, db, s);
 }
 
-}
+int head_bwd_src_blocks(const ConvGeom& g) {
+    const int64_t items = ((int64_t)g.D * g.H * g.W) << ilog2_exact(g.Cin / 16);
+    const int64_t nb = (items + 255) / 256;
+    return nb < 1 ? 1 : (nb > 1024 ? 1024 : (int)nb);
+}
+static HeadArgs head_loss_args(const ConvGeom& g, const HeadLoss& loss, const float* w) {
+    HeadArgs a = {};
+    a.w = w; a.Cin = g.Cin; a.Cout = g.Cout; a.lc = ilog2_exact(g.Cin / 16);
+    a.S = (int64_t)g.D * g.H * g.W; a.loss = loss;
+    return a;
+}
+int launch_head_bwd_src(const ConvGeom& g, const HeadLoss& loss, const float* w, DstGrad dst, const BnBwdStats* bn, hipStream_t s) {
+    if (!dst.ptr) return 0;
+    HeadArgs a = head_loss_args(g, loss, w);
+    a.dst = dst;
+    if (bn) { a.bn_u = bn->u; a.bn_stat = bn->stat; a.bn_partial = bn->partial; a.bn_act = bn->act; }
+    const int CO = head_co(g.Cout), nb = head_bwd_src_blocks(g);
+    const size_t l0 = (size_t)(CO + 4) * g.Cin * 4, l1 = small_wgrad_lds_bytes(32, 1 << a.lc), lds = l0 > l1 ? l0 : l1;
+    switch (CO) {
+        case 2: k_head_bwd_src<2><<<nb, 256, lds, s>>>(a); break;
+        case 4: k_head_bwd_src<4><<<nb, 256, lds, s>>>(a); break;
+        case 6: k_head_bwd_src<6><<<nb, 256, lds, s>>>(a); break;
+        default: k_head_bwd_src<8><<<nb, 256, lds, s>>>(a); break;
+    }
+    return bn ? nb : 0;
+}
+void launch_head_bwd_w(const ConvGeom& g, const SrcDesc& src, const HeadLoss& loss, const float* w, float* dw, float* db, void* scratch,
+                       hipStream_t s) {
+    HeadArgs a = head_loss_args(g, loss, w);
+    a.src = src; a.slab = (float*)scratch;
+    const int CO = head_co(g.Cout);
+    const int nb = wgrad_reg_blocks((a.S << a.lc) * 4);
+    const size_t l0 = (size_t)(CO + 2) * g.Cin * 4, l1 = small_wgrad_lds_bytes(CO * 17, 1 << a.lc), lds = l0 > l1 ? l0 : l1;
+    switch (CO) {
+        case 2: k_head_bwd_w<2><<<nb, 256, lds, s>>>(a); break;
+        case 4: k_head_bwd_w<4><<<nb, 256, lds, s>>>(a); break;
+        case 6: k_head_bwd_w<6><<<nb, 256, lds, s>>>(a); break;
+        default: k_head_bwd_w<8><<<nb, 256, lds, s>>>(a); break;
+    }
+    slab_reduce2(a.slab, nb, (int64_t)g.Cin * g.Cout + g.Cout, dw, (int64_t)g.Cin * g.Cout, db, s);
+}
+
+}
diff --git a/unet-studio_amd/csrc/kernels_elem.hip b/unet-studio_amd/csrc/kernels_elem.hip
--- a/unet-studio_amd/csrc/kernels_elem.hip
+++ b/unet-studio_amd/csrc/kernels_elem.hip
@@ -1,4 +1,5 @@
 #include "device_util.h"
+#include "loss_grad.h"
 
 namespace unet {
 
@@ -737,7 +738,6 @@
     }
     return L;
 }
-__device__ __forceinline__ float clamp_p(float q) { return fminf(fmaxf(q, 1e-6f), 1.0f - 1e-6f); }
 
 __global__ void __launch_bounds__(256) k_loss_partial(const float* __restrict__ logits, const int64_t* __restrict__ target, int C,
                                                       int64_t S, int k, float* __restrict__ partial) {
@@ -991,20 +991,7 @@
     const int oc = C;
     const int64_t q4 = (int64_t)blockIdx.x * 256 + threadIdx.x;
     if (q4 >= (S >> 2)) return;
-    const float w_ce = (!(cost_mask & 7) || (cost_mask & 1)) ? weight : 0.f;
-    const float w_dice = (cost_mask & 2) ? weight : 0.f, w_mse = (cost_mask & 4) ? weight : 0.f;
-    const float n = level_out[3];
-    const float dden = (float)(oc - 1 > 1 ? oc - 1 : 1), eps = 1e-5f;
-    float dice_hit[OCMAX], dice_miss[OCMAX];
-#pragma unroll
-    for (int c = 0; c < OCMAX; ++c) {
-        dice_hit[c] = dice_miss[c] = 0.f;
-        if (c >= 1 && c < oc) {
-            const float den = level_out[4 + oc + c] + eps, in2 = 2.f * level_out[4 + c] + eps;
-            dice_hit[c] = w_dice * (-(2.f * 1.f * den - in2) / (den * den)) / dden;
-            dice_miss[c] = w_dice * (-(2.f * 0.f * den - in2) / (den * den)) / dden;
-        }
-    }
+    const LossGradCoef<OCMAX> k = loss_grad_coef<OCMAX>(level_out, oc, weight, cost_mask);
     const longlong2 t01 = ((const longlong2*)target)[2 * q4], t23 = ((const longlong2*)target)[2 * q4 + 1];
     const int64_t tv[4] = {t01.x, t01.y, t23.x, t23.y};
     float4 pl[OCMAX];
@@ -1014,33 +1001,12 @@
     float out[OCMAX][4];
 #pragma unroll
     for (int j = 0; j < 4; ++j) {
-        const int64_t t = tv[j];
-        const bool valid = t < C;
-        const int tt = (int)t;
-        float lg[OCMAX], mx = -INFINITY;
-#pragma unroll
-        for (int c = 0; c < OCMAX; ++c) { lg[c] = j == 0 ? pl[c].x : j == 1 ? pl[c].y : j == 2 ? pl[c].z : pl[c].w; mx = fmaxf(mx, lg[c]); }
-        float sum = 0.f;
-#pragma unroll
-        for (int c = 0; c < OCMAX; ++c) { lg[c] = c < oc ? __expf(lg[c] - mx) : 0.f; sum += lg[c]; }
-        const float inv = 1.f / sum;
-        float g[OCMAX], dot = 0.f;
-#pragma unroll
-        for (int c = 0; c < OCMAX; ++c) {
-            g[c] = 0.f;
-            if (c < oc) {
-                const float q = lg[c] * inv, p = clamp_p(q);
-                float gg = 0.f;
-                gg += w_mse * (2.f * p - (c == tt ? 2.f : 0.f)) / n;
-                if (c >= 1) gg += c == tt ? dice_hit[c] : dice_miss[c];
-                if (!(q >= 1e-6f && q <= 1.0f - 1e-6f)) gg = 0.f;
-                dot = fmaf(gg, q, dot);
-                g[c] = gg; lg[c] = q;
-            }
-        }
-#pragma unroll
-        for (int c = 0; c < OCMAX; ++c)
-            out[c][j] = (c < oc && valid) ? lg[c] * (g[c] - dot) + w_ce * (lg[c] - (c == tt ? 1.f : 0.f)) / n : 0.f;
+        float lg[OCMAX], o[OCMAX];
+#pragma unroll
+        for (int c = 0; c < OCMAX; ++c) lg[c] = j == 0 ? pl[c].x : j == 1 ? pl[c].y : j == 2 ? pl[c].z : pl[c].w;
+        loss_dlogits<OCMAX>(lg, tv[j], oc, k, o);
+#pragma unroll
+        for (int c = 0; c < OCMAX; ++c) out[c][j] = o[c];
     }
 #pragma unroll
     for (int c = 0; c < OCMAX; ++c)
diff --git a/unet-studio_amd/csrc/loss_grad.h b/unet-studio_amd/csrc/loss_grad.h
--- /dev/null
+++ b/unet-studio_amd/csrc/loss_grad.h
@@ -0,0 +1,63 @@
+#pragma once
+#include "device_util.h"
+
+namespace unet {
+
+__device__ __forceinline__ float clamp_p(float q) { return fminf(fmaxf(q, 1e-6f), 1.0f - 1e-6f); }
+
+template <int OCMAX> struct LossGradCoef {
+    float w_ce, w_mse, n;
+    float dice_hit[OCMAX], dice_miss[OCMAX];
+};
+template <int OCMAX>
+__device__ __forceinline__ LossGradCoef<OCMAX> loss_grad_coef(const float* __restrict__ level_out, int oc, float weight, int cost_mask) {
+    LossGradCoef<OCMAX> k;
+    k.w_ce = (!(cost_mask & 7) || (cost_mask & 1)) ? weight : 0.f;
+    const float w_dice = (cost_mask & 2) ? weight : 0.f;
+    k.w_mse = (cost_mask & 4) ? weight : 0.f;
+    k.n = level_out[3];
+    const float dden = (float)(oc - 1 > 1 ? oc - 1 : 1), eps = 1e-5f;
+#pragma unroll
+    for (int c = 0; c < OCMAX; ++c) {
+        k.dice_hit[c] = k.dice_miss[c] = 0.f;
+        if (c >= 1 && c < oc) {
+            const float den = level_out[4 + oc + c] + eps, in2 = 2.f * level_out[4 + c] + eps;
+            k.dice_hit[c] = w_dice * (-(2.f * 1.f * den - in2) / (den * den)) / dden;
+            k.dice_miss[c] = w_dice * (-(2.f * 0.f * den - in2) / (den * den)) / dden;
+        }
+    }
+    return k;
+}
+
+template <int OCMAX>
+__device__ __forceinline__ void loss_dlogits(const float (&lg_in)[OCMAX], int64_t t, int oc, const LossGradCoef<OCMAX>& k, float (&out)[OCMAX]) {
+#pragma clang fp contract(off)
+    const bool valid = t < oc;
+    const int tt = (int)t;
+    float lg[OCMAX], mx = -INFINITY;
+#pragma unroll
+    for (int c = 0; c < OCMAX; ++c) { lg[c] = c < oc ? lg_in[c] : -INFINITY; mx = fmaxf(mx, lg[c]); }
+    float sum = 0.f;
+#pragma unroll
+    for (int c = 0; c < OCMAX; ++c) { lg[c] = c < oc ? __expf(lg[c] - mx) : 0.f; sum += lg[c]; }
+    const float inv = 1.f / sum;
+    float g[OCMAX], dot = 0.f;
+#pragma unroll
+    for (int c = 0; c < OCMAX; ++c) {
+        g[c] = 0.f;
+        if (c < oc) {
+            const float q = lg[c] * inv, p = clamp_p(q);
+            float gg = 0.f;
+            gg += k.w_mse * (2.f * p - (c == tt ? 2.f : 0.f)) / k.n;
+            if (c >= 1) gg += c == tt ? k.dice_hit[c] : k.dice_miss[c];
+            if (!(q >= 1e-6f && q <= 1.0f - 1e-6f)) gg = 0.f;
+            dot = fmaf(gg, q, dot);
+            g[c] = gg; lg[c] = q;
+        }
+    }
+#pragma unroll
+    for (int c = 0; c < OCMAX; ++c)
+        out[c] = (c < oc && valid) ? lg[c] * (g[c] - dot) + k.w_ce * (lg[c] - (c == tt ? 1.f : 0.f)) / k.n : 0.f;
+}
+
+}
diff --git a/unet-studio_amd/csrc/unet_host.cpp b/unet-studio_amd/csrc/unet_host.cpp
--- a/unet-studio_amd/csrc/unet_host.cpp
+++ b/unet-studio_amd/csrc/unet_host.cpp
@@ -289,6 +289,48 @@
     check(unet_backward(plan, pp.data(), go.data(), gp.data(), nullptr, ws.data_ptr(), stream_of(flat_params.device())));
 }
 
+namespace {
+struct LossStep {
+    std::vector<torch::Tensor> outs, gouts;
+    std::vector<const float*> op, go;
+    torch::Tensor losses, scratch, target;
+    int mask = 0;
+};
+}
+static LossStep forward_loss_step(unet_plan* plan, torch::Tensor ws, torch::Tensor x, torch::Tensor target, bool ce, bool dice, bool mse,
+                                  int collapse_before, const std::vector<const float*>& pp, std::vector<float*>& bp)
+{
+    LossStep r;
+    int nl = 0;
+    unet_plan_output_count(plan, &nl);
+    std::vector<float*> ow, gw;
+    for (int l = 0; l < nl; ++l) {
+        int64_t d[5];
+        unet_plan_output_shape(plan, l, d);
+        if (d[1]) {
+            r.outs.push_back(torch::empty({d[0], d[1], d[2], d[3], d[4]}, torch::TensorOptions().dtype(torch::kFloat32).device(x.device())));
+            r.gouts.push_back(torch::empty_like(r.outs.back()));
+        } else {
+            r.outs.push_back(torch::Tensor());
+            r.gouts.push_back(torch::Tensor());
+        }
+        ow.push_back(d[1] ? r.outs.back().data_ptr<float>() : nullptr);
+        gw.push_back(d[1] ? r.gouts.back().data_ptr<float>() : nullptr);
+        r.op.push_back(ow.back());
+        r.go.push_back(gw.back());
+    }
+    size_t sb = 0;
+    unet_loss_scratch_bytes(plan, &sb);
+    r.scratch = torch::empty({(int64_t)sb}, torch::TensorOptions().dtype(torch::kUInt8).device(x.device()));
+    r.losses = torch::empty({4}, torch::TensorOptions().dtype(torch::kFloat32).device(x.device()));
+    r.target = target.to(torch::kLong).contiguous();
+    r.mask = (ce ? 1 : 0) | (dice ? 2 : 0) | (mse ? 4 : 0);
+    check(unet_forward_loss_mode(plan, pp.data(), bp.empty() ? nullptr : bp.data(), x.data_ptr<float>(), ow.data(), r.target.data_ptr<int64_t>(),
+                                 r.mask, collapse_before, gw.data(), r.losses.data_ptr<float>(), r.scratch.data_ptr(), ws.data_ptr(),
+                                 1 | UNET_MODE_LOSS_BACKWARD, stream_of(x.device())));
+    return r;
+}
+
 struct UNetForwardFn : torch::autograd::Function<UNetForwardFn> {
     static torch::autograd::variable_list forward(torch::autograd::AutogradContext* ctx, torch::Tensor x, torch::Tensor trigger,
                                                   int64_t self, int64_t plan, torch::Tensor ws) {
@@ -401,28 +443,19 @@
 torch::Tensor UNet3dImpl::loss_and_backward(torch::Tensor input, torch::Tensor target, bool ce, bool dice, bool mse, int collapse_before)
 {
     ensure_flat();
+    rebind_grads();
     auto x = input.to(torch::kFloat32).contiguous();
     unet_plan* plan = plan_for(x.size(2), x.size(3), x.size(4));
     auto ws = workspace_for(plan);
-    auto outs = run_forward(plan, ws, x, 1);
-    size_t sb = 0;
-    unet_loss_scratch_bytes(plan, &sb);
-    auto sc = torch::empty({(int64_t)sb}, torch::TensorOptions().dtype(torch::kUInt8).device(x.device()));
-    auto losses = torch::empty({4}, torch::TensorOptions().dtype(torch::kFloat32).device(x.device()));
-    std::vector<torch::Tensor> gouts;
-    std::vector<const float*> op;
-    std::vector<float*> gp;
-    for (auto& o : outs) {
-        gouts.push_back(o.defined() ? torch::empty_like(o) : torch::Tensor());
-        op.push_back(o.defined() ? o.data_ptr<float>() : nullptr);
-        gp.push_back(o.defined() ? gouts.back().data_ptr<float>() : nullptr);
-    }
-    auto t = target.to(torch::kLong).contiguous();
-    int mask = (ce ? 1 : 0) | (dice ? 2 : 0) | (mse ? 4 : 0);
-    check(unet_loss(plan, op.data(), t.data_ptr<int64_t>(), mask, collapse_before, gp.data(), losses.data_ptr<float>(), sc.data_ptr(),
-                    stream_of(x.device())));
-    run_backward(plan, ws, gouts);
-    return losses;
+    std::vector<const float*> pp;
+    std::vector<float*> bp, gw;
+    int64_t off = 0;
+    for (auto& p : params_) { pp.push_back(p.data_ptr<float>()); gw.push_back(flat_grads.data_ptr<float>() + off); off += p.numel(); }
+    for (auto& b : buffers_) bp.push_back(b.data_ptr<float>());
+    LossStep r = forward_loss_step(plan, ws, x, target, ce, dice, mse, collapse_before, pp, bp);
+    check(unet_backward_loss(plan, pp.data(), r.go.data(), r.op.data(), r.target.data_ptr<int64_t>(), r.mask, collapse_before,
+                             r.scratch.data_ptr(), gw.data(), nullptr, ws.data_ptr(), stream_of(x.device())));
+    return r.losses;
 }
 
 void UNet3dImpl::broadcast_parameters(int root)
@@ -466,42 +499,28 @@
     auto x = input.to(torch::kFloat32).contiguous();
     unet_plan* plan = plan_for(x.size(2), x.size(3), x.size(4));
     auto ws = workspace_for(plan);
-    auto outs = run_forward(plan, ws, x, 1);
-    size_t sb = 0;
-    unet_loss_scratch_bytes(plan, &sb);
-    auto sc = torch::empty({(int64_t)sb}, torch::TensorOptions().dtype(torch::kUInt8).device(x.device()));
-    auto losses = torch::empty({4}, torch::TensorOptions().dtype(torch::kFloat32).device(x.device()));
-    std::vector<torch::Tensor> gouts;
-    std::vector<const float*> op, go;
-    std::vector<float*> gp;
-    for (auto& o : outs) {
-        gouts.push_back(o.defined() ? torch::empty_like(o) : torch::Tensor());
-        op.push_back(o.defined() ? o.data_ptr<float>() : nullptr);
-        gp.push_back(o.defined() ? gouts.back().data_ptr<float>() : nullptr);
-        go.push_back(gp.back());
-    }
-    auto t = target.to(torch::kLong).contiguous();
-    int mask = (ce ? 1 : 0) | (dice ? 2 : 0) | (mse ? 4 : 0);
     void* st = stream_of(x.device());
-    check(unet_loss(plan, op.data(), t.data_ptr<int64_t>(), mask, collapse_before, gp.data(), losses.data_ptr<float>(), sc.data_ptr(), st));
     std::vector<const float*> pp;
-    std::vector<float*> gw;
+    std::vector<float*> bp, gw;
     int64_t off = 0;
     for (auto& p : params_) { pp.push_back(p.data_ptr<float>()); gw.push_back(flat_grads.data_ptr<float>() + off); off += p.numel(); }
+    for (auto& b : buffers_) bp.push_back(b.data_ptr<float>());
+    LossStep r = forward_loss_step(plan, ws, x, target, ce, dice, mse, collapse_before, pp, bp);
     int nb = 0, op_lo[8];
     int64_t elem_lo[8];
     check(unet_plan_backward_buckets(plan, 3, &nb, op_lo, elem_lo));
     int op_hi = 1 << 30;
     int64_t elem_hi = flat_grads.numel();
     for (int k = 0; k < nb; ++k) {
-        check(unet_backward_part(plan, pp.data(), go.data(), gw.data(), nullptr, ws.data_ptr(), op_hi, op_lo[k], st));
+        check(unet_backward_loss_part(plan, pp.data(), r.go.data(), r.op.data(), r.target.data_ptr<int64_t>(), r.mask, collapse_before,
+                                      r.scratch.data_ptr(), gw.data(), nullptr, ws.data_ptr(), op_hi, op_lo[k], st));
         if (k + 1 < nb) {
             check(unet_allreduce_grads(comm_, flat_grads.data_ptr<float>(), elem_lo[k], elem_hi, st));
             reduced_from_ = elem_lo[k];
         }
         op_hi = op_lo[k]; elem_hi = elem_lo[k];
     }
-    return losses;
+    return r.losses;
 }
 
 void UNet3dImpl::bind_optimizer_state(void)
diff --git a/unet-studio_amd/engine.py b/unet-studio_amd/engine.py
--- a/unet-studio_amd/engine.py
+++ b/unet-studio_amd/engine.py
@@ -52,6 +52,8 @@
 _sig("unet_forward", _i, _vp, _pp, _pp, _vp, _pp, _vp, _i, _vp)
 _sig("unet_backward", _i, _vp, _pp, _pp, _pp, _vp, _vp, _vp)
 _sig("unet_backward_part", _i, _vp, _pp, _pp, _pp, _vp, _vp, _i, _i, _vp)
+_sig("unet_backward_loss", _i, _vp, _pp, _pp, _pp, _vp, _i, _i, _vp, _pp, _vp, _vp, _vp)
+_sig("unet_backward_loss_part", _i, _vp, _pp, _pp, _pp, _vp, _i, _i, _vp, _pp, _vp, _vp, _i, _i, _vp)
 _sig("unet_plan_backward_buckets", _i, _vp, _i, C.POINTER(_i), C.POINTER(_i), C.POINTER(C.c_int64))
 _sig("unet_loss_scratch_bytes", _i, _vp, C.POINTER(_sz))
 _sig("unet_loss", _i, _vp, _pp, _vp, _i, _i, _pp, _vp, _vp, _vp)
@@ -93,7 +95,7 @@
     "unet_last_error", "unet_init", "unet_device_info", "unet_plan_create", "unet_plan_destroy", "unet_plan_param_count",
     "unet_plan_param_shape", "unet_plan_param_name", "unet_plan_param_decay", "unet_plan_param_fan_in", "unet_plan_buffer_count",
     "unet_plan_buffer_shape", "unet_plan_output_count", "unet_plan_output_shape", "unet_plan_workspace_bytes",
-    "unet_plan_flops", "unet_plan_describe", "unet_plan_op_count", "unet_plan_op_info", "unet_profile_begin", "unet_profile_end", "unet_forward", "unet_backward", "unet_backward_part", "unet_plan_backward_buckets", "unet_loss_scratch_bytes", "unet_loss", "unet_forward_loss", "unet_forward_loss_mode", "unet_sum_buffers",
+    "unet_plan_flops", "unet_plan_describe", "unet_plan_op_count", "unet_plan_op_info", "unet_profile_begin", "unet_profile_end", "unet_forward", "unet_backward", "unet_backward_part", "unet_backward_loss", "unet_backward_loss_part", "unet_plan_backward_buckets", "unet_loss_scratch_bytes", "unet_loss", "unet_forward_loss", "unet_forward_loss_mode", "unet_sum_buffers",
     "unet_sgd_step", "unet_pack_filters", "unet_stream_create_cu_range", "unet_stream_destroy", "unet_plan_side_cu_range", "unet_set_error", "unet_comm_unique_id", "unet_comm_create", "unet_comm_create_all", "unet_comm_destroy", "unet_comm_rank",
     "unet_allreduce_grads", "unet_allreduce_grads_all", "unet_comm_broadcast", "unet_comm_join", "unet_op_scratch_bytes", "unet_op_conv3d_fwd", "unet_op_conv3d_fwd_fused", "unet_op_conv3d_pack", "unet_op_conv3d_fwd_packed", "unet_op_conv3d_bwd_data", "unet_op_conv3d_fwd_norm", "unet_op_conv3d_bwd_data_norm", "unet_op_conv3d_bwd_weight",
     "unet_op_convt_fwd", "unet_op_convt_bwd_data", "unet_op_convt_bwd_weight", "unet_op_pack_ndhwc", "unet_op_unpack_ncdhw",
@@ -101,6 +103,7 @@
 
 
 MODE_PACKS_CURRENT = 2
+MODE_LOSS_BACKWARD = 4
 
 
 class UNetError(RuntimeError):
diff --git a/unet-studio_amd/unet3d.py b/unet-studio_amd/unet3d.py
--- a/unet-studio_amd/unet3d.py
+++ b/unet-studio_amd/unet3d.py
@@ -279,16 +279,30 @@
         go = E.ptr_array([g.data_ptr() if g is not None else None for g in grad_outs])
         E.check(E.lib.unet_backward_part(plan.handle, pp, go, gp, None, ws.data_ptr(), op_hi, op_lo, _stream_ptr(self._device)))
 
+    def _run_backward_loss(self, plan, ws, grad_outs, src, gp=None, part=None):
+        if src is None:
+            return self._run_backward(plan, ws, grad_outs, gp=gp) if part is None else self._run_backward_part(plan, ws, grad_outs, *part)
+        pp, gp = self._pp, (gp if gp is not None else self._gp)
+        go = E.ptr_array([g.data_ptr() if g is not None else None for g in grad_outs])
+        outs, target, mask, collapse_before, scratch = src
+        op = E.ptr_array([o.data_ptr() for o in outs])
+        if part is None:
+            E.check(E.lib.unet_backward_loss(plan.handle, pp, go, op, target.data_ptr(), mask, collapse_before, scratch.data_ptr(), gp, None,
+                                             ws.data_ptr(), _stream_ptr(self._device)))
+        else:
+            E.check(E.lib.unet_backward_loss_part(plan.handle, pp, go, op, target.data_ptr(), mask, collapse_before, scratch.data_ptr(), gp,
+                                                  None, ws.data_ptr(), part[0], part[1], _stream_ptr(self._device)))
+
     def forward_backward_bucketed(self, x, target, on_bucket, cost_ce=True, cost_dice=True, cost_mse=True, collapse_before=0,
                                   max_buckets=3, packs_current=False, losses_out=None):
         x = self._check_input(x)
         plan = self.plan_for(x.shape[2:])
         ws = self._workspace(plan)
-        outs, losses, gouts = self._run_forward_loss(plan, ws, x, target, cost_ce, cost_dice, cost_mse, collapse_before, packs_current,
-                                                     losses_out=losses_out)
+        outs, losses, gouts, src = self._run_forward_loss(plan, ws, x, target, cost_ce, cost_dice, cost_mse, collapse_before, packs_current,
+                                                          losses_out=losses_out, loss_backward=True)
         op_hi, elem_hi = 1 << 30, int(self.flat_grads.numel())
         for op_lo, elem_lo in plan.backward_buckets(max_buckets):
-            self._run_backward_part(plan, ws, gouts, op_hi, op_lo)
+            self._run_backward_loss(plan, ws, gouts, src, part=(op_hi, op_lo))
             on_bucket(int(elem_lo), elem_hi)
             op_hi, elem_hi = op_lo, int(elem_lo)
         return losses
@@ -314,9 +328,9 @@
     def forward_backward_lane(self, lane, x, target, gp, cost_ce=True, cost_dice=True, cost_mse=True, collapse_before=0, packs_current=False):
         x = self._check_input(x)
         plan, ws = lane["plan"], lane["ws"]
-        outs, losses, gouts = self._run_forward_loss(plan, ws, x, target, cost_ce, cost_dice, cost_mse, collapse_before, packs_current,
-                                                     loss_scratch=lane["loss"])
-        self._run_backward(plan, ws, gouts, gp=gp)
+        outs, losses, gouts, src = self._run_forward_loss(plan, ws, x, target, cost_ce, cost_dice, cost_mse, collapse_before, packs_current,
+                                                          loss_scratch=lane["loss"], loss_backward=True)
+        self._run_backward_loss(plan, ws, gouts, src, gp=gp)
         return losses
 
     def _check_input(self, x):
@@ -355,9 +369,9 @@
         x = self._check_input(x)
         plan = self.plan_for(x.shape[2:])
         ws = self._workspace(plan)
-        outs, losses, gouts = self._run_forward_loss(plan, ws, x, target, cost_ce, cost_dice, cost_mse, collapse_before, packs_current,
-                                                     losses_out=losses_out)
-        self._run_backward(plan, ws, gouts)
+        outs, losses, gouts, src = self._run_forward_loss(plan, ws, x, target, cost_ce, cost_dice, cost_mse, collapse_before, packs_current,
+                                                          losses_out=losses_out, loss_backward=True)
+        self._run_backward_loss(plan, ws, gouts, src)
         return losses
 
     def _loss_scratch(self, plan):
@@ -369,7 +383,7 @@
         return sc
 
     def _run_forward_loss(self, plan, ws, x, target, cost_ce, cost_dice, cost_mse, collapse_before, packs_current=False, loss_scratch=None,
-                          losses_out=None):
+                          losses_out=None, loss_backward=False):
         if target.dtype != torch.int64 or target.device != self._device:
             raise E.UNetError("target must be an int64 tensor on the model's device")
         target = target.contiguous()
@@ -379,19 +393,22 @@
             if losses_out is not None:
                 losses_out.copy_(losses)
                 losses = losses_out
-            return outs, losses, gouts
+            return (outs, losses, gouts, None) if loss_backward else (outs, losses, gouts)
         outs = [torch.empty(s, dtype=torch.float32, device=self._device) for s in plan.output_shapes]
         gouts = [torch.empty_like(o) for o in outs]
         losses = losses_out if losses_out is not None else torch.empty(4, dtype=torch.float32, device=self._device)
         mask = (1 if cost_ce else 0) | (2 if cost_dice else 0) | (4 if cost_mse else 0)
-        mode = 1 | (E.MODE_PACKS_CURRENT if packs_current else 0)
+        mode = 1 | (E.MODE_PACKS_CURRENT if packs_current else 0) | (E.MODE_LOSS_BACKWARD if loss_backward else 0)
+        scratch = loss_scratch if loss_scratch is not None else self._loss_scratch(plan)
         E.check(E.lib.unet_forward_loss_mode(plan.handle, self._pp, self._bp, x.data_ptr(), E.ptr_array([o.data_ptr() for o in outs]),
                                              target.data_ptr(), mask, collapse_before, E.ptr_array([g.data_ptr() for g in gouts]),
-                                             losses.data_ptr(), (loss_scratch if loss_scratch is not None else self._loss_scratch(plan)).data_ptr(),
+                                             losses.data_ptr(), scratch.data_ptr(),
                                              ws.data_ptr(), mode,
                                              _stream_ptr(self._device)))
         if self._buffers:
             self.num_batches_tracked += 1
+        if loss_backward:
+            return outs, losses, gouts, (outs, target, mask, collapse_before, scratch)
         return outs, losses, gouts
 
     def loss(self, outs, target, cost_ce=True, cost_dice=True, cost_mse=True, collapse_before=0, want_grad=True, plan=None):
```

New measurement: 754.2 million. 0.945x the previous value.
